# PARC-projects/video-query-algorithms

Measured on AMD Instinct MI355X. Metric: clips/sec TSN feature-extract, higher is better.
Workload: dtype f32; 1 GPU; configs[1]: TSN BN-Inception RGB, 224x224x3, T=3, B=32/GPU (96 crops/step), crops in HBM; global_batch=32, parallelism=dp1

## Files before the change

video-query-algorithms_amd/csrc/vq_tsn.hip:

```cpp
#include <algorithm>
#include <cmath>
#include <cstring>
#include <map>
#include <set>
#include <tuple>
#include <type_traits>
#include <vector>

#include "vq_common.h"
#include "vq_tsn_kernels.h"
#include "host/vq_block_pool.h"

using namespace vq;

typedef float floatx16 __attribute__((ext_vector_type(16)));
typedef float floatx4 __attribute__((ext_vector_type(4)));
typedef unsigned uintx4 __attribute__((__vector_size__(4 * sizeof(unsigned))));

__global__ void preprocess_kernel(const uint8_t* __restrict__ src, float* __restrict__ dst, int64_t nchunk, int C, int Cpad,
                                  const float* __restrict__ mean) {
    const int64_t i = (int64_t)blockIdx.x * blockDim.x + threadIdx.x;
    if (i >= nchunk) return;
    const int cpp = Cpad >> 2;
    const int64_t p = i / cpp;
    const int c0 = (int)(i - p * cpp) * 4;
    floatx4 v;
#pragma unroll
    for (int e = 0; e < 4; ++e) v[e] = c0 + e < C ? (float)src[p * C + c0 + e] - mean[c0 + e] : 0.0f;
    *reinterpret_cast<floatx4*>(dst + p * Cpad + c0) = v;
}

__global__ void preprocess_s2d_kernel(const uint8_t* __restrict__ src, float* __restrict__ dst, int64_t nchunk, int H, int W, int C,
                                      int Hs, int Ws, int pad, const float* __restrict__ mean, int xmajor) {
    const int64_t i = (int64_t)blockIdx.x * blockDim.x + threadIdx.x;
    if (i >= nchunk) return;
    const int64_t cell = i / C;
    const int j0 = (int)(i - cell * C) * 4;
    const int X = (int)(cell % Ws), Y = (int)((cell / Ws) % Hs);
    const int64_t n = cell / ((int64_t)Ws * Hs);
    floatx4 v;
#pragma unroll
    for (int e = 0; e < 4; ++e) {
        const int j = j0 + e, pq = j / C, c = j - pq * C;
        const int p = xmajor ? pq & 1 : pq >> 1, q = xmajor ? pq >> 1 : pq & 1;
        const int y = 2 * Y + p - pad, x = 2 * X + q - pad;
        const bool in = (unsigned)y < (unsigned)H && (unsigned)x < (unsigned)W;
        v[e] = in ? (float)src[((n * H + y) * W + x) * C + c] - mean[c] : 0.0f;
    }
    *reinterpret_cast<floatx4*>(dst + cell * (4 * C) + j0) = v;
}

__global__ __launch_bounds__(256) void preprocess_s2d3_kernel(const uint8_t* __restrict__ src, float* __restrict__ dst, int64_t ncell, int H, int W,
                                                              int Hs, int Ws, int pad, const float* __restrict__ mean, int xmajor) {
    const int64_t cell = (int64_t)blockIdx.x * blockDim.x + threadIdx.x;
    if (cell >= ncell) return;
    const int X = (int)(cell % Ws);
    const int64_t ny = cell / Ws;
    const int Y = (int)(ny % Hs);
    const int64_t n = ny / Hs;
    const float m0 = mean[0], m1 = mean[1], m2 = mean[2];
    float v[12];
#pragma unroll
    for (int p = 0; p < 2; ++p) {
        const int y = 2 * Y + p - pad;
        const bool row_in = (unsigned)y < (unsigned)H;
        const uint8_t* r = src + ((n * H + (row_in ? y : 0)) * W) * 3;
#pragma unroll
        for (int q = 0; q < 2; ++q) {
            const int x = 2 * X + q - pad;
            const bool in = row_in && (unsigned)x < (unsigned)W;
            const uint8_t* px = r + (in ? x : 0) * 3;
            const float a = (float)px[0] - m0, b = (float)px[1] - m1, c = (float)px[2] - m2;
            const int slot = xmajor ? q * 2 + p : p * 2 + q;
            v[slot * 3 + 0] = in ? a : 0.0f;
            v[slot * 3 + 1] = in ? b : 0.0f;
            v[slot * 3 + 2] = in ? c : 0.0f;
        }
    }
    floatx4* o = reinterpret_cast<floatx4*>(dst + cell * 12);
#pragma unroll
    for (int k = 0; k < 3; ++k) {
        floatx4 t;
        t[0] = v[4 * k], t[1] = v[4 * k + 1], t[2] = v[4 * k + 2], t[3] = v[4 * k + 3];
        o[k] = t;
    }
}

struct ConvSeg {
    float* out_base;
    int Cs;
    int relu;
};

struct ConvArgs {
    const float* in;
    const ConvSeg* segs;
    float* out;
    const float* w;
    const float* bias;
    const float* zeros;
    int H, W, Cs_in, coff_in, Cin;
    int Ho, Wo, Cs_out, coff_out, Cout;
    int k, stride, pad;
    int kw;
    int col_off;
    int c_step;
    int M, Kp, relu;
    int out_row0;
    int pool_k, pool_s;
    int tiles_m, tiles_n;
    unsigned in_bytes, w_bytes;
    int ksplit;
    int k_per;
    int seg_stride;
    unsigned m_tiles_n;
    FullDiv d_howo, d_wo;
    unsigned s_wo, s_ho;
};

constexpr int KPAD = 32;
static inline int stem_rows_kp(int c) { return 4 * ((14 * c + 3) / 4 * 4); }

template <int BM, int BN, int BK>
struct ConvSmem {
    float a[2][BM][BK + 4];
    float b[2][BN][BK + 4];
};

#define VQ_EPILOGUE()                                                                                             \
    {                                                                                                             \
        __syncthreads();                                \
        float* patch = reinterpret_cast<float*>(smem_raw) + wave * (32 * 36);                                     \
        const int prow = lane >> 3, pc4 = lane & 7;                                                               \
        const bool full_m = m0 + BM <= a.M;                                                                       \
        _Pragma("unroll") for (int j = 0; j < TN; ++j) {                                                          \
            const int nb = n0 + wn * (BN / WN) + 32 * j;                                                          \
            if (nb < a.Cout) {                                                                                    \
                const ConvSeg sg = seg_v[j];                                                                      \
                _Pragma("unroll") for (int i = 0; i < TM; ++i) {                                                  \
                    _Pragma("unroll") for (int r = 0; r < 16; ++r)                                                \
                        patch[((r & 3) + 8 * (r >> 2) + 4 * half) * 36 + l31] = acc[i][j][r];                     \
                    const int mb = m0 + wm * (BM / WM) + 32 * i;                                                  \
                    _Pragma("unroll") for (int ps = 0; ps < 4; ++ps) {                                            \
                        const int row = prow + 8 * ps;                                                            \
                        floatx4 v = *reinterpret_cast<const floatx4*>(&patch[row * 36 + pc4 * 4]);                \
                        v += bias_v[j];                                                                           \
                        if (sg.relu) {                                                                            \
                            v[0] = fmaxf(v[0], 0.f);                                                              \
                            v[1] = fmaxf(v[1], 0.f);                                                              \
                            v[2] = fmaxf(v[2], 0.f);                                                              \
                            v[3] = fmaxf(v[3], 0.f);                                                              \
                        }                                                                                         \
                        if ((full_m || mb + row < a.M) && nb + pc4 * 4 < a.Cout)                                  \
                            *reinterpret_cast<floatx4*>(sg.out_base + (size_t)(a.out_row0 + mb + row) * sg.Cs + nb + pc4 * 4) = v; \
                    }                                                                                             \
                }                                                                                                 \
            }                                                                                                     \
        }                                                                                                         \
    }

#define VQ_EPILOGUE_BUF()                                                                                         \
    {                                                                                                             \
        __syncthreads();                                \
        float* patch = reinterpret_cast<float*>(smem_raw) + wave * (32 * 36);                                     \
        const int prow = lane >> 3, pc4 = lane & 7;                                                               \
        const bool full_m = m0 + BM <= a.M;                                                                       \
        _Pragma("unroll") for (int j = 0; j < TN; ++j) {                                                          \
            const int nb = n0 + wn * (BN / WN) + 32 * j;                                                          \
            if (nb < a.Cout) {                                                                                    \
                const ConvSeg sg = seg_v[j];                                                                      \
                const __amdgpu_buffer_rsrc_t o_rsrc =                                                             \
                    __builtin_amdgcn_make_buffer_rsrc(sg.out_base + (size_t)a.out_row0 * sg.Cs, 0, 0x7FFFFFF0u, 0x00020000); \
                const unsigned lane_off = nb + pc4 * 4 < a.Cout ? (unsigned)((imul24(prow, sg.Cs) + pc4 * 4) * 4) : 0xFFFFFFFFu; \
                _Pragma("unroll") for (int i = 0; i < TM; ++i) {                                                  \
                    _Pragma("unroll") for (int r = 0; r < 16; ++r)                                                \
                        patch[((r & 3) + 8 * (r >> 2) + 4 * half) * 36 + l31] = acc[i][j][r];                     \
                    const int mb = m0 + wm * (BM / WM) + 32 * i;                                                  \
                    _Pragma("unroll") for (int ps = 0; ps < 4; ++ps) {                                            \
                        const int row = prow + 8 * ps;                                                            \
                        floatx4 v = *reinterpret_cast<const floatx4*>(&patch[row * 36 + pc4 * 4]);                \
                        v += bias_v[j];                                                                           \
                        if (sg.relu) {                                                                            \
                            v[0] = fmaxf(v[0], 0.f);                                                              \
                            v[1] = fmaxf(v[1], 0.f);                                                              \
                            v[2] = fmaxf(v[2], 0.f);                                                              \
                            v[3] = fmaxf(v[3], 0.f);                                                              \
                        }                                                                                         \
                        const unsigned off = (full_m || mb + row < a.M) ? lane_off : 0xFFFFFFFFu;                 \
                        __builtin_amdgcn_raw_buffer_store_b128(__builtin_bit_cast(uintx4, v), o_rsrc, off,        \
                                                               ((mb + 8 * ps) * sg.Cs + nb) * 4, 0);              \
                    }                                                                                             \
                }                                                                                                 \
            }                                                                                                     \
        }                                                                                                         \
    }

template <int BM, int BN, int WM, int WN, int BK, bool SMALL_CIN, bool POOL = false>
__global__ __launch_bounds__(256) void conv_igemm_kernel(ConvArgs a) {
    static_assert(WM * WN == 4, "4 waves per workgroup");
    static_assert(BK == 16 || BK == 32, "BK is 16 or 32");
    static_assert(!(POOL && SMALL_CIN), "the pooled loader walks whole channel chunks");
    constexpr int TM = BM / WM / 32, TN = BN / WN / 32;
    constexpr int CPR = BK / 4;
    constexpr int NA = (BM * CPR + 255) / 256, NB = (BN * CPR + 255) / 256;
    extern __shared__ __attribute__((aligned(16))) char smem_raw[];
    ConvSmem<BM, BN, BK>& sm = *reinterpret_cast<ConvSmem<BM, BN, BK>*>(smem_raw);

    const int tid = threadIdx.x;
    const int n_tiles = a.tiles_m * a.tiles_n;
    const int ks = a.ksplit > 1 ? (int)blockIdx.x / n_tiles : 0;
    const int kbeg = ks * a.k_per;
    const int tile = xcd_remap(blockIdx.x - ks * n_tiles, n_tiles);
    const int m0 = (tile / a.tiles_n) * BM;
    const int n0 = (tile % a.tiles_n) * BN;

    const float* a_img[NA];
    int a_ih0[NA], a_iw0[NA], a_row[NA], a_col[NA];
    const int HoWo = a.Ho * a.Wo;
#pragma unroll
    for (int i = 0; i < NA; ++i) {
        const int c = tid + 256 * i;
        a_row[i] = c / CPR;
        a_col[i] = c % CPR;
        const int m = m0 + a_row[i];
        const bool ok = m < a.M && a_row[i] < BM;
        const int mm = ok ? m : 0;
        const int n_img = mm / HoWo, rem = mm - n_img * HoWo;
        const int oh = rem / a.Wo, ow = rem - oh * a.Wo;
        a_img[i] = a.in + (size_t)n_img * a.H * a.W * a.Cs_in + a.coff_in;
        a_ih0[i] = ok ? oh * a.stride - a.pad : -(1 << 20);
        a_iw0[i] = ow * a.stride - a.pad;
        if (POOL) {
            a_ih0[i] = ok ? oh * a.pool_s : -(1 << 20);
            a_iw0[i] = ow * a.pool_s;
        }
    }
    const float* b_ptr[NB];
    bool b_ok[NB];
    int b_row[NB], b_col[NB];
#pragma unroll
    for (int i = 0; i < NB; ++i) {
        const int c = tid + 256 * i;
        b_row[i] = c / CPR;
        b_col[i] = c % CPR;
        const int n = n0 + b_row[i];
        b_ok[i] = n < a.Cout && b_row[i] < BN;
        b_ptr[i] = a.w + (size_t)(b_ok[i] ? n : 0) * a.Kp + b_col[i] * 4 + kbeg;
    }

    floatx4 ra[NA], rb[NB];
    constexpr int PT = POOL ? 8 : 1;
    floatx4 rp[NA][PT];
    int kh = 0, kw = 0, c0 = 0;
    if (!SMALL_CIN && kbeg > 0) {
        const int tap0 = kbeg / a.Cin;
        c0 = kbeg - tap0 * a.Cin;
        kh = tap0 / a.kw;
        kw = tap0 - kh * a.kw;
    }
#define VQ_LOAD_TILES(KC)                                                                                          \
    {                                                                                                              \
        _Pragma("unroll") for (int i = 0; i < NA; ++i) {                                                           \
            const float* src = a.zeros;                                                                            \
            if (SMALL_CIN) {                                                                                       \
                const int kidx = ((KC) * CPR + a_col[i]) * 4;                                                      \
                const int tap = kidx / a.Cin, c = kidx - tap * a.Cin;                                              \
                const int th = tap / a.kw, tw = tap - th * a.kw;                                                   \
                const int ih = a_ih0[i] + th, iw = a_iw0[i] + tw;                                                  \
                if (tap < a.k * a.kw && (unsigned)ih < (unsigned)a.H && (unsigned)iw < (unsigned)a.W)              \
                    src = a_img[i] + ((size_t)ih * a.W + iw) * a.Cs_in + c;                                        \
            } else if (POOL) {                                                                                     \
                      \
                const bool ok = a_ih0[i] >= 0;                                                                     \
                if (ok) src = a_img[i] + ((size_t)a_ih0[i] * a.W + a_iw0[i]) * a.Cs_in + c0 + a_col[i] * a.col_off; \
                _Pragma("unroll") for (int t = 1; t < 9; ++t) {                                                    \
                    const int ih = a_ih0[i] + t / 3, iw = a_iw0[i] + t % 3;                                        \
                    const float* q = src;                                                                          \
                    if (ok && ih < a.H && iw < a.W) q = a_img[i] + ((size_t)ih * a.W + iw) * a.Cs_in + c0 + a_col[i] * a.col_off; \
                    rp[i][t - 1] = *reinterpret_cast<const floatx4*>(q);                                           \
                }                                                                                                  \
            } else {                                                                                               \
                const int ih = a_ih0[i] + kh, iw = a_iw0[i] + kw;                                                  \
                if ((unsigned)ih < (unsigned)a.H && (unsigned)iw < (unsigned)a.W)                                  \
                    src = a_img[i] + ((size_t)ih * a.W + iw) * a.Cs_in + c0 + a_col[i] * a.col_off;                \
            }                                                                                                      \
            ra[i] = *reinterpret_cast<const floatx4*>(src);                                                        \
        }                                                                                                          \
        _Pragma("unroll") for (int i = 0; i < NB; ++i)                                                             \
            rb[i] = *reinterpret_cast<const floatx4*>(b_ok[i] ? b_ptr[i] + (size_t)(KC) * BK : a.zeros);           \
        if (!SMALL_CIN) {                                                                                          \
            c0 += a.c_step ? a.c_step : BK;                                                                        \
            if (c0 >= a.Cin) {                                                                                     \
                c0 = 0;                                                                                            \
                if (++kw == a.kw) {                                                                                \
                    kw = 0;                                                                                        \
                    ++kh;                                                                                          \
                }                                                                                                  \
            }                                                                                                      \
        }                                                                                                          \
    }
#define VQ_STORE_TILES(BUF)                                                                                        \
    {                                                                                                              \
        if (POOL) {                                                                                                \
            _Pragma("unroll") for (int i = 0; i < NA; ++i)                                                         \
                _Pragma("unroll") for (int t = 0; t < 8; ++t)                                                      \
                    _Pragma("unroll") for (int e = 0; e < 4; ++e) ra[i][e] = fmaxf(ra[i][e], rp[i][t][e]);         \
        }                                                                                                          \
        _Pragma("unroll") for (int i = 0; i < NA; ++i)                                                             \
            if ((BM * CPR) % 256 == 0 || a_row[i] < BM)                                                            \
                *reinterpret_cast<floatx4*>(&sm.a[BUF][a_row[i]][a_col[i] * 4]) = ra[i];                           \
        _Pragma("unroll") for (int i = 0; i < NB; ++i)                                                             \
            if ((BN * CPR) % 256 == 0 || b_row[i] < BN)                                                            \
                *reinterpret_cast<floatx4*>(&sm.b[BUF][b_row[i]][b_col[i] * 4]) = rb[i];                           \
    }

    const int wave = tid >> 6, lane = tid & 63, l31 = lane & 31, half = lane >> 5;
    const int wm = wave / WN, wn = wave % WN;
    const int arow0 = wm * (BM / WM) + l31, brow0 = wn * (BN / WN) + l31;
    floatx16 acc[TM][TN];
#pragma unroll
    for (int i = 0; i < TM; ++i)
#pragma unroll
        for (int j = 0; j < TN; ++j)
#pragma unroll
            for (int r = 0; r < 16; ++r) acc[i][j][r] = 0.f;

    floatx4 bias_v[TN];
    ConvSeg seg_v[TN];
#pragma unroll
    for (int j = 0; j < TN; ++j) {
        const int nb_ = n0 + wn * (BN / WN) + 32 * j;
        const int n = nb_ + (lane & 7) * 4;
        bias_v[j] = *reinterpret_cast<const floatx4*>(a.bias + (n < a.Cout ? n : 0));
        seg_v[j] = a.segs[ks * a.seg_stride + (nb_ < a.Cout ? nb_ >> 5 : 0)];
    }

    const int nk = (a.ksplit > 1 ? a.k_per : a.Kp) / BK;
    VQ_LOAD_TILES(0)
    VQ_STORE_TILES(0)
    __syncthreads();
    for (int kc = 0; kc < nk; ++kc) {
        const int buf = kc & 1;
        if (kc + 1 < nk) VQ_LOAD_TILES(kc + 1)
#pragma unroll
        for (int kk = 0; kk < BK / 8; ++kk) {
            floatx4 af[TM], bf[TN];
#pragma unroll
            for (int i = 0; i < TM; ++i) af[i] = *reinterpret_cast<const floatx4*>(&sm.a[buf][arow0 + 32 * i][kk * 8 + half * 4]);
#pragma unroll
            for (int j = 0; j < TN; ++j) bf[j] = *reinterpret_cast<const floatx4*>(&sm.b[buf][brow0 + 32 * j][kk * 8 + half * 4]);
#pragma unroll
            for (int s = 0; s < 4; ++s)
#pragma unroll
                for (int i = 0; i < TM; ++i)
#pragma unroll
                    for (int j = 0; j < TN; ++j)
                        acc[i][j] = __builtin_amdgcn_mfma_f32_32x32x2f32(af[i][s], bf[j][s], acc[i][j], 0, 0, 0);
        }
        if (kc + 1 < nk) VQ_STORE_TILES(buf ^ 1)
        __syncthreads();
    }

    VQ_EPILOGUE()
#undef VQ_LOAD_TILES
#undef VQ_STORE_TILES
}

#ifndef VQ_PIPE_WPE
#define VQ_PIPE_WPE 4
#endif
template <int BM, int BN, int WM, int WN, int BK, bool SMALL_CIN>
__global__ __launch_bounds__(256) __attribute__((amdgpu_waves_per_eu(BM * BN == 128 * 64 && BK == 16 ? VQ_PIPE_WPE : 1, 8)))
void conv_igemm_pipe_kernel(ConvArgs a) {
    static_assert(WM * WN == 4, "4 waves per workgroup");
    constexpr int NT = 256;
    constexpr int TM = BM / WM / 32, TN = BN / WN / 32;
    constexpr int CPR = BK / 4;
    constexpr int NA = (BM * CPR + NT - 1) / NT, NB = (BN * CPR + NT - 1) / NT;
    constexpr int NKK = BK / 8;
    constexpr int MFK = 4 * TM * TN;
    constexpr int NMF = NKK * MFK;
    constexpr int NFR = TM + TN;
    constexpr int NG = NA + NB;
    constexpr int NFREE = NMF - (NKK - 1) * NFR;
    static_assert(NFREE >= 2 * NG, "not enough MFMA gaps for the staging slices");
    constexpr bool EARLY = (NKK - 1) * (MFK - NFR) >= NG && NFREE - NFR >= 2 * NG;
    extern __shared__ __attribute__((aligned(16))) char smem_raw[];
    ConvSmem<BM, BN, BK>& sm = *reinterpret_cast<ConvSmem<BM, BN, BK>*>(smem_raw);

    const int tid = threadIdx.x;
    const int n_tiles = a.tiles_m * a.tiles_n;
    const int ks = a.ksplit > 1 ? (int)blockIdx.x / n_tiles : 0;
    const int kbeg = ks * a.k_per;
    const int tile = xcd_remap(blockIdx.x - ks * n_tiles, n_tiles);
    const int tm = (int)magic_div((unsigned)tile, a.m_tiles_n);
    const int m0 = tm * BM;
    const int n0 = (tile - tm * a.tiles_n) * BN;
    const unsigned img0 = full_div((unsigned)m0, a.d_howo), rem0 = (unsigned)m0 - img0 * (unsigned)(a.Ho * a.Wo);
    const unsigned oh0 = full_div(rem0, a.d_wo), ow0 = rem0 - oh0 * (unsigned)a.Wo;

    const __amdgpu_buffer_rsrc_t in_rsrc = __builtin_amdgcn_make_buffer_rsrc(const_cast<float*>(a.in), 0, a.in_bytes, 0x00020000);
    const __amdgpu_buffer_rsrc_t w_rsrc = __builtin_amdgcn_make_buffer_rsrc(const_cast<float*>(a.w), 0, a.w_bytes, 0x00020000);
    int a_off[NA];
    unsigned long long a_mask[NA];
    int a_row[NA], a_col[NA];
    const unsigned HW = (unsigned)(a.H * a.W);
#pragma unroll
    for (int i = 0; i < NA; ++i) {
        const int c = tid + NT * i;
        a_row[i] = c / CPR;
        a_col[i] = c % CPR;
        const bool ok = m0 + a_row[i] < a.M && a_row[i] < BM;
        const unsigned lin = ow0 + (unsigned)a_row[i];
        const unsigned q1 = umul24(lin, a.s_wo) >> kRecipShift;
        const unsigned ly = oh0 + q1;
        const unsigned q2 = umul24(ly, a.s_ho) >> kRecipShift;
        const int ow = (int)(lin - umul24(q1, (unsigned)a.Wo)), oh = (int)(ly - umul24(q2, (unsigned)a.Ho));
        const int ih0 = imul24(oh, a.stride) - a.pad, iw0 = imul24(ow, a.stride) - a.pad;
        a_off[i] = (imul24((int)umul24(img0 + q2, HW) + imul24(ih0, a.W) + iw0, a.Cs_in) + a.coff_in + (SMALL_CIN ? 0 : imul24(a_col[i], a.col_off))) * 4;
        unsigned long long mask = 0;
        for (int th = 0; th < a.k; ++th)
            for (int tw = 0; tw < a.kw; ++tw)
                if (ok && (unsigned)(ih0 + th) < (unsigned)a.H && (unsigned)(iw0 + tw) < (unsigned)a.W) mask |= 1ull << (th * a.kw + tw);
        a_mask[i] = mask;
    }
    unsigned b_off[NB];
    int b_row[NB], b_col[NB];
#pragma unroll
    for (int i = 0; i < NB; ++i) {
        const int c = tid + NT * i;
        b_row[i] = c / CPR;
        b_col[i] = c % CPR;
        const int n = n0 + b_row[i];
        b_off[i] = (n < a.Cout && b_row[i] < BN) ? (unsigned)((imul24(n, a.Kp) + b_col[i] * 4 + kbeg) * 4) : 0xFFFFFFFFu;
    }

    floatx4 ra[2][NA], rb[2][NB];
    int kh = 0, kw = 0, c0 = 0, tap = 0;
    unsigned a_voff[NA];
    if (!SMALL_CIN && kbeg > 0) {
        tap = kbeg / a.Cin;
        c0 = kbeg - tap * a.Cin;
        kh = tap / a.kw;
        kw = tap - kh * a.kw;
    }
    {
        const int tap_pix0 = ((kh * a.W + kw) * a.Cs_in) * 4;
#pragma unroll
        for (int i = 0; i < NA; ++i) a_voff[i] = ((a_mask[i] >> tap) & 1ull) ? (unsigned)(a_off[i] + tap_pix0) : 0xFFFFFFFFu;
    }
    const int c_step = a.c_step ? a.c_step : BK;
    const unsigned cpt = (unsigned)a.Cin >> 2, inv_cpt = 65536u / cpt + 1u, inv_k = 65536u / (unsigned)a.kw + 1u;

    const int wave = __builtin_amdgcn_readfirstlane(tid >> 6), lane = tid & 63, l31 = lane & 31, half = lane >> 5;
    const int wm = wave / WN, wn = wave % WN;
    const int arow0 = wm * (BM / WM) + l31, brow0 = wn * (BN / WN) + l31;
    floatx16 acc[TM][TN];
#pragma unroll
    for (int i = 0; i < TM; ++i)
#pragma unroll
        for (int j = 0; j < TN; ++j)
#pragma unroll
            for (int r = 0; r < 16; ++r) acc[i][j][r] = 0.f;
    floatx4 bias_v[TN];
    ConvSeg seg_v[TN];
#pragma unroll
    for (int j = 0; j < TN; ++j) {
        const int nb_ = n0 + wn * (BN / WN) + 32 * j;
        const int n = nb_ + (lane & 7) * 4;
        bias_v[j] = *reinterpret_cast<const floatx4*>(a.bias + (n < a.Cout ? n : 0));
        seg_v[j] = a.segs[ks * a.seg_stride + (nb_ < a.Cout ? nb_ >> 5 : 0)];
    }

#define VQ_G_LOAD(IDX, KC, SET)                                                                                \
    {                                                                                                          \
        if ((IDX) < NA) {                                                                                      \
            const int ii = (IDX) < NA ? (IDX) : 0;                                                             \
            unsigned off;                                                                                      \
            if (SMALL_CIN) {                                                                                   \
                const unsigned g_ = (unsigned)(KC) * CPR + a_col[ii];                                          \
                const unsigned tap_ = (g_ * inv_cpt) >> 16, c4_ = g_ - tap_ * cpt;                             \
                const unsigned th_ = (tap_ * inv_k) >> 16, tw_ = tap_ - th_ * a.kw;                            \
                const unsigned ok_ = (unsigned)(a_mask[ii] >> (tap_ & 63u)) & (tap_ < 64u ? 1u : 0u);          \
                off = ok_ ? (unsigned)(a_off[ii] + (int)(((th_ * a.W + tw_) * a.Cs_in + c4_ * 4) * 4)) : 0xFFFFFFFFu; \
            } else {                                                                                           \
                off = a_voff[ii];                                                                              \
            }                                                                                                  \
            ra[SET][ii] = __builtin_bit_cast(floatx4, __builtin_amdgcn_raw_buffer_load_b128(in_rsrc, off, SMALL_CIN ? 0 : c0 * 4, 0)); \
        } else {                                                                                               \
            const int ii = (IDX) >= NA ? (IDX) - NA : 0;                                                       \
            rb[SET][ii] = __builtin_bit_cast(floatx4, __builtin_amdgcn_raw_buffer_load_b128(w_rsrc, b_off[ii], (KC) * (BK * 4), 0)); \
        }                                                                                                      \
    }
#define VQ_G_STORE(IDX, BUF, SET)                                                                              \
    {                                                                                                          \
        if ((IDX) < NA) {                                                                                      \
            const int ii = (IDX) < NA ? (IDX) : 0;                                                             \
            if ((BM * CPR) % NT == 0 || a_row[ii] < BM)                                                        \
                *reinterpret_cast<floatx4*>(&sm.a[BUF][a_row[ii]][a_col[ii] * 4]) = ra[SET][ii];               \
        } else {                                                                                               \
            const int ii = (IDX) >= NA ? (IDX) - NA : 0;                                                       \
            if ((BN * CPR) % NT == 0 || b_row[ii] < BN)                                                        \
                *reinterpret_cast<floatx4*>(&sm.b[BUF][b_row[ii]][b_col[ii] * 4]) = rb[SET][ii];               \
        }                                                                                                      \
    }
#define VQ_ADVANCE_TAP()                                                                     \
    if (!SMALL_CIN) {                                                                        \
        c0 += c_step;                                                                        \
        if (c0 >= a.Cin) {                                                                   \
            c0 = 0;                                                                          \
            ++tap;                                                                           \
            if (++kw == a.kw) {                                                              \
                kw = 0;                                                                      \
                ++kh;                                                                        \
            }                                                                                \
            asm volatile("" ::: "memory");                  \
            const int tap_pix = ((kh * a.W + kw) * a.Cs_in) * 4;                             \
            _Pragma("unroll") for (int i = 0; i < NA; ++i)                                   \
                a_voff[i] = ((a_mask[i] >> tap) & 1ull) ? (unsigned)(a_off[i] + tap_pix) : 0xFFFFFFFFu; \
        }                                                                                    \
    }
#define VQ_PIPE_STEP(BUF, KC, DO_STORE, DO_LOAD, SS, SL)                                                       \
    {                                                                                                          \
        if (!EARLY) {                                                                                          \
            _Pragma("unroll") for (int i = 0; i < TM; ++i)                                                     \
                fa[0][i] = *reinterpret_cast<const floatx4*>(&sm.a[BUF][arow0 + 32 * i][half * 4]);            \
            _Pragma("unroll") for (int j = 0; j < TN; ++j)                                                     \
                fb[0][j] = *reinterpret_cast<const floatx4*>(&sm.b[BUF][brow0 + 32 * j][half * 4]);            \
        }                                                                                                      \
        _Pragma("unroll") for (int q = 0; q < NMF; ++q) {                                                      \
            const int kk = q / MFK, r = q % MFK, s_ = r / (TM * TN), i_ = (r / TN) % TM, j_ = r % TN;          \
            acc[i_][j_] = __builtin_amdgcn_mfma_f32_32x32x2f32(fa[kk & 1][i_][s_], fb[kk & 1][j_][s_], acc[i_][j_], 0, 0, 0); \
            if (kk + 1 < NKK && r < NFR) {                                                                     \
                if (r < TM)                                                                                    \
                    fa[(kk + 1) & 1][r < TM ? r : 0] = *reinterpret_cast<const floatx4*>(                      \
                        &sm.a[BUF][arow0 + 32 * (r < TM ? r : 0)][(kk + 1) * 8 + half * 4]);                   \
                else                                                                                           \
                    fb[(kk + 1) & 1][r >= TM ? r - TM : 0] = *reinterpret_cast<const floatx4*>(                \
                        &sm.b[BUF][brow0 + 32 * (r >= TM ? r - TM : 0)][(kk + 1) * 8 + half * 4]);             \
            } else if (EARLY && (DO_STORE) && kk + 1 == NKK && r < NFR) {                                      \
                if (r < TM)                                                                                    \
                    fa[0][r < TM ? r : 0] = *reinterpret_cast<const floatx4*>(                                 \
                        &sm.a[(BUF) ^ 1][arow0 + 32 * (r < TM ? r : 0)][half * 4]);                            \
                else                                                                                           \
                    fb[0][r >= TM ? r - TM : 0] = *reinterpret_cast<const floatx4*>(                           \
                        &sm.b[(BUF) ^ 1][brow0 + 32 * (r >= TM ? r - TM : 0)][half * 4]);                      \
            } else {                                                                                           \
                const int fidx = q - (kk + 1 < NKK ? (kk + 1) * NFR : (NKK - 1) * NFR + (EARLY && (DO_STORE) ? NFR : 0)); \
                if ((DO_STORE) && fidx < NG) {                                                                 \
                    VQ_G_STORE(fidx < NG ? fidx : 0, (BUF) ^ 1, SS)                                            \
                    if (EARLY && fidx == NG - 1) __syncthreads();            \
                } else if ((DO_LOAD) && fidx >= NG && fidx < 2 * NG)                                           \
                    VQ_G_LOAD(fidx - NG < NG ? fidx - NG : 0, (KC) + 2, SL)                                    \
            }                                                                                                  \
            __builtin_amdgcn_sched_barrier(0);                                                                 \
        }                                                                                                      \
    }

    const int nk = (a.ksplit > 1 ? a.k_per : a.Kp) / BK;
    _Pragma("unroll") for (int i = 0; i < NG; ++i) VQ_G_LOAD(i, 0, 0)
    _Pragma("unroll") for (int i = 0; i < NG; ++i) VQ_G_STORE(i, 0, 0)
    if (nk > 1) {
        VQ_ADVANCE_TAP()
        _Pragma("unroll") for (int i = 0; i < NG; ++i) VQ_G_LOAD(i, 1, 1)
    }
    __syncthreads();
    floatx4 fa[2][TM], fb[2][TN];
    if (EARLY) {
#pragma unroll
        for (int i = 0; i < TM; ++i) fa[0][i] = *reinterpret_cast<const floatx4*>(&sm.a[0][arow0 + 32 * i][half * 4]);
#pragma unroll
        for (int j = 0; j < TN; ++j) fb[0][j] = *reinterpret_cast<const floatx4*>(&sm.b[0][brow0 + 32 * j][half * 4]);
    }
#define VQ_END_BARRIER()                                                     \
    {                                                                        \
        if (EARLY) {                                                         \
            asm volatile("s_waitcnt lgkmcnt(%0)" ::"n"(NFR) : "memory");     \
            __builtin_amdgcn_s_barrier();                                    \
            asm volatile("" ::: "memory");                                   \
        } else {                                                             \
            __syncthreads();                                                 \
        }                                                                    \
    }
    const int n_steady = nk > 2 ? nk - 2 : 0;
    int kc = 0;
    for (; kc + 1 < n_steady; kc += 2) {
        VQ_ADVANCE_TAP()
        VQ_PIPE_STEP(0, kc, true, true, 1, 0)
        VQ_END_BARRIER()
        VQ_ADVANCE_TAP()
        VQ_PIPE_STEP(1, kc + 1, true, true, 0, 1)
        VQ_END_BARRIER()
    }
    if (kc < n_steady) {
        VQ_ADVANCE_TAP()
        VQ_PIPE_STEP(0, kc, true, true, 1, 0)
        VQ_END_BARRIER()
        ++kc;
    }
    if (kc + 1 < nk) {
        if (kc & 1) {
            VQ_PIPE_STEP(1, kc, true, false, 0, 0)
        } else {
            VQ_PIPE_STEP(0, kc, true, false, 1, 1)
        }
        VQ_END_BARRIER()
        ++kc;
    }
    if (kc & 1) {
        VQ_PIPE_STEP(1, kc, false, false, 0, 0)
    } else {
        VQ_PIPE_STEP(0, kc, false, false, 0, 0)
    }
    VQ_EPILOGUE_BUF()
#undef VQ_G_LOAD
#undef VQ_G_STORE
#undef VQ_ADVANCE_TAP
#undef VQ_PIPE_STEP
#undef VQ_END_BARRIER
}

template <int BM, int BN, int WM, int WN>
__global__ __launch_bounds__(256) void pool_gemm_kernel(ConvArgs a) {
    static_assert(WM * WN == 4, "4 waves per workgroup");
    static_assert(BM == 64 || BM == 128, "two staged chunks per thread and slab");
    constexpr int TM = BM / WM / 32, TN = BN / WN / 32;
    constexpr int SLAB = 2048 / BM;
    constexpr int CPS = SLAB / 4;
    constexpr int GS = SLAB / 8;
    extern __shared__ __attribute__((aligned(16))) char smem_raw[];
    float* As = reinterpret_cast<float*>(smem_raw);
    const int K = a.Cin, pitch = K + 4;
    const int tid = threadIdx.x;
    const int tile = xcd_remap(blockIdx.x, a.tiles_m * a.tiles_n);
    const int m0 = (tile / a.tiles_n) * BM, n0 = (tile % a.tiles_n) * BN;
    const __amdgpu_buffer_rsrc_t in_rsrc = __builtin_amdgcn_make_buffer_rsrc(const_cast<float*>(a.in), 0, a.in_bytes, 0x00020000);
    const __amdgpu_buffer_rsrc_t w_rsrc = __builtin_amdgcn_make_buffer_rsrc(const_cast<float*>(a.w), 0, a.w_bytes, 0x00020000);

    const int wave = tid >> 6, lane = tid & 63, l31 = lane & 31, half = lane >> 5;
    const int wm = wave / WN, wn = wave % WN;
    floatx4 bias_v[TN];
    ConvSeg seg_v[TN];
    unsigned b_voff[TN];
#pragma unroll
    for (int j = 0; j < TN; ++j) {
        const int nb_ = n0 + wn * (BN / WN) + 32 * j;
        const int n = nb_ + (lane & 7) * 4;
        bias_v[j] = *reinterpret_cast<const floatx4*>(a.bias + (n < a.Cout ? n : 0));
        seg_v[j] = a.segs[nb_ < a.Cout ? nb_ >> 5 : 0];
        b_voff[j] = nb_ + l31 < a.Cout ? (unsigned)(((nb_ + l31) * a.Kp + half * 4) * 4) : 0xFFFFFFFFu;
    }

    unsigned tap_base[2], tap_ok[2];
    int a_dst[2];
    const int px = a.Cs_in * 4, rowb = a.W * px;
    {
        const int HoWo = a.Ho * a.Wo;
#pragma unroll
        for (int u = 0; u < 2; ++u) {
            const int idx = tid + 256 * u, row = idx / CPS, col = idx % CPS;
            const int m = m0 + row;
            const bool ok = m < a.M;
            const int mm = ok ? m : 0;
            const int n_img = mm / HoWo, rem = mm - n_img * HoWo;
            const int oh = rem / a.Wo, ow = rem - oh * a.Wo;
            const int ih0 = oh * a.pool_s, iw0 = ow * a.pool_s;
            tap_base[u] = ok ? (unsigned)((((n_img * a.H + ih0) * a.W + iw0) * a.Cs_in + a.coff_in + col * 4) * 4) : 0xFFFFFFFFu;
            const int nvy = min(3, a.H - ih0), nvx = min(3, a.W - iw0);
            unsigned mask = 0;
#pragma unroll
            for (int t = 0; t < 9; ++t)
                if (ok && t / 3 < nvy && t % 3 < nvx) mask |= 1u << t;
            tap_ok[u] = mask;
            a_dst[u] = row * pitch + col * 4;
        }
    }
    floatx4 v[2][9];
#define VQ_PG_TAPS(S)                                                                                               \
    _Pragma("unroll") for (int u = 0; u < 2; ++u) {                                                                 \
        unsigned inside = tap_ok[u];                                                                                \
        asm volatile("" : "+v"(inside));  \
        _Pragma("unroll") for (int t = 0; t < 9; ++t)                                                               \
            v[u][t] = __builtin_bit_cast(floatx4, __builtin_amdgcn_raw_buffer_load_b128(                            \
                in_rsrc, tap_base[u] + (((inside >> t) & 1u) ? (unsigned)((t / 3) * rowb + (t % 3) * px) : 0u), (S) * (SLAB * 4), 0)); \
    }
#define VQ_PG_POOL(S)                                                                                               \
    _Pragma("unroll") for (int u = 0; u < 2; ++u) {                                                                 \
        floatx4 r;                                                                                                  \
        _Pragma("unroll") for (int e = 0; e < 4; ++e) {                                                             \
            const float x = __builtin_fmaxf(__builtin_fmaxf(v[u][0][e], v[u][1][e]), v[u][2][e]);                  \
            const float y = __builtin_fmaxf(__builtin_fmaxf(v[u][3][e], v[u][4][e]), v[u][5][e]);                  \
            const float z = __builtin_fmaxf(__builtin_fmaxf(v[u][6][e], v[u][7][e]), v[u][8][e]);                  \
            r[e] = __builtin_fmaxf(__builtin_fmaxf(x, y), z);                                                       \
        }                                                                                                           \
        *reinterpret_cast<floatx4*>(As + a_dst[u] + (S) * SLAB) = r;                                                \
    }

    floatx16 acc[TM][TN];
#pragma unroll
    for (int i = 0; i < TM; ++i)
#pragma unroll
        for (int j = 0; j < TN; ++j)
#pragma unroll
            for (int r = 0; r < 16; ++r) acc[i][j][r] = 0.f;
    const float* a_frag = As + (wm * (BM / WM) + l31) * pitch + half * 4;
    floatx4 fa[2][TM], fbs[2][GS][TN];
#define VQ_PG_FETCH_B(SET, S)                                                                                       \
    _Pragma("unroll") for (int q = 0; q < GS; ++q)                                                                  \
        _Pragma("unroll") for (int j = 0; j < TN; ++j)                                                              \
            fbs[SET][q][j] = __builtin_bit_cast(floatx4, __builtin_amdgcn_raw_buffer_load_b128(w_rsrc, b_voff[j], ((S) * GS + q) * 32, 0));
#define VQ_PG_FETCH_A(SET, G)                                                                                       \
    _Pragma("unroll") for (int i = 0; i < TM; ++i)                                                                  \
        fa[SET][i] = *reinterpret_cast<const floatx4*>(a_frag + 32 * i * pitch + (G) * 8);
#define VQ_PG_MFMA(SET, BSET, Q)                                                                                    \
    _Pragma("unroll") for (int s_ = 0; s_ < 4; ++s_)                                                                \
        _Pragma("unroll") for (int i = 0; i < TM; ++i)                                                              \
            _Pragma("unroll") for (int j = 0; j < TN; ++j)                                                          \
                acc[i][j] = __builtin_amdgcn_mfma_f32_32x32x2f32(fa[SET][i][s_], fbs[BSET][Q][j][s_], acc[i][j], 0, 0, 0);
#define VQ_PG_SLAB(S, BSET)                                                                                         \
    {                                                                                                               \
        const bool more = (S) + 1 < ns;                                                                             \
        if (more) {                                                                                                 \
            VQ_PG_FETCH_B((BSET) ^ 1, (S) + 1)                                                                      \
            VQ_PG_TAPS((S) + 1)                                              \
        }                                                                                                           \
        VQ_PG_FETCH_A(0, (S) * GS)                                                                                  \
        __builtin_amdgcn_sched_barrier(0);                                                                          \
        _Pragma("unroll") for (int q = 0; q < GS; ++q) {                                                            \
            if (q + 1 < GS) VQ_PG_FETCH_A((q + 1) & 1, (S) * GS + q + 1)                                            \
            __builtin_amdgcn_sched_barrier(0);                                                                      \
            VQ_PG_MFMA(q & 1, BSET, q)                                                                              \
            __builtin_amdgcn_sched_barrier(0);                                                                      \
        }                                                                                                           \
        if (more) {                                                                                                 \
            VQ_PG_POOL((S) + 1)                                                                                     \
            __syncthreads();                                  \
        }                                                                                                           \
    }

    const int ns = K / SLAB;
    VQ_PG_FETCH_B(0, 0)
    VQ_PG_TAPS(0)
    VQ_PG_POOL(0)
    __syncthreads();
    int s = 0;
    for (; s + 1 < ns; s += 2) {
        VQ_PG_SLAB(s, 0)
        VQ_PG_SLAB(s + 1, 1)
    }
    if (s < ns) VQ_PG_SLAB(s, 0)
#undef VQ_PG_SLAB
#undef VQ_PG_TAPS
#undef VQ_PG_POOL
#undef VQ_PG_FETCH_A
#undef VQ_PG_FETCH_B
#undef VQ_PG_MFMA
    VQ_EPILOGUE()
}

template <bool IS_MAX>
__global__ __launch_bounds__(256) void pool_kernel(PoolArgs a) {
    const int64_t i = (int64_t)blockIdx.x * blockDim.x + threadIdx.x;
    if (i < a.total) pool_one<IS_MAX>(a, i);
}

__global__ void gavgpool_kernel(const float* __restrict__ in, float* __restrict__ out, int n, int HW, int Cs_in, int coff_in,
                                int C, int Cs_out, int coff_out) {
    const int i = blockIdx.x * blockDim.x + threadIdx.x;
    if (i >= n * C) return;
    const int c = i % C, img = i / C;
    const float* p = in + (size_t)img * HW * Cs_in + coff_in + c;
    float acc = 0.f;
    for (int q = 0; q < HW; ++q) acc += p[(size_t)q * Cs_in];
    out[(size_t)img * Cs_out + coff_out + c] = acc / (float)HW;
}

__global__ void splitk_combine_kernel(const float* __restrict__ part, int ksplit, size_t slice_stride, int M, int Cout,
                                      const float* __restrict__ bias, int relu, float* __restrict__ out, int Cs_out) {
    const int64_t i = (int64_t)blockIdx.x * blockDim.x + threadIdx.x;
    const int c4 = Cout / 4;
    if (i >= (int64_t)M * c4) return;
    const int m = (int)(i / c4), n = (int)(i - (int64_t)m * c4) * 4;
    floatx4 v = *reinterpret_cast<const floatx4*>(part + (size_t)m * Cout + n);
    for (int q = 1; q < ksplit; ++q) v += *reinterpret_cast<const floatx4*>(part + q * slice_stride + (size_t)m * Cout + n);
    v += *reinterpret_cast<const floatx4*>(bias + n);
    if (relu) {
        v[0] = fmaxf(v[0], 0.f);
        v[1] = fmaxf(v[1], 0.f);
        v[2] = fmaxf(v[2], 0.f);
        v[3] = fmaxf(v[3], 0.f);
    }
    *reinterpret_cast<floatx4*>(out + (size_t)m * Cs_out + n) = v;
}

constexpr int kMaxFusedT = 16;
__global__ void gavgpool_consensus_kernel(const float* __restrict__ in, float* __restrict__ out, double* __restrict__ feat, int T,
                                          int HW, int Cs_in, int coff_in, int C, int Cs_out, int coff_out) {
    __shared__ float pooled[kMaxFusedT][64];
    const int c = blockIdx.x * 64 + threadIdx.x, t = threadIdx.y, b = blockIdx.y;
    float v = 0.f;
    if (c < C) {
        const int img = b * T + t;
        const float* p = in + (size_t)img * HW * Cs_in + coff_in + c;
        float acc = 0.f;
        int q = 0;
        for (; q + 7 <= HW; q += 7) {
            float x[7];
#pragma unroll
            for (int u = 0; u < 7; ++u) x[u] = p[(size_t)(q + u) * Cs_in];
#pragma unroll
            for (int u = 0; u < 7; ++u) acc += x[u];
        }
        for (; q < HW; ++q) acc += p[(size_t)q * Cs_in];
        v = acc / (float)HW;
        out[(size_t)img * Cs_out + coff_out + c] = v;
    }
    pooled[t][threadIdx.x] = v;
    __syncthreads();
    if (t == 0 && c < C) {
        double cons = (double)pooled[0][threadIdx.x];
        for (int s = 1; s < T; ++s) cons = cons + (double)pooled[s][threadIdx.x];
        feat[(size_t)b * C + c] = cons / (double)T;
    }
}

__global__ void consensus_kernel(const float* __restrict__ per_snippet, double* __restrict__ feat, int B, int T, int D, int Cs) {
    const int i = blockIdx.x * blockDim.x + threadIdx.x;
    if (i >= B * D) return;
    const int d = i % D, b = i / D;
    double acc = (double)per_snippet[(size_t)(b * T) * Cs + d];
    for (int t = 1; t < T; ++t) acc = acc + (double)per_snippet[(size_t)(b * T + t) * Cs + d];
    feat[i] = acc / (double)T;
}

static inline double first_layer_k2c(const vq_input_desc& in, const vq_layer_desc& L) {
    if (L.src != 0) return (double)L.k * L.k * L.cin;
    const int k = (in.s2d_pad >= 0 && in.s2d_kernel > 0) ? in.s2d_kernel : L.k;
    return (double)k * k * in.c;
}

static inline bool is_wino(int op) { return op == VQ_OP_CONV_WINOGRAD || op == VQ_OP_CONV_WINOGRAD16; }
static inline bool is_conv(int op) { return op == VQ_OP_CONV || is_wino(op); }

struct LaunchItem {
    int kind = 0;
    std::vector<int> layers;
    int max_crops = 0;
};

struct vq_tsn {
    std::mutex mu;
    int device = 0;
    hipStream_t stream = nullptr;
    int cus = 256;
    int max_crops = 0;
    int in_channels = 0;
    vq_input_desc input = {0, 0, 0, -1, 0};
    std::vector<vq_tensor_desc> tensors;
    std::vector<vq_layer_desc> layers;
    std::vector<LaunchItem> items;
    std::vector<int> item_of_layer;
    int consensus_layer = -1;
    std::map<int, std::vector<int>> tuned;
    std::map<int, int> split_pref;
    std::set<int> tuned_borrowed;
    bool autotune = true;
    bool group_wino = true;
    bool group_pool = true;
    bool poison = false;
    int forced_tile = -1;
    std::vector<float*> slots;
    std::vector<size_t> slot_bytes;
    size_t blob_bytes = 0;
    float* zeros = nullptr;
    ConvSeg* seg_table = nullptr;
    std::vector<int> seg_table_off;
    std::vector<int> ksplit;
    float* split_scratch = nullptr;
    size_t split_slice_floats = 0;
    size_t split_crop_floats = 0;
    float* zero_bias = nullptr;
    float* blob = nullptr;
    int64_t blob_floats = 0;
    int feature_slot = -1, D = 0;
    uint8_t* crops_dev = nullptr;
    size_t crops_cap = 0;
    float* mean_dev = nullptr;
    std::vector<float> mean_cached;
    double* feat_dev = nullptr;
    double flops_per_crop = 0;
    int last_crops = 0;
    int cur_T = 1;
    bool fused_consensus = false;
    int profile_depth = 0;
    int profile_count = 0;
    int profile_every = 1;
    int profile_tick = 0;
    bool profile_split = false;
    std::vector<hipEvent_t> events;
    int crop_off = 0;
    int n_split = 1;
    std::vector<int> split_parts;
    hipStream_t ls = nullptr;
    hipEvent_t ev_start = nullptr, ev_stop = nullptr;
    std::vector<hipStream_t> split_streams;
    hipEvent_t fork_ev = nullptr;
    std::vector<hipEvent_t> join_ev;
};

static vq::BlockPool& device_pool() {
    static vq::BlockPool p(vq::BlockPool::cap_from_env());
    return p;
}
void vq::device_pool_trim() {
    for (void* blk : device_pool().drain()) (void)hipFree(blk);
}
static hipError_t pool_alloc(int device, size_t bytes, void** out) {
    if (void* blk = device_pool().take(device, bytes)) {
        *out = blk;
        return hipSuccess;
    }
    hipError_t e = hipMalloc(out, bytes);
    if (e == hipErrorOutOfMemory) {
        (void)hipGetLastError();
        vq::device_pool_trim();
        e = hipMalloc(out, bytes);
    }
    return e;
}
static void pool_free(int device, void* p, size_t bytes) {
    if (!p) return;
    if (!device_pool().give(device, p, bytes)) (void)hipFree(p);
}

static void tsn_free(vq_tsn* net) {
    for (hipEvent_t e : net->events) (void)hipEventDestroy(e);
    net->events.clear();
    for (hipEvent_t e : net->join_ev)
        if (e) (void)hipEventDestroy(e);
    if (net->fork_ev) (void)hipEventDestroy(net->fork_ev);
    for (hipStream_t st : net->split_streams)
        if (st) (void)hipStreamDestroy(st);
    for (size_t i = 0; i < net->slots.size(); ++i) pool_free(net->device, net->slots[i], i < net->slot_bytes.size() ? net->slot_bytes[i] : 0);
    pool_free(net->device, net->blob, net->blob_bytes);
    if (net->zeros) (void)hipFree(net->zeros);
    if (net->seg_table) (void)hipFree(net->seg_table);
    pool_free(net->device, net->split_scratch, net->split_slice_floats * 4 * sizeof(float));
    if (net->zero_bias) (void)hipFree(net->zero_bias);
    if (net->crops_dev) (void)hipFree(net->crops_dev);
    if (net->mean_dev) (void)hipFree(net->mean_dev);
    if (net->feat_dev) (void)hipFree(net->feat_dev);
}

enum : int { kConv = 1, kPipe = 2, kPool = 4, kGemm = 8 };

constexpr size_t kPoolGemmMaxLds = 64 * 1024;
static size_t pool_gemm_lds(int bm, int K) { return std::max((size_t)bm * (K + 4) * sizeof(float), (size_t)4 * 32 * 36 * sizeof(float)); }

static bool pixel_walk_ok(const ConvArgs& a) {
    const long long n_img = cdiv(a.M, a.Ho * a.Wo);
    return n_img * a.H * a.W < (1 << 23) && a.Cs_in < (1 << 23) && a.Kp < (1 << 23) && a.Cout < (1 << 23) && a.stride < (1 << 23) &&
           recip22_ok((unsigned)a.Wo, (unsigned)a.Wo + 128u) && recip22_ok((unsigned)a.Ho, (unsigned)a.Ho + 130u);
}

template <int BM, int BN, int WM, int WN, int BK, int KERNEL, bool SMALL>
static int launch_conv_t(vq_tsn* net, ConvArgs& a) {
    a.tiles_m = cdiv(a.M, BM);
    a.tiles_n = cdiv(a.Cout, BN);
    void (*kern)(ConvArgs);
    size_t lds = sizeof(ConvSmem<BM, BN, BK>), lds_max = lds;
    if constexpr (KERNEL == kPipe) {
        VQ_REQUIRE(pixel_walk_ok(a) && (unsigned long long)a.tiles_m * a.tiles_n * a.tiles_n < 0x100000000ull,
                   "pipelined convolution: shape outside the range of its reciprocal divisions");
        a.m_tiles_n = a.tiles_n == 1 ? 0u : (unsigned)(0x100000000ull / (unsigned)a.tiles_n) + 1u;
        a.d_howo = full_div_for((unsigned)(a.Ho * a.Wo));
        a.d_wo = full_div_for((unsigned)a.Wo);
        a.s_wo = recip22((unsigned)a.Wo);
        a.s_ho = recip22((unsigned)a.Ho);
        kern = conv_igemm_pipe_kernel<BM, BN, WM, WN, BK, SMALL>;
    } else if constexpr (KERNEL == kGemm) {
        VQ_REQUIRE(a.pool_k == 3 && a.Cin % 32 == 0 && a.Kp == a.Cin, "pool_gemm_kernel: a 3x3 window over a multiple of 32 channels");
        kern = pool_gemm_kernel<BM, BN, WM, WN>;
        lds = pool_gemm_lds(BM, a.Cin);
        lds_max = kPoolGemmMaxLds;
    } else {
        kern = conv_igemm_kernel<BM, BN, WM, WN, BK, SMALL, KERNEL == kPool>;
    }
    VQ_DYN_LDS(kern, lds_max);
    VQ_LAUNCH(kern, a.tiles_m * a.tiles_n * a.ksplit, 256, lds, net->ls, net->ev_start, net->ev_stop, a);
    VQ_CHECK_LAUNCH();
    return VQ_OK;
}

typedef int (*ConvLaunch)(vq_tsn*, ConvArgs&);

struct ConvTile {
    int bm, bn, bk;
    int pipe;
    ConvLaunch conv[2];
    ConvLaunch piped[2];
    ConvLaunch pooled;
};

template <int BM, int BN, int BK, int WM, int WN, int HAS>
constexpr ConvTile tiling() {
    ConvTile t{BM, BN, BK, (HAS & kGemm) ? 3 : (HAS & kPipe) ? 1 : 0, {}, {}, nullptr};
    if constexpr ((HAS & (kConv | kPipe)) != 0) {
        t.conv[0] = launch_conv_t<BM, BN, WM, WN, BK, kConv, false>;
        t.conv[1] = launch_conv_t<BM, BN, WM, WN, BK, kConv, true>;
    }
    if constexpr ((HAS & kPipe) != 0) {
        t.piped[0] = launch_conv_t<BM, BN, WM, WN, BK, kPipe, false>;
        t.piped[1] = launch_conv_t<BM, BN, WM, WN, BK, kPipe, true>;
    }
    if constexpr ((HAS & kPool) != 0) t.pooled = launch_conv_t<BM, BN, WM, WN, BK, kPool, false>;
    if constexpr ((HAS & kGemm) != 0) t.pooled = launch_conv_t<BM, BN, WM, WN, BK, kGemm, false>;
    return t;
}

static constexpr ConvTile kTiles[] = {
    tiling<128, 128, 32, 2, 2, kConv>(), tiling<128, 128, 16, 2, 2, kConv | kPool>(),
    tiling<128, 96, 32, 4, 1, kConv>(),  tiling<128, 96, 16, 4, 1, kConv | kPool>(),
    tiling<128, 64, 32, 2, 2, kConv>(),  tiling<128, 64, 16, 2, 2, kConv | kPool>(),
    tiling<64, 128, 32, 2, 2, kConv | kPool>(), tiling<64, 128, 16, 2, 2, kConv | kPool>(),
    tiling<64, 64, 32, 2, 2, kConv | kPool>(),  tiling<64, 64, 16, 2, 2, kConv | kPool>(),
    tiling<128, 32, 32, 4, 1, kConv>(),  tiling<128, 32, 16, 4, 1, kConv | kPool>(),
    tiling<32, 128, 32, 1, 4, kConv>(),  tiling<32, 128, 16, 1, 4, kConv>(),
    tiling<128, 128, 32, 2, 2, kPipe>(), tiling<128, 128, 16, 2, 2, kPipe>(),
    tiling<128, 96, 32, 4, 1, kPipe>(),  tiling<128, 96, 16, 4, 1, kPipe>(),
    tiling<128, 64, 32, 2, 2, kPipe>(),  tiling<128, 64, 16, 2, 2, kPipe>(),
    tiling<64, 128, 32, 2, 2, kPipe>(),  tiling<64, 128, 16, 2, 2, kPipe>(),
    tiling<64, 64, 32, 2, 2, kPipe>(),   tiling<64, 64, 16, 2, 2, kPipe>(),
    tiling<128, 32, 32, 4, 1, kPipe>(),  tiling<128, 32, 16, 4, 1, kPipe>(),
    tiling<32, 128, 32, 1, 4, kPipe>(),  tiling<32, 128, 16, 1, 4, kPipe>(),
    tiling<64, 256, 16, 1, 4, kPool>(), tiling<64, 256, 8, 1, 4, kGemm>(), tiling<64, 64, 8, 2, 2, kGemm>(), tiling<128, 64, 8, 2, 2, kGemm>()};
constexpr int kNumTiles = (int)(sizeof(kTiles) / sizeof(kTiles[0]));

static int tile_index(int bm, int bn, int bk, int pipe) {
    for (int i = 0; i < kNumTiles; ++i)
        if (kTiles[i].bm == bm && kTiles[i].bn == bn && kTiles[i].bk == bk && kTiles[i].pipe == pipe) return i;
    return -1;
}

static bool pooled_ok(const ConvTile& t, int K) { return t.pooled && (t.pipe != 3 || pool_gemm_lds(t.bm, K) <= kPoolGemmMaxLds); }

static bool tile_candidate(const vq_layer_desc& L, const ConvTile& t, bool timed) {
    if (!timed) return t.pipe == 0 && t.bk == 32 && t.conv[0];
    if (L.pre_pool_k > 0 ? !pooled_ok(t, L.cin) : !t.conv[0]) return false;
    return t.bn < 2 * ((L.cout + 63) / 64 * 64);
}

static int heuristic_tile(const vq_tsn* net, int li, int n_crops) {
    const vq_layer_desc& L = net->layers[li];
    const vq_tensor_desc& td = net->tensors[L.dst];
    const int M = n_crops * td.h * td.w, N = L.cout;
    int best = 0;
    double bs = -1;
    for (int i = 0; i < kNumTiles; ++i) {
        const ConvTile& t = kTiles[i];
        if (!tile_candidate(L, t, false)) continue;
        const long long tiles = (long long)cdiv(M, t.bm) * cdiv(N, t.bn);
        const double per_cu = (double)tiles / net->cus;
        const double balance = per_cu / std::ceil(per_cu);
        const double padding = ((double)M * N) / ((double)tiles * t.bm * t.bn);
        const double area = (double)t.bm * t.bn;
        const double intrinsic = area >= 128 * 128 ? 1.0 : area >= 128 * 96 ? 0.97 : area >= 128 * 64 ? 0.92 : area >= 64 * 64 ? 0.8 : 0.7;
        const double sc = balance * padding * intrinsic;
        if (sc > bs) {
            bs = sc;
            best = i;
        }
    }
    return best;
}

static ConvLaunch conv_launch(const vq_tsn* net, int li, const ConvArgs& a, bool stem_rows, int ti) {
    const ConvTile* t = &kTiles[ti];
    if (net->layers[li].pre_pool_k > 0) {
        if (!pooled_ok(*t, a.Cin)) ti = tile_index(std::min(t->bm, 128), std::min(t->bn, 128), 16, 0);
        return ti < 0 ? nullptr : kTiles[ti].pooled;
    }
    if (stem_rows) ti = tile_index(t->bm, t->bn, 16, t->pipe);
    if (ti < 0) return nullptr;
    t = &kTiles[ti];
    const bool small = (a.Cin % t->bk) != 0;
    return t->piped[small] && pixel_walk_ok(a) ? t->piped[small] : t->conv[small];
}

static void fill_conv_args(vq_tsn* net, int li, int n_crops, ConvArgs& a) {
    const vq_layer_desc& L = net->layers[li];
    const vq_tensor_desc& ts = net->tensors[L.src];
    const vq_tensor_desc& td = net->tensors[L.dst];
    a.in = net->slots[L.src] + (size_t)net->crop_off * ts.h * ts.w * ts.c;
    a.out = net->slots[L.dst];
    a.out_row0 = net->crop_off * td.h * td.w;
    a.w = net->blob + L.w_off;
    a.bias = net->blob + L.b_off;
    a.zeros = net->zeros;
    a.segs = net->seg_table + net->seg_table_off[li];
    a.H = ts.h;
    a.W = ts.w;
    a.Cs_in = ts.c;
    a.coff_in = L.src_coff;
    a.Cin = L.cin;
    a.Ho = td.h;
    a.Wo = td.w;
    a.Cs_out = td.c;
    a.coff_out = L.dst_coff;
    a.Cout = L.cout;
    a.k = L.k;
    a.kw = L.k;
    a.col_off = 4;
    a.c_step = 0;
    a.stride = L.stride;
    a.pad = L.pad;
    a.M = n_crops * td.h * td.w;
    a.Kp = (L.k * L.k * L.cin + KPAD - 1) / KPAD * KPAD;
    a.relu = L.relu;
    a.pool_k = L.pre_pool_k;
    a.pool_s = L.pre_pool_stride;
    a.ksplit = 1;
    a.k_per = 0;
    a.seg_stride = 0;
    a.tiles_m = a.tiles_n = 0;
    a.in_bytes = (unsigned)((size_t)n_crops * ts.h * ts.w * ts.c * sizeof(float));
    a.w_bytes = (unsigned)((size_t)L.cout * a.Kp * sizeof(float));
}

static int launch_conv_layer(vq_tsn* net, int li, int n_crops, int tile_idx) {
    ConvArgs a;
    fill_conv_args(net, li, n_crops, a);
    const vq_layer_desc& L = net->layers[li];
    const bool stem_rows = L.src == 0 && net->input.s2d_pad >= 0 && net->input.s2d_order == 1;
    if (stem_rows) {
        a.k = a.kw = 1;
        a.Cin = 4 * L.k * L.cin;
        a.col_off = net->tensors[L.src].w * net->tensors[L.src].c;
        a.c_step = 4;
        a.Kp = stem_rows_kp(net->input.c);
        a.w_bytes = (unsigned)((size_t)L.cout * a.Kp * sizeof(float));
    } else if (L.pad == 0 && L.k > 1 && L.cin == net->tensors[L.src].c && L.src_coff == 0) {
        a.kw = 1;
        a.Cin = L.k * L.cin;
    }
    const ConvLaunch run = conv_launch(net, li, a, stem_rows, tile_idx);
    const ConvTile& t = kTiles[tile_idx];
    if (!run) return fail(VQ_E_INVALID, "layer %d: no kernel for tile %dx%dx%d pipe=%d", li, t.bm, t.bn, t.bk, t.pipe);
    if (net->ksplit[li] == 1) return run(net, a);
    const hipEvent_t e0 = net->ev_start, e1 = net->ev_stop;
    a.ksplit = net->ksplit[li];
    a.k_per = a.Kp / a.ksplit;
    a.seg_stride = (L.cout + 31) / 32;
    a.bias = net->zero_bias;
    a.out_row0 = (int)cdiv((int64_t)net->crop_off * (int64_t)net->split_crop_floats, (int64_t)L.cout);
    net->ev_stop = nullptr;
    int rc = run(net, a);
    net->ev_stop = e1;
    if (rc != VQ_OK) return rc;
    net->ev_start = nullptr;
    const vq_tensor_desc& td = net->tensors[L.dst];
    float* out = net->slots[L.dst] + (size_t)net->crop_off * td.h * td.w * td.c + L.dst_coff;
    const int64_t work = (int64_t)a.M * (L.cout / 4);
    VQ_LAUNCH(splitk_combine_kernel, (unsigned)cdiv(work, 256), 256, 0, net->ls, net->ev_start, net->ev_stop,
              net->split_scratch + (size_t)a.out_row0 * L.cout, a.ksplit, net->split_slice_floats, a.M, L.cout, net->blob + L.b_off, L.relu, out, td.c);
    net->ev_start = e0;
    VQ_CHECK_LAUNCH();
    return VQ_OK;
}

static void fill_wino_job(vq_tsn* net, int li, int n_crops, WinoJob& a, int variant) {
    const vq_layer_desc& L = net->layers[li];
    const vq_tensor_desc& ts = net->tensors[L.src];
    const vq_tensor_desc& td = net->tensors[L.dst];
    memset(&a, 0, sizeof a);
    a.in = net->slots[L.src] + (size_t)net->crop_off * ts.h * ts.w * ts.c;
    a.u = net->blob + L.w_off;
    a.bias = net->blob + L.b_off;
    a.out = net->slots[L.dst] + (size_t)net->crop_off * td.h * td.w * td.c;
    a.H = ts.h;
    a.W = ts.w;
    a.Cs_in = ts.c;
    a.coff_in = L.src_coff;
    a.Cin = L.cin;
    a.Cs_out = td.c;
    a.coff_out = L.dst_coff;
    a.Cout = L.cout;
    a.th = (ts.h + 1) / 2;
    a.tw = (ts.w + 1) / 2;
    a.P = n_crops * a.th * a.tw;
    a.relu = L.relu;
    a.t16 = L.op == VQ_OP_CONV_WINOGRAD16 && variant >= 2;
    if (a.t16) a.u += (size_t)16 * L.cout * L.cin;
    a.in_bytes = (unsigned)((size_t)n_crops * ts.h * ts.w * ts.c * sizeof(float));
    a.out_bytes = (unsigned)((size_t)n_crops * td.h * td.w * td.c * sizeof(float));
    a.u_bytes = (unsigned)((size_t)16 * L.cout * L.cin * sizeof(float));
}

static void fill_pool_args(vq_tsn* net, int li, int n_crops, PoolArgs& a) {
    const vq_layer_desc& L = net->layers[li];
    const vq_tensor_desc& ts = net->tensors[L.src];
    const vq_tensor_desc& td = net->tensors[L.dst];
    memset(&a, 0, sizeof a);
    a.in = net->slots[L.src] + (size_t)net->crop_off * ts.h * ts.w * ts.c;
    a.out = net->slots[L.dst] + (size_t)net->crop_off * td.h * td.w * td.c;
    a.H = ts.h;
    a.W = ts.w;
    a.Cs_in = ts.c;
    a.coff_in = L.src_coff;
    a.C = L.cin;
    a.Ho = td.h;
    a.Wo = td.w;
    a.Cs_out = td.c;
    a.coff_out = L.dst_coff;
    a.k = L.k;
    a.stride = L.stride;
    a.pad = L.pad;
    a.is_max = L.op == VQ_OP_MAXPOOL;
    a.total = (int64_t)n_crops * td.h * td.w * (L.cin / 4);
    a.bias = (L.op == VQ_OP_AVGPOOL && L.has_bias) ? net->blob + L.b_off : nullptr;
    a.relu = (L.op == VQ_OP_AVGPOOL) ? L.relu : 0;
}

static int launch_wino_layers(vq_tsn* net, const std::vector<int>& members, int n_crops, int variant) {
    WinoGroup g;
    memset(&g, 0, sizeof g);
    for (int li : members) {
        if (is_wino(net->layers[li].op)) {
            VQ_REQUIRE(g.n_jobs < kWinoMaxJobs, "a Winograd launch carries at most %d convolutions", kWinoMaxJobs);
            fill_wino_job(net, li, n_crops, g.job[g.n_jobs++], variant);
        } else {
            VQ_REQUIRE(g.n_pools < kWinoMaxPools, "a Winograd launch carries at most %d pooling layers", kWinoMaxPools);
            fill_pool_args(net, li, n_crops, g.pool[g.n_pools++]);
        }
    }
    bool both = true;
    for (int li : members)
        if (net->layers[li].op == VQ_OP_CONV_WINOGRAD) both = false;
    if (variant >= 2 && !both) {
        variant -= 2;
        for (int q = 0; q < g.n_jobs; ++q) VQ_REQUIRE(!g.job[q].t16, "internal: mixed Winograd layouts in one launch");
    }
    return launch_wino_group(g, variant, net->ls, net->ev_start, net->ev_stop);
}

static int run_layer(vq_tsn* net, int li, int n_crops, int tune_key);

static int run_item(vq_tsn* net, const LaunchItem& it, int crop0, int n_crops, int tune_key) {
    const hipEvent_t e0 = net->ev_start, e1 = net->ev_stop;
    for (int done = 0; done < n_crops;) {
        const int n = std::min(n_crops - done, it.max_crops);
        net->crop_off = crop0 + done;
        net->ev_start = done == 0 ? e0 : nullptr;
        net->ev_stop = done + n == n_crops ? e1 : nullptr;
        int rc;
        if (it.kind == 1) {
            auto tn = net->tuned.find(tune_key);
            rc = launch_wino_layers(net, it.layers, n, tn != net->tuned.end() ? tn->second[it.layers[0]] : 0);
        } else {
            rc = run_layer(net, it.layers[0], n, tune_key);
        }
        if (rc != VQ_OK) {
            net->crop_off = 0;
            net->ev_start = net->ev_stop = nullptr;
            return rc;
        }
        done += n;
    }
    net->crop_off = 0;
    net->ev_start = net->ev_stop = nullptr;
    return VQ_OK;
}

constexpr int kPairedKey = 1 << 24;
static inline int tile_key(int n_crops, bool paired) { return n_crops + (paired ? kPairedKey : 0); }

struct EventSet {
    std::vector<hipEvent_t> ev;
    ~EventSet() {
        for (hipEvent_t e : ev)
            if (e) (void)hipEventDestroy(e);
    }
};

static int autotune(vq_tsn* net, int n_crops, bool paired) {
    const int key = tile_key(n_crops, paired);
    std::vector<int>& choice = net->tuned[key];
    choice.assign(net->layers.size(), 0);
    net->tuned_borrowed.erase(key);
    net->ls = net->stream;
    const int ways = paired ? std::max(1, std::min(net->n_split, net->max_crops / n_crops)) : 1;
    EventSet events;
    events.ev.assign(2 + ways, nullptr);
    for (int l = 0; l < 2 + ways; ++l)
        if (l != 2) VQ_HIP(hipEventCreate(&events.ev[l]));
    const hipEvent_t e0 = events.ev[0], e1 = events.ev[1];
    hipEvent_t* const f = events.ev.data() + 2;
    auto timed = [&](const LaunchItem& it, int reps, float* ms) -> int {
        VQ_HIP(hipEventRecord(e0, net->stream));
        int rc = run_item(net, it, 0, n_crops, key);
        if (rc != VQ_OK) return rc;
        VQ_HIP(hipEventRecord(e1, net->stream));
        VQ_HIP(hipEventSynchronize(e1));
        float warm = 0.f;
        VQ_HIP(hipEventElapsedTime(&warm, e0, e1));
        if (warm > 2.0f) reps = 1;
        VQ_HIP(hipEventRecord(e0, net->stream));
        for (int l = 1; l < ways; ++l) VQ_HIP(hipStreamWaitEvent(net->split_streams[l], e0, 0));
        for (int r = 0; r < reps; ++r)
            for (int l = 0; l < ways; ++l) {
                net->ls = l > 0 ? net->split_streams[l] : net->stream;
                rc = run_item(net, it, l * n_crops, n_crops, key);
                net->ls = net->stream;
                if (rc != VQ_OK) return rc;
            }
        VQ_HIP(hipEventRecord(e1, net->stream));
        for (int l = 1; l < ways; ++l) VQ_HIP(hipEventRecord(f[l], net->split_streams[l]));
        VQ_HIP(hipEventSynchronize(e1));
        VQ_HIP(hipEventElapsedTime(ms, e0, e1));
        for (int l = 1; l < ways; ++l) {
            float other = 0.f;
            VQ_HIP(hipEventSynchronize(f[l]));
            VQ_HIP(hipEventElapsedTime(&other, e0, f[l]));
            *ms = std::max(*ms, other);
        }
        return VQ_OK;
    };
    {
        std::vector<int> saved = choice;
        net->tuned.erase(key);
        for (int r = 0; r < 10; ++r)
            for (const LaunchItem& it : net->items) {
                const int rc = run_item(net, it, 0, n_crops, key);
                if (rc != VQ_OK) return rc;
            }
        VQ_HIP(hipStreamSynchronize(net->stream));
        net->tuned[key] = saved;
    }
    std::vector<int>& pick = net->tuned[key];
    for (const LaunchItem& it : net->items) {
        const int li = it.layers[0];
        if (!is_conv(net->layers[li].op)) continue;
        const bool wino = is_wino(net->layers[li].op);
        std::vector<std::pair<float, int>> seen;
        const int n_wino = net->layers[li].op == VQ_OP_CONV_WINOGRAD16 ? 2 * kWinoVariants : kWinoVariants;
        for (int t = 0; t < (wino ? n_wino : kNumTiles); ++t) {
            if (!wino && !tile_candidate(net->layers[li], kTiles[t], true)) continue;
            for (int m : it.layers) pick[m] = t;
            float ms = 0.f;
            const int rc = timed(it, 3, &ms);
            if (rc != VQ_OK) return rc;
            seen.emplace_back(ms, t);
        }
        std::sort(seen.begin(), seen.end());
        float best = 1e30f;
        int win = seen.empty() ? 0 : seen[0].second;
        for (size_t k = 0; k < std::min<size_t>(3, seen.size()) && seen.size() > 1; ++k) {
            for (int m : it.layers) pick[m] = seen[k].second;
            float ms = 0.f;
            const int rc = timed(it, 5, &ms);
            if (rc != VQ_OK) return rc;
            if (ms < best) {
                best = ms;
                win = seen[k].second;
            }
        }
        for (int m : it.layers) pick[m] = win;
    }
    return VQ_OK;
}

static int ensure_tuned(vq_tsn* net, int n_crops, bool paired) {
    const int key = tile_key(n_crops, paired);
    if (net->forced_tile >= 0 || net->tuned.find(key) != net->tuned.end()) return VQ_OK;
    int nearest = 0, nearest_key = 0;
    for (int same = 1; same >= 0 && nearest == 0; --same)
        for (const auto& kv : net->tuned) {
            const bool kp = kv.first >= kPairedKey;
            const int size = kv.first - (kp ? kPairedKey : 0);
            if ((kp == paired) != (same == 1) || net->tuned_borrowed.count(kv.first)) continue;
            if (10 * std::max(size, n_crops) > 16 * std::min(size, n_crops)) continue;
            if (nearest == 0 || std::abs(size - n_crops) < std::abs(nearest - n_crops)) {
                nearest = size;
                nearest_key = kv.first;
            }
        }
    if (nearest > 0) {
        net->tuned[key] = net->tuned[nearest_key];
        net->tuned_borrowed.insert(key);
        return VQ_OK;
    }
    if (!net->autotune) return VQ_OK;
    return autotune(net, n_crops, paired);
}

static int run_layer(vq_tsn* net, int li, int n_crops, int tune_key) {
    const vq_layer_desc& L = net->layers[li];
    const vq_tensor_desc& ts = net->tensors[L.src];
    const vq_tensor_desc& td = net->tensors[L.dst];
    if (L.op == VQ_OP_CONV) {
        int t = net->forced_tile;
        if (t < 0) {
            auto it = net->tuned.find(tune_key);
            t = it != net->tuned.end() ? it->second[li] : heuristic_tile(net, li, n_crops);
        }
        return launch_conv_layer(net, li, n_crops, t);
    }
    if (is_wino(L.op)) {
        auto it = net->tuned.find(tune_key);
        return launch_wino_layers(net, std::vector<int>{li}, n_crops, it != net->tuned.end() ? it->second[li] : 0);
    }
    if (L.op == VQ_OP_MAXPOOL || L.op == VQ_OP_AVGPOOL) {
        PoolArgs a;
        fill_pool_args(net, li, n_crops, a);
        const int64_t blocks = (a.total + 255) / 256;
        if (L.op == VQ_OP_MAXPOOL)
            VQ_LAUNCH(pool_kernel<true>, (unsigned)blocks, 256, 0, net->ls, net->ev_start, net->ev_stop, a);
        else
            VQ_LAUNCH(pool_kernel<false>, (unsigned)blocks, 256, 0, net->ls, net->ev_start, net->ev_stop, a);
        VQ_CHECK_LAUNCH();
        return VQ_OK;
    }
    if (L.op == VQ_OP_GLOBAL_AVGPOOL) {
        const float* gin = net->slots[L.src] + (size_t)net->crop_off * ts.h * ts.w * ts.c;
        float* gout = net->slots[L.dst] + (size_t)net->crop_off * td.c;
        const int T = net->cur_T;
        if (li == net->consensus_layer && net->fused_consensus) {
            const int B = n_crops / T;
            VQ_LAUNCH(gavgpool_consensus_kernel, dim3(cdiv(L.cin, 64), B), dim3(64, T), 0, net->ls, net->ev_start, net->ev_stop, gin, gout,
                      net->feat_dev + (size_t)(net->crop_off / T) * net->D, T, ts.h * ts.w, ts.c, L.src_coff, L.cin, td.c, L.dst_coff);
        } else {
            VQ_LAUNCH(gavgpool_kernel, cdiv((int64_t)n_crops * L.cin, 256), 256, 0, net->ls, net->ev_start, net->ev_stop, gin, gout, n_crops,
                      ts.h * ts.w, ts.c, L.src_coff, L.cin, td.c, L.dst_coff);
        }
        VQ_CHECK_LAUNCH();
        return VQ_OK;
    }
    return fail(VQ_E_INVALID, "layer %d: unknown op %d", li, L.op);
}

static int pool_out_size(int size, int k, int s, int p) {
    int out = (size + 2 * p - k + s - 1) / s + 1;
    if (p > 0 && (out - 1) * s >= size + p) --out;
    return out;
}

struct SlotRange {
    int slot, c0, c1;
};
static bool overlaps(const std::vector<SlotRange>& x, const std::vector<SlotRange>& y) {
    for (const SlotRange& p : x)
        for (const SlotRange& q : y)
            if (p.slot == q.slot && p.c0 < q.c1 && q.c0 < p.c1) return true;
    return false;
}

static void build_items(vq_tsn* net, const vq_conv_segment* segments) {
    const int n = (int)net->layers.size();
    std::vector<std::vector<SlotRange>> rd(n), wr(n);
    for (int i = 0; i < n; ++i) {
        const vq_layer_desc& L = net->layers[i];
        const bool whole = L.op == VQ_OP_CONV && L.cin % KPAD != 0;
        rd[i].push_back(whole ? SlotRange{L.src, 0, net->tensors[L.src].c} : SlotRange{L.src, L.src_coff, L.src_coff + L.cin});
        if (L.op == VQ_OP_CONV && L.seg_count > 0)
            for (int q = 0; q < L.seg_count; ++q) {
                const vq_conv_segment& sg = segments[L.seg_first + q];
                wr[i].push_back(SlotRange{sg.dst, sg.dst_coff, sg.dst_coff + sg.cout});
            }
        else
            wr[i].push_back(SlotRange{L.dst, L.dst_coff, L.dst_coff + L.cout});
    }
    std::vector<int> level(n, 0), floor_level(n, 0);
    int n_levels = 0;
    auto levelise = [&]() {
        n_levels = 0;
        for (int i = 0; i < n; ++i) {
            level[i] = floor_level[i];
            for (int j = 0; j < i; ++j)
                if (overlaps(wr[j], rd[i]) || overlaps(rd[j], wr[i]) || overlaps(wr[j], wr[i])) level[i] = std::max(level[i], level[j] + 1);
            n_levels = std::max(n_levels, level[i] + 1);
        }
    };
    levelise();
    if (net->group_wino && net->group_pool) {
        for (int i = 0; i < n; ++i) {
            const int op = net->layers[i].op;
            if (op != VQ_OP_MAXPOOL && op != VQ_OP_AVGPOOL) continue;
            bool here = false, next = false;
            for (int j = 0; j < n; ++j)
                if (is_wino(net->layers[j].op)) {
                    here |= level[j] == level[i];
                    next |= level[j] == level[i] + 1;
                }
            if (!here && next) floor_level[i] = level[i] + 1;
        }
        levelise();
    }
    auto slot_bytes_per_crop = [&](int slot) {
        const vq_tensor_desc& t = net->tensors[slot];
        return (size_t)t.h * t.w * t.c * sizeof(float);
    };
    auto item_limit = [&](const std::vector<int>& members) {
        size_t worst = 1;
        for (int li : members) {
            const vq_layer_desc& L = net->layers[li];
            worst = std::max(worst, slot_bytes_per_crop(L.src));
            if (L.op == VQ_OP_CONV && L.seg_count > 0)
                for (int q = 0; q < L.seg_count; ++q) worst = std::max(worst, slot_bytes_per_crop(segments[L.seg_first + q].dst));
            else
                worst = std::max(worst, slot_bytes_per_crop(L.dst));
        }
        size_t limit = std::max<size_t>(1, (size_t)0x7FFFFFF0u / worst);
        for (int li : members) {
            const vq_layer_desc& L = net->layers[li];
            if (!is_wino(L.op)) continue;
            for (int slot : {L.src, L.dst}) {
                const vq_tensor_desc& t = net->tensors[slot];
                limit = std::min(limit, std::max<size_t>(1, ((size_t)(1u << 23) - 1) / ((size_t)t.h * t.w)));
            }
            const vq_tensor_desc& ts = net->tensors[L.src];
            const size_t tpi = (size_t)((ts.h + 1) / 2) * ((ts.w + 1) / 2);
            if ((1ull << 32) / tpi > 64) limit = std::min(limit, std::max<size_t>(1, ((size_t)((1ull << 32) / tpi) - 64) / tpi));
        }
        return (int)limit;
    };
    net->items.clear();
    net->item_of_layer.assign(n, -1);
    for (int lv = 0; lv < n_levels; ++lv) {
        std::vector<int> wino, pools;
        for (int i = 0; i < n; ++i)
            if (level[i] == lv && is_wino(net->layers[i].op) && net->group_wino) wino.push_back(i);
        for (int i = 0; i < n; ++i) {
            if (level[i] != lv || (is_wino(net->layers[i].op) && net->group_wino)) continue;
            const int op = net->layers[i].op;
            if (!wino.empty() && (op == VQ_OP_MAXPOOL || op == VQ_OP_AVGPOOL) && (int)pools.size() < kWinoMaxPools && net->group_pool) {
                pools.push_back(i);
                continue;
            }
            LaunchItem it;
            it.kind = 0;
            it.layers = {i};
            it.max_crops = item_limit(it.layers);
            net->item_of_layer[i] = (int)net->items.size();
            net->items.push_back(it);
        }
        std::stable_sort(wino.begin(), wino.end(), [&](int x, int y) {
            if (net->layers[x].op != net->layers[y].op) return net->layers[x].op < net->layers[y].op;
            return net->layers[x].cin > net->layers[y].cin;
        });
        for (size_t q = 0; q < wino.size();) {
            size_t end = q;
            while (end < wino.size() && end - q < (size_t)kWinoMaxJobs && net->layers[wino[end]].op == net->layers[wino[q]].op) ++end;
            LaunchItem it;
            it.kind = 1;
            it.layers.assign(wino.begin() + q, wino.begin() + end);
            const bool first = q == 0;
            q = end;
            if (first) it.layers.insert(it.layers.end(), pools.begin(), pools.end());
            it.max_crops = item_limit(it.layers);
            for (int m : it.layers) net->item_of_layer[m] = (int)net->items.size();
            net->items.push_back(it);
        }
    }
}

extern "C" {

int vq_tsn_create(const vq_tensor_desc* tensors, int32_t n_tensors, const vq_layer_desc* layers, int32_t n_layers,
                  const vq_conv_segment* segments, int32_t n_segments, const float* blob_host, int64_t blob_floats,
                  const vq_input_desc* input, int32_t feature_slot, int32_t max_crops, int32_t device, vq_tsn** out) {
    VQ_REQUIRE(out, "out is NULL");
    *out = nullptr;
    VQ_REQUIRE(tensors && layers && blob_host && input, "NULL argument");
    const int in_channels = input->c;
    VQ_REQUIRE(n_tensors > 0 && n_layers > 0 && blob_floats > 0 && max_crops > 0, "sizes must be positive");
    VQ_REQUIRE(n_segments >= 0 && (n_segments == 0 || segments), "bad segment table");
    VQ_REQUIRE(feature_slot > 0 && feature_slot < n_tensors, "feature_slot out of range");
    VQ_REQUIRE(tensors[feature_slot].h == 1 && tensors[feature_slot].w == 1, "feature slot must be 1x1xD");
    VQ_REQUIRE(tensors[0].c % 4 == 0, "input slot channels must be padded to a multiple of 4 (got %d)", tensors[0].c);
    VQ_REQUIRE(input->h > 0 && input->w > 0 && in_channels > 0, "input crops must be h x w x c with positive sizes");
    if (input->s2d_pad < 0) {
        VQ_REQUIRE(tensors[0].h == input->h && tensors[0].w == input->w, "input slot is %dx%d but the crops are %dx%d", tensors[0].h,
                   tensors[0].w, input->h, input->w);
        VQ_REQUIRE(in_channels <= tensors[0].c && tensors[0].c - in_channels < 4, "in_channels %d does not fit the %d-channel input slot",
                   in_channels, tensors[0].c);
    } else {
        VQ_REQUIRE(tensors[0].c == 4 * in_channels, "space-to-depth input slot needs 4 x %d channels (got %d)", in_channels, tensors[0].c);
        VQ_REQUIRE(input->s2d_pad <= 64, "space-to-depth shift out of range");
        VQ_REQUIRE(input->s2d_order == 0 || input->s2d_order == 1, "s2d_order must be 0 or 1");
    }
    double macs = 0;
    for (int i = 0; i < n_layers; ++i) {
        const vq_layer_desc& L = layers[i];
        const bool multi = L.op == VQ_OP_CONV && L.seg_count > 0;
        VQ_REQUIRE(L.src >= 0 && L.src < n_tensors && L.dst > 0 && L.dst < n_tensors && L.src != L.dst,
                   "layer %d: bad tensor slots %d -> %d", i, L.src, L.dst);
        const vq_tensor_desc& ts = tensors[L.src];
        const vq_tensor_desc& td = tensors[L.dst];
        VQ_REQUIRE((size_t)ts.h * ts.w * ts.c * sizeof(float) <= 0x7FFFFFF0u && (size_t)td.h * td.w * td.c * sizeof(float) <= 0x7FFFFFF0u,
                   "layer %d: one crop of a tensor slot exceeds 2 GiB", i);
        VQ_REQUIRE(L.src_coff >= 0 && L.cin > 0 && L.src_coff + L.cin <= ts.c, "layer %d: reads channels [%d,%d) of a %d-channel slot",
                   i, L.src_coff, L.src_coff + L.cin, ts.c);
        VQ_REQUIRE(multi || (L.dst_coff >= 0 && L.cout > 0 && L.dst_coff + L.cout <= td.c),
                   "layer %d: writes channels [%d,%d) of a %d-channel slot", i, L.dst_coff, L.dst_coff + L.cout, td.c);
        if (multi) {
            VQ_REQUIRE(L.seg_first >= 0 && L.seg_first + L.seg_count <= n_segments, "layer %d: segments outside the table", i);
            int sum = 0;
            for (int q = 0; q < L.seg_count; ++q) {
                const vq_conv_segment& sg = segments[L.seg_first + q];
                VQ_REQUIRE(sg.dst > 0 && sg.dst < n_tensors && sg.dst != L.src, "layer %d segment %d: bad slot", i, q);
                const vq_tensor_desc& t2 = tensors[sg.dst];
                VQ_REQUIRE(sg.cout > 0 && sg.cout % 32 == 0 && sg.dst_coff >= 0 && sg.dst_coff % 4 == 0 && sg.dst_coff + sg.cout <= t2.c,
                           "layer %d segment %d: channels [%d,%d) do not fit a %d-channel slot (cout must be a multiple of 32)", i, q,
                           sg.dst_coff, sg.dst_coff + sg.cout, t2.c);
                VQ_REQUIRE(t2.h == td.h && t2.w == td.w && t2.c % 4 == 0, "layer %d segment %d: spatial size differs", i, q);
                sum += sg.cout;
            }
            VQ_REQUIRE(sum == L.cout, "layer %d: segments cover %d of %d output channels", i, sum, L.cout);
        }
        VQ_REQUIRE(L.k >= 1 && L.stride >= 1 && L.pad >= 0 && L.pad < L.k, "layer %d: bad kernel/stride/pad", i);
        VQ_REQUIRE(ts.c % 4 == 0 && td.c % 4 == 0 && L.src_coff % 4 == 0 && L.dst_coff % 4 == 0 && L.cin % 4 == 0 && L.cout % 4 == 0,
                   "layer %d: channel counts and offsets must be multiples of 4", i);
        if (L.op == VQ_OP_CONV) {
            VQ_REQUIRE(L.k <= 8, "layer %d: conv kernels up to 8x8 (the tap mask is 64 bits)", i);
            if (L.pre_pool_k > 0) {
                VQ_REQUIRE(L.pre_pool_k == 3 && L.pre_pool_stride >= 1 && L.pre_pool_stride <= 3,
                           "layer %d: the pooled-input form takes a 3x3 max window with stride 1..3", i);
                VQ_REQUIRE(L.k == 1 && L.stride == 1 && L.pad == 0 && L.cin % 32 == 0, "layer %d: the pooled-input form is a 1x1 convolution over a multiple of 32 channels", i);
                VQ_REQUIRE(td.h == pool_out_size(ts.h, 3, L.pre_pool_stride, 0) && td.w == pool_out_size(ts.w, 3, L.pre_pool_stride, 0),
                           "layer %d: pooled-input size mismatch (Caffe ceil rule)", i);
            } else
            VQ_REQUIRE(td.h == (ts.h + 2 * L.pad - L.k) / L.stride + 1 && td.w == (ts.w + 2 * L.pad - L.k) / L.stride + 1,
                       "layer %d: conv output size mismatch", i);
            int64_t kp = (int64_t)(L.k * L.k * L.cin + KPAD - 1) / KPAD * KPAD;
            if (L.src == 0 && input->s2d_pad >= 0 && input->s2d_order == 1) {
                VQ_REQUIRE(L.k == 4 && L.cin == 4 * in_channels && L.stride == 1 && L.pad == 0 && L.src_coff == 0 && L.pre_pool_k == 0 &&
                               L.seg_count == 0 && input->s2d_kernel == 7,
                           "layer %d: the x-major space-to-depth stem is a 7x7 / stride-2 convolution reading the whole input slot", i);
                kp = stem_rows_kp(in_channels);
            }
            VQ_REQUIRE(L.w_off >= 0 && L.w_off % 4 == 0 && L.w_off + (int64_t)L.cout * kp <= blob_floats,
                       "layer %d: weights outside the blob", i);
            VQ_REQUIRE(L.b_off >= 0 && L.b_off + L.cout <= blob_floats, "layer %d: bias outside the blob", i);
            VQ_REQUIRE(L.cin % KPAD == 0 || L.src_coff == 0, "layer %d: small-Cin convolution must read a whole slot", i);
            VQ_REQUIRE(L.cin % KPAD == 0 || L.cin == ts.c, "layer %d: small-Cin convolution must read a whole slot", i);
            macs += (double)td.h * td.w * L.cout * first_layer_k2c(*input, L);
        } else if (is_wino(L.op)) {
            VQ_REQUIRE(L.k == 3 && L.stride == 1 && L.pad == 1 && L.seg_count == 0, "layer %d: Winograd form is 3x3 / stride 1 / pad 1, one destination", i);
            VQ_REQUIRE(L.cin % (L.op == VQ_OP_CONV_WINOGRAD16 ? 16 : 8) == 0 && L.cout % 32 == 0,
                       "layer %d: Winograd form needs Cin %% 8 == 0 (16-tile units: %% 16) and Cout %% 32 == 0", i);
            VQ_REQUIRE(td.h == ts.h && td.w == ts.w, "layer %d: conv output size mismatch", i);
            VQ_REQUIRE(L.w_off >= 0 && L.w_off % 4 == 0 &&
                           L.w_off + (int64_t)(L.op == VQ_OP_CONV_WINOGRAD16 ? 2 : 1) * 16 * L.cout * L.cin <= blob_floats,
                       "layer %d: transformed filters outside the blob", i);
            VQ_REQUIRE(L.b_off >= 0 && L.b_off % 4 == 0 && L.b_off + L.cout <= blob_floats, "layer %d: bias outside the blob", i);
            macs += (double)td.h * td.w * L.cout * L.cin * 9;
        } else if (L.op == VQ_OP_MAXPOOL || L.op == VQ_OP_AVGPOOL) {
            VQ_REQUIRE(L.cin == L.cout, "layer %d: pooling keeps the channel count", i);
            VQ_REQUIRE(!(L.op == VQ_OP_AVGPOOL && L.has_bias) || (L.b_off >= 0 && L.b_off % 4 == 0 && L.b_off + L.cout <= blob_floats),
                       "layer %d: pooling bias outside the blob", i);
            VQ_REQUIRE(td.h == pool_out_size(ts.h, L.k, L.stride, L.pad) && td.w == pool_out_size(ts.w, L.k, L.stride, L.pad),
                       "layer %d: pooling output size mismatch (Caffe ceil rule)", i);
        } else if (L.op == VQ_OP_GLOBAL_AVGPOOL) {
            VQ_REQUIRE(L.cin == L.cout && td.h == 1 && td.w == 1, "layer %d: global pool must write a 1x1 slot", i);
        } else {
            return fail(VQ_E_INVALID, "layer %d: unknown op %d", i, L.op);
        }
    }
    int ndev = 0;
    VQ_HIP(hipGetDeviceCount(&ndev));
    VQ_REQUIRE(device >= 0 && device < ndev, "device %d out of range (%d visible)", device, ndev);
    DeviceGuard g(device);
    auto* net = new vq_tsn;
    net->device = device;
    net->max_crops = max_crops;
    net->in_channels = in_channels;
    net->input = *input;
    net->tensors.assign(tensors, tensors + n_tensors);
    net->layers.assign(layers, layers + n_layers);
    net->feature_slot = feature_slot;
    net->D = tensors[feature_slot].c;
    net->blob_floats = blob_floats;
    net->flops_per_crop = 2.0 * macs;
    for (int i = 0; i < n_layers; ++i)
        if (layers[i].op == VQ_OP_GLOBAL_AVGPOOL && layers[i].dst == feature_slot && layers[i].dst_coff == 0 && layers[i].cout == net->D)
            net->consensus_layer = i;
    hipDeviceProp_t prop;
    if (hipGetDeviceProperties(&prop, device) == hipSuccess) net->cus = prop.multiProcessorCount;
    net->slots.assign(n_tensors, nullptr);
    auto bail = [&](const char* what, hipError_t e) {
        tsn_free(net);
        delete net;
        return fail(e == hipErrorOutOfMemory ? VQ_E_NOMEM : VQ_E_HIP, "%s failed: %s", what, hipGetErrorString(e));
    };
    net->slot_bytes.assign(n_tensors, 0);
    for (int i = 0; i < n_tensors; ++i) {
        const size_t bytes = (size_t)max_crops * tensors[i].h * tensors[i].w * tensors[i].c * sizeof(float);
        hipError_t e = pool_alloc(device, bytes, (void**)&net->slots[i]);
        if (e != hipSuccess) return bail("hipMalloc(activation slot)", e);
        net->slot_bytes[i] = bytes;
    }
    net->blob_bytes = (size_t)blob_floats * sizeof(float);
    hipError_t e = pool_alloc(device, net->blob_bytes, (void**)&net->blob);
    if (e != hipSuccess) return bail("hipMalloc(weights)", e);
    e = hipMemcpy(net->blob, blob_host, (size_t)blob_floats * sizeof(float), hipMemcpyHostToDevice);
    if (e != hipSuccess) return bail("hipMemcpy(weights)", e);
    {
        net->ksplit.assign(n_layers, 1);
        const char* sk = getenv("VQ_TSN_SPLITK");
        size_t scratch = 0;
        int max_cout = 4;
        for (int i = 0; i < n_layers && !(sk && atoi(sk) == 0); ++i) {
            const vq_layer_desc& L = layers[i];
            const vq_tensor_desc& td = tensors[L.dst];
            if (L.op != VQ_OP_CONV || L.seg_count > 0 || L.pre_pool_k > 0 || L.cin % KPAD != 0 || td.h * td.w > 49) continue;
            const int steps = L.k * L.k * L.cin / KPAD;
            int ks = std::min(4, steps / 16);
            while (ks > 1 && steps % ks != 0) --ks;
            if (ks <= 1) continue;
            net->ksplit[i] = ks;
            scratch = std::max(scratch, (size_t)td.h * td.w * L.cout);
            max_cout = std::max(max_cout, L.cout);
        }
        if (scratch > 0) {
            net->split_crop_floats = scratch + (size_t)max_cout;
            net->split_slice_floats = (size_t)max_crops * net->split_crop_floats;
            e = pool_alloc(device, net->split_slice_floats * 4 * sizeof(float), (void**)&net->split_scratch);
            if (e != hipSuccess) return bail("hipMalloc(split-K scratch)", e);
            e = hipMalloc((void**)&net->zero_bias, (size_t)max_cout * sizeof(float));
            if (e != hipSuccess) return bail("hipMalloc(zero bias)", e);
            e = hipMemset(net->zero_bias, 0, (size_t)max_cout * sizeof(float));
            if (e != hipSuccess) return bail("hipMemset(zero bias)", e);
        }
    }
    {
        std::vector<ConvSeg> table;
        net->seg_table_off.assign(n_layers, 0);
        for (int i = 0; i < n_layers; ++i) {
            const vq_layer_desc& L = layers[i];
            if (L.op != VQ_OP_CONV) continue;
            net->seg_table_off[i] = (int)table.size();
            if (net->ksplit[i] > 1) {
                for (int q = 0; q < net->ksplit[i]; ++q)
                    for (int b = 0; b < (L.cout + 31) / 32; ++b)
                        table.push_back(ConvSeg{net->split_scratch + (size_t)q * net->split_slice_floats, L.cout, 0});
                continue;
            }
            if (L.seg_count > 0) {
                int col0 = 0;
                for (int q = 0; q < L.seg_count; ++q) {
                    const vq_conv_segment& sg = segments[L.seg_first + q];
                    for (int b = 0; b < sg.cout / 32; ++b)
                        table.push_back(ConvSeg{net->slots[sg.dst] + sg.dst_coff - col0, tensors[sg.dst].c, sg.relu});
                    col0 += sg.cout;
                }
            } else {
                for (int b = 0; b < (L.cout + 31) / 32; ++b)
                    table.push_back(ConvSeg{net->slots[L.dst] + L.dst_coff, tensors[L.dst].c, L.relu});
            }
        }
        e = vq::malloc_trim((void**)&net->seg_table, std::max<size_t>(table.size(), 1) * sizeof(ConvSeg));
        if (e != hipSuccess) return bail("vq::malloc_trim(destination tables)", e);
        e = hipMemcpy(net->seg_table, table.data(), table.size() * sizeof(ConvSeg), hipMemcpyHostToDevice);
        if (e != hipSuccess) return bail("hipMemcpy(destination tables)", e);
    }
    {
        if (const char* at = getenv("VQ_TSN_AUTOTUNE")) net->autotune = atoi(at) != 0;
        if (const char* gr = getenv("VQ_TSN_GROUP")) net->group_wino = atoi(gr) != 0;
        if (const char* gp = getenv("VQ_TSN_GROUP_POOL")) net->group_pool = atoi(gp) != 0;
        if (const char* po = getenv("VQ_TSN_POISON")) net->poison = atoi(po) != 0;
        if (const char* force = getenv("VQ_TSN_TILE")) {
            int bm = 0, bn = 0, bk = 32, pipe = 0;
            if (sscanf(force, "%dx%dx%dx%d", &bm, &bn, &bk, &pipe) >= 2) net->forced_tile = tile_index(bm, bn, bk, pipe);
        }
        const char* sp = getenv("VQ_TSN_SPLIT");
        if (sp && strchr(sp, ',')) {
            for (const char* q = sp; *q;) {
                net->split_parts.push_back(std::max(atoi(q), 1));
                q = strchr(q, ',');
                if (!q) break;
                ++q;
            }
            net->n_split = std::min<int>((int)net->split_parts.size(), 8);
            net->split_parts.resize(net->n_split);
        } else {
            net->n_split = std::min(std::max(sp ? atoi(sp) : 2, 1), 8);
            net->split_parts.assign(net->n_split, 1);
        }
        build_items(net, segments);
        net->split_streams.assign(net->n_split, nullptr);
        net->join_ev.assign(net->n_split, nullptr);
        for (int l = 1; l < net->n_split; ++l) {
            e = hipStreamCreateWithFlags(&net->split_streams[l], hipStreamNonBlocking);
            if (e != hipSuccess) return bail("hipStreamCreate(sub-batch)", e);
            e = hipEventCreateWithFlags(&net->join_ev[l], hipEventDisableTiming);
            if (e != hipSuccess) return bail("hipEventCreate(sub-batch join)", e);
        }
        e = hipEventCreateWithFlags(&net->fork_ev, hipEventDisableTiming);
        if (e != hipSuccess) return bail("hipEventCreate(fork)", e);
    }
    e = vq::malloc_trim((void**)&net->zeros, 256);
    if (e != hipSuccess) return bail("vq::malloc_trim(zero page)", e);
    e = hipMemset(net->zeros, 0, 256);
    if (e != hipSuccess) return bail("hipMemset(zero page)", e);
    e = vq::malloc_trim((void**)&net->mean_dev, (size_t)in_channels * sizeof(float));
    if (e != hipSuccess) return bail("vq::malloc_trim(mean)", e);
    e = vq::malloc_trim((void**)&net->feat_dev, (size_t)max_crops * net->D * sizeof(double));
    if (e != hipSuccess) return bail("vq::malloc_trim(features)", e);
    *out = net;
    return VQ_OK;
}

int vq_tsn_destroy(vq_tsn* net) {
    if (!net) return VQ_OK;
    {
        DeviceGuard g(net->device);
        (void)hipDeviceSynchronize();
        tsn_free(net);
    }
    delete net;
    return VQ_OK;
}

int vq_tsn_set_stream(vq_tsn* net, void* s) {
    VQ_REQUIRE(net, "net is NULL");
    std::lock_guard<std::mutex> lk(net->mu);
    net->stream = (hipStream_t)s;
    return VQ_OK;
}

static int forward_launches(vq_tsn* net, const uint8_t* src, int n_crops, int T, int n_split, const std::vector<int>& sub,
                            const std::vector<int>& sub_off, hipEvent_t* ev) {
    const vq_tensor_desc& t0 = net->tensors[0];
    const int in_c = net->in_channels;
    const int n_items = (int)net->items.size();
    auto preprocess = [&](int crop0, int n, hipStream_t st) -> int {
        const uint8_t* from = src + (size_t)crop0 * net->input.h * net->input.w * in_c;
        float* to = net->slots[0] + (size_t)crop0 * t0.h * t0.w * t0.c;
        if (net->input.s2d_pad < 0) {
            const int64_t nchunk = (int64_t)n * net->input.h * net->input.w * (t0.c / 4);
            preprocess_kernel<<<cdiv(nchunk, 256), 256, 0, st>>>(from, to, nchunk, in_c, t0.c, net->mean_dev);
        } else {
            const int64_t nchunk = (int64_t)n * t0.h * t0.w * in_c;
            if (in_c == 3 && t0.c == 12)
                preprocess_s2d3_kernel<<<cdiv(nchunk / 3, 256), 256, 0, st>>>(from, to, nchunk / 3, net->input.h, net->input.w, t0.h, t0.w,
                                                                               net->input.s2d_pad, net->mean_dev, net->input.s2d_order);
            else
                preprocess_s2d_kernel<<<cdiv(nchunk, 256), 256, 0, st>>>(from, to, nchunk, net->input.h, net->input.w, in_c, t0.h, t0.w,
                                                                        net->input.s2d_pad, net->mean_dev, net->input.s2d_order);
        }
        VQ_CHECK_LAUNCH();
        return VQ_OK;
    };
    if (n_split > 1) {
        VQ_HIP(hipEventRecord(net->fork_ev, net->stream));
        for (int l = 1; l < n_split; ++l) VQ_HIP(hipStreamWaitEvent(net->split_streams[l], net->fork_ev, 0));
        for (int sb = 0; sb < n_split; ++sb) {
            const int rc = preprocess(sub_off[sb], sub[sb], sb > 0 ? net->split_streams[sb] : net->stream);
            if (rc != VQ_OK) return rc;
        }
        for (const LaunchItem& it : net->items)
            for (int sb = 0; sb < n_split; ++sb) {
                net->ls = sb > 0 ? net->split_streams[sb] : net->stream;
                const int rc = run_item(net, it, sub_off[sb], sub[sb], tile_key(sub[sb], true));
                if (rc != VQ_OK) return rc;
            }
        net->ls = net->stream;
        for (int l = 1; l < n_split; ++l) {
            VQ_HIP(hipEventRecord(net->join_ev[l], net->split_streams[l]));
            VQ_HIP(hipStreamWaitEvent(net->stream, net->join_ev[l], 0));
        }
    } else {
        const int prc = preprocess(0, n_crops, net->stream);
        if (prc != VQ_OK) return prc;
        net->ls = net->stream;
        for (int q = 0; q < n_items; ++q) {
            if (ev) {
                net->ev_start = ev[2 * q];
                net->ev_stop = ev[2 * q + 1];
            }
            const int rc = run_item(net, net->items[q], 0, n_crops, tile_key(n_crops, false));
            if (rc != VQ_OK) return rc;
        }
    }
    if (ev) ++net->profile_count;
    const int B = n_crops / T;
    if (!net->fused_consensus) {
        consensus_kernel<<<cdiv((int64_t)B * net->D, 256), 256, 0, net->stream>>>(net->slots[net->feature_slot], net->feat_dev, B, T,
                                                                                  net->D, net->D);
        VQ_CHECK_LAUNCH();
    }
    return VQ_OK;
}

int vq_tsn_forward(vq_tsn* net, const uint8_t* crops, int32_t crops_on_device, int32_t n_crops, int32_t T,
                   const float* mean_host, double* feat_host, float* per_snippet_host) {
    VQ_REQUIRE(net && crops && mean_host, "NULL argument");
    VQ_REQUIRE(n_crops > 0 && n_crops <= net->max_crops, "n_crops %d outside (0,%d]", n_crops, net->max_crops);
    VQ_REQUIRE(T > 0 && n_crops % T == 0, "n_crops (%d) must be a multiple of T (%d)", n_crops, T);
    std::lock_guard<std::mutex> lk(net->mu);
    DeviceGuard g(net->device);
    const int in_c = net->in_channels;
    const int64_t npix = (int64_t)n_crops * net->input.h * net->input.w;
    const uint8_t* src = crops;
    if (!crops_on_device) {
        const size_t bytes = (size_t)npix * in_c;
        if (net->crops_cap < bytes) {
            if (net->crops_dev) VQ_HIP(hipFree(net->crops_dev));
            net->crops_dev = nullptr;
            net->crops_cap = 0;
            VQ_HIP(vq::malloc_trim((void**)&net->crops_dev, bytes));
            net->crops_cap = bytes;
        }
        VQ_HIP(hipMemcpyAsync(net->crops_dev, crops, bytes, hipMemcpyHostToDevice, net->stream));
        src = net->crops_dev;
    }
    if (net->mean_cached.size() != (size_t)in_c || memcmp(net->mean_cached.data(), mean_host, in_c * sizeof(float)) != 0) {
        net->mean_cached.assign(mean_host, mean_host + in_c);
        VQ_HIP(hipMemcpyAsync(net->mean_dev, net->mean_cached.data(), in_c * sizeof(float), hipMemcpyHostToDevice, net->stream));
        VQ_HIP(hipStreamSynchronize(net->stream));
    }
    if (net->poison)
        for (size_t i = 0; i < net->slots.size(); ++i) {
            const vq_tensor_desc& t = net->tensors[i];
            VQ_HIP(hipMemsetAsync(net->slots[i], 0xFF, (size_t)net->max_crops * t.h * t.w * t.c * sizeof(float), net->stream));
        }
    net->cur_T = T;
    const int n_items = (int)net->items.size();
    hipEvent_t* ev = nullptr;
    const bool profiling = net->profile_depth > 0;
    if (profiling && net->profile_tick++ % net->profile_every == 0)
        ev = net->events.data() + (size_t)(net->profile_count % net->profile_depth) * (2 * n_items);
    int parts_sum = 0;
    for (int v : net->split_parts) parts_sum += v;
    bool one_stream = profiling && (ev || !net->profile_split);
    if (!one_stream && !net->split_pref.empty()) {
        int best = 0, pref = 1;
        for (const auto& kv : net->split_pref)
            if (10 * std::max(kv.first, n_crops) <= 16 * std::min(kv.first, n_crops) && (best == 0 || std::abs(kv.first - n_crops) < std::abs(best - n_crops))) {
                best = kv.first;
                pref = kv.second;
            }
        if (pref == 0) one_stream = true;
    }
    int n_split = (!one_stream && net->n_split > 1 && n_crops % parts_sum == 0) ? net->n_split : 1;
    std::vector<int> sub(n_split, n_crops), sub_off(n_split, 0);
    if (n_split > 1) {
        for (int sb = 0, o = 0; sb < n_split; ++sb) {
            sub[sb] = n_crops / parts_sum * net->split_parts[sb];
            sub_off[sb] = o;
            o += sub[sb];
        }
    }
    {
        bool whole = net->consensus_layer >= 0 && T <= kMaxFusedT;
        if (whole) {
            const int cap = net->items[net->item_of_layer[net->consensus_layer]].max_crops;
            for (int sb = 0; sb < n_split; ++sb)
                if (sub[sb] % T != 0 || sub_off[sb] % T != 0 || (sub[sb] > cap && cap % T != 0)) whole = false;
        }
        net->fused_consensus = whole;
    }
    for (int sb = 0; sb < n_split; ++sb) {
        const int rc = ensure_tuned(net, sub[sb], n_split > 1);
        if (rc != VQ_OK) return rc;
    }
    const int frc = forward_launches(net, src, n_crops, T, n_split, sub, sub_off, ev);
    if (frc != VQ_OK) return frc;
    net->last_crops = n_crops;
    const int B = n_crops / T;
    if (feat_host)
        VQ_HIP(hipMemcpyAsync(feat_host, net->feat_dev, (size_t)B * net->D * sizeof(double), hipMemcpyDeviceToHost, net->stream));
    if (per_snippet_host)
        VQ_HIP(hipMemcpyAsync(per_snippet_host, net->slots[net->feature_slot], (size_t)n_crops * net->D * sizeof(float),
                              hipMemcpyDeviceToHost, net->stream));
    if (feat_host || per_snippet_host || !crops_on_device) VQ_HIP(hipStreamSynchronize(net->stream));
    return VQ_OK;
}

int vq_tsn_feat_devptr(vq_tsn* net, void** feat_dev, void** per_snippet_dev) {
    VQ_REQUIRE(net, "net is NULL");
    if (feat_dev) *feat_dev = net->feat_dev;
    if (per_snippet_dev) *per_snippet_dev = net->slots[net->feature_slot];
    return VQ_OK;
}

int vq_tsn_read_tensor(vq_tsn* net, int32_t slot, int32_t n_crops, float* host) {
    VQ_REQUIRE(net && host, "NULL argument");
    VQ_REQUIRE(slot >= 0 && slot < (int)net->tensors.size(), "slot out of range");
    VQ_REQUIRE(n_crops > 0 && n_crops <= net->max_crops, "n_crops out of range");
    std::lock_guard<std::mutex> lk(net->mu);
    DeviceGuard g(net->device);
    const vq_tensor_desc& t = net->tensors[slot];
    VQ_HIP(hipMemcpyAsync(host, net->slots[slot], (size_t)n_crops * t.h * t.w * t.c * sizeof(float), hipMemcpyDeviceToHost,
                          net->stream));
    VQ_HIP(hipStreamSynchronize(net->stream));
    return VQ_OK;
}

int vq_tsn_set_profile(vq_tsn* net, int32_t depth) {
    VQ_REQUIRE(net, "net is NULL");
    VQ_REQUIRE(depth >= 0 && depth <= 1024, "profile depth must be in [0,1024]");
    std::lock_guard<std::mutex> lk(net->mu);
    DeviceGuard g(net->device);
    VQ_HIP(hipStreamSynchronize(net->stream));
    for (hipEvent_t e : net->events) (void)hipEventDestroy(e);
    net->events.clear();
    net->events.resize((size_t)depth * 2 * net->items.size());
    for (hipEvent_t& e : net->events) VQ_HIP(hipEventCreate(&e));
    net->profile_depth = depth;
    net->profile_count = 0;
    net->profile_tick = 0;
    return VQ_OK;
}

int vq_tsn_set_profile_every(vq_tsn* net, int32_t every) {
    VQ_REQUIRE(net && every >= 1, "every must be >= 1");
    std::lock_guard<std::mutex> lk(net->mu);
    net->profile_every = every;
    net->profile_tick = 0;
    return VQ_OK;
}

static double wino_weight(const vq_tsn* net, int li) {
    const vq_layer_desc& L = net->layers[li];
    const vq_tensor_desc& td = net->tensors[L.dst];
    if (!is_wino(L.op)) {
        const vq_tensor_desc& ts = net->tensors[L.src];
        return ((double)ts.h * ts.w + (double)td.h * td.w) * L.cin * 4.0 / 4e12;
    }
    return 2.0 * 16.0 * ((td.h + 1) / 2) * ((td.w + 1) / 2) * (double)L.cin * L.cout / 100e12;
}

int vq_tsn_set_profile_split(vq_tsn* net, int32_t unsampled_split) {
    VQ_REQUIRE(net, "net is NULL");
    std::lock_guard<std::mutex> lk(net->mu);
    net->profile_split = unsampled_split != 0;
    return VQ_OK;
}

int vq_tsn_layer_times(vq_tsn* net, float* ms, double* flops, int32_t n_layers) {
    VQ_REQUIRE(net && ms, "NULL argument");
    VQ_REQUIRE(n_layers == (int)net->layers.size(), "n_layers must be %d", (int)net->layers.size());
    std::lock_guard<std::mutex> lk(net->mu);
    if (net->profile_depth == 0 || net->profile_count == 0) return fail(VQ_E_STATE, "no profiled forward has run");
    DeviceGuard g(net->device);
    VQ_HIP(hipStreamSynchronize(net->stream));
    const int sets = std::min(net->profile_count, net->profile_depth);
    const int n_items = (int)net->items.size();
    for (int i = 0; i < n_layers; ++i) ms[i] = 0.f;
    for (int sidx = 0; sidx < sets; ++sidx) {
        hipEvent_t* ev = net->events.data() + (size_t)sidx * (2 * n_items);
        for (int q = 0; q < n_items; ++q) {
            float t = 0.f;
            VQ_HIP(hipEventElapsedTime(&t, ev[2 * q], ev[2 * q + 1]));
            const LaunchItem& it = net->items[q];
            double wsum = 0;
            for (int m : it.layers) wsum += it.kind == 1 ? wino_weight(net, m) : 1.0;
            for (int m : it.layers)
                ms[m] += (float)(t / sets * ((it.kind == 1 ? wino_weight(net, m) : 1.0) / wsum));
        }
    }
    if (flops) {
        for (int i = 0; i < n_layers; ++i) {
            const vq_layer_desc& L = net->layers[i];
            const vq_tensor_desc& td = net->tensors[L.dst];
            flops[i] = is_conv(L.op) ? 2.0 * net->last_crops * td.h * td.w * L.cout * first_layer_k2c(net->input, L)
                                          : 0.0;
        }
    }
    return VQ_OK;
}

int vq_tsn_launch_items(vq_tsn* net, int32_t* item_of_layer, int32_t n_layers, int32_t* n_items) {
    VQ_REQUIRE(net && item_of_layer && n_items, "NULL argument");
    VQ_REQUIRE(n_layers == (int)net->layers.size(), "n_layers must be %d", (int)net->layers.size());
    for (int i = 0; i < n_layers; ++i) item_of_layer[i] = net->item_of_layer[i];
    *n_items = (int)net->items.size();
    return VQ_OK;
}

int vq_tsn_tuned_sizes(vq_tsn* net, int32_t* sizes, int32_t cap, int32_t* n) {
    VQ_REQUIRE(net && n && (cap == 0 || sizes), "NULL argument");
    std::lock_guard<std::mutex> lk(net->mu);
    std::set<int> distinct;
    for (const auto& kv : net->tuned) distinct.insert(kv.first >= kPairedKey ? kv.first - kPairedKey : kv.first);
    int k = 0;
    for (int v : distinct) {
        if (k < cap) sizes[k] = v;
        ++k;
    }
    *n = k;
    return VQ_OK;
}

int vq_device_pool_trim(void) {
    vq::device_pool_trim();
    return VQ_OK;
}

int vq_tsn_set_split(vq_tsn* net, int32_t n_crops, int32_t split) {
    VQ_REQUIRE(net && n_crops > 0, "bad argument");
    std::lock_guard<std::mutex> lk(net->mu);
    if (split < 0)
        net->split_pref.erase(n_crops);
    else
        net->split_pref[n_crops] = split ? 1 : 0;
    return VQ_OK;
}

int vq_tsn_tune(vq_tsn* net, int32_t n_crops, int32_t paired) {
    VQ_REQUIRE(net, "net is NULL");
    VQ_REQUIRE(n_crops > 0 && n_crops * (paired ? std::min(net->n_split, 2) : 1) <= net->max_crops, "n_crops out of range");
    std::lock_guard<std::mutex> lk(net->mu);
    DeviceGuard g(net->device);
    const int rc = autotune(net, n_crops, paired != 0);
    if (rc != VQ_OK) net->tuned.erase(tile_key(n_crops, paired != 0));
    VQ_HIP(hipStreamSynchronize(net->stream));
    return rc;
}

int vq_tsn_tile_tables(vq_tsn* net, int32_t* sizes, int32_t* flags, int32_t cap, int32_t* n) {
    VQ_REQUIRE(net && n && (cap == 0 || (sizes && flags)), "NULL argument");
    std::lock_guard<std::mutex> lk(net->mu);
    int k = 0;
    for (const auto& kv : net->tuned) {
        if (k < cap) {
            const bool paired = kv.first >= kPairedKey;
            sizes[k] = paired ? kv.first - kPairedKey : kv.first;
            flags[k] = (paired ? 1 : 0) | (net->tuned_borrowed.count(kv.first) ? 2 : 0);
        }
        ++k;
    }
    *n = k;
    return VQ_OK;
}

int vq_tsn_get_tiles(vq_tsn* net, int32_t n_crops, int32_t paired, int32_t* tiles, int32_t n_layers) {
    VQ_REQUIRE(net && tiles, "NULL argument");
    VQ_REQUIRE(n_layers == (int)net->layers.size(), "n_layers must be %d", (int)net->layers.size());
    std::lock_guard<std::mutex> lk(net->mu);
    auto it = net->tuned.find(tile_key(n_crops, paired != 0));
    for (int i = 0; i < n_layers; ++i) {
        tiles[4 * i] = tiles[4 * i + 1] = tiles[4 * i + 2] = tiles[4 * i + 3] = 0;
        if (is_wino(net->layers[i].op)) {
            const int lead = net->items[net->item_of_layer[i]].layers[0];
            const int v = it != net->tuned.end() ? it->second[lead] : 0;
            tiles[4 * i] = v >= 2 ? 64 : 128;
            tiles[4 * i + 1] = 32 * ((v & 1) + 1);
            tiles[4 * i + 2] = v >= 2 ? 16 : 8;
            tiles[4 * i + 3] = 2;
            continue;
        }
        if (net->layers[i].op != VQ_OP_CONV) continue;
        const int t = it != net->tuned.end() ? it->second[i] : heuristic_tile(net, i, n_crops);
        tiles[4 * i] = kTiles[t].bm;
        tiles[4 * i + 1] = kTiles[t].bn;
        tiles[4 * i + 2] = kTiles[t].bk;
        tiles[4 * i + 3] = kTiles[t].pipe;
    }
    return VQ_OK;
}

int vq_tsn_layer_tiles(vq_tsn* net, int32_t n_crops, int32_t* tiles, int32_t n_layers) {
    VQ_REQUIRE(net, "NULL argument");
    bool paired = false;
    {
        std::lock_guard<std::mutex> lk(net->mu);
        paired = net->tuned.find(tile_key(n_crops, false)) == net->tuned.end() && net->tuned.find(tile_key(n_crops, true)) != net->tuned.end();
    }
    return vq_tsn_get_tiles(net, n_crops, paired ? 1 : 0, tiles, n_layers);
}

int vq_tsn_set_tiles(vq_tsn* net, int32_t n_crops, int32_t paired, const int32_t* tiles, int32_t n_layers) {
    VQ_REQUIRE(net && tiles, "NULL argument");
    VQ_REQUIRE(n_layers == (int)net->layers.size(), "n_layers must be %d", (int)net->layers.size());
    VQ_REQUIRE(n_crops > 0 && n_crops <= net->max_crops, "n_crops out of range");
    std::vector<int> choice(net->layers.size(), 0);
    for (int i = 0; i < n_layers; ++i) {
        if (is_wino(net->layers[i].op)) {
            const int bn = tiles[4 * i + 1], bk = tiles[4 * i + 2];
            const bool t16 = tiles[4 * i] == 64 && bk == 16;
            VQ_REQUIRE(tiles[4 * i + 3] == 2 && (bn == 32 || bn == 64) && (t16 || (tiles[4 * i] == 128 && bk == 8)) &&
                           (!t16 || net->layers[i].op == VQ_OP_CONV_WINOGRAD16),
                       "layer %d: no Winograd variant for tile %dx%dx%d", i, tiles[4 * i], bn, bk);
            choice[i] = bn / 32 - 1 + (t16 ? 2 : 0);
            continue;
        }
        if (net->layers[i].op != VQ_OP_CONV) continue;
        const int found = tile_index(tiles[4 * i], tiles[4 * i + 1], tiles[4 * i + 2], tiles[4 * i + 3]);
        VQ_REQUIRE(found >= 0, "layer %d: no kernel for tile %dx%dx%d pipe=%d", i, tiles[4 * i], tiles[4 * i + 1], tiles[4 * i + 2],
                   tiles[4 * i + 3]);
        choice[i] = found;
    }
    std::lock_guard<std::mutex> lk(net->mu);
    const int key = tile_key(n_crops, paired != 0);
    net->tuned[key] = choice;
    net->tuned_borrowed.erase(key);
    return VQ_OK;
}

int vq_tsn_set_layer_tiles(vq_tsn* net, int32_t n_crops, const int32_t* tiles, int32_t n_layers) {
    int rc = vq_tsn_set_tiles(net, n_crops, 0, tiles, n_layers);
    if (rc != VQ_OK) return rc;
    int parts_sum = 0;
    for (int v : net->split_parts) parts_sum += v;
    if (net->n_split > 1 && parts_sum > 0 && n_crops % parts_sum == 0)
        for (int v : net->split_parts) {
            rc = vq_tsn_set_tiles(net, n_crops / parts_sum * v, 1, tiles, n_layers);
            if (rc != VQ_OK) return rc;
        }
    return VQ_OK;
}

int vq_tsn_flops_per_crop(vq_tsn* net, double* flops) {
    VQ_REQUIRE(net && flops, "NULL argument");
    *flops = net->flops_per_crop;
    return VQ_OK;
}

}
```

video-query-algorithms_amd/csrc/vq_tsn_kernels.h:

```cpp
#pragma once
#include <hip/hip_runtime.h>
#include <hip/hip_ext.h>

namespace vq {

__device__ __forceinline__ int xcd_remap(int bid, int nwg) {
    const int q = nwg >> 3, r = nwg & 7, xcd = bid & 7, idx = bid >> 3;
    return (xcd < r ? xcd * (q + 1) : r * (q + 1) + (xcd - r) * q) + idx;
}

__device__ __forceinline__ unsigned magic_div(unsigned x, unsigned m) { return m ? __umulhi(x, m) : x; }

struct FullDiv {
    unsigned m, sh1, sh2;
};
__device__ __forceinline__ unsigned full_div(unsigned x, const FullDiv& d) {
    const unsigned t = __umulhi(d.m, x);
    return (t + ((x - t) >> d.sh1)) >> d.sh2;
}
static inline FullDiv full_div_for(unsigned d) {
    unsigned l = 0;
    while ((1ull << l) < d) ++l;
    FullDiv f;
    f.m = (unsigned)(((1ull << 32) * ((1ull << l) - d)) / d + 1);
    f.sh1 = l < 1 ? l : 1;
    f.sh2 = l > 1 ? l - 1 : 0;
    return f;
}
constexpr int kRecipShift = 22;
__device__ __forceinline__ unsigned umul24(unsigned x, unsigned y_uniform) {
    unsigned r;
    asm("v_mul_u32_u24 %0, %2, %1" : "=v"(r) : "v"(x), "s"(y_uniform));
    return r;
}
__device__ __forceinline__ int imul24(int x, int y_uniform) {
    int r;
    asm("v_mul_i32_i24 %0, %2, %1" : "=v"(r) : "v"(x), "s"(y_uniform));
    return r;
}
static inline unsigned recip22(unsigned d) { return (1u << kRecipShift) / d + 1u; }
static inline bool recip22_ok(unsigned d, unsigned xmax) {
    return d >= 1 && (unsigned long long)xmax * d < (1ull << kRecipShift) && (unsigned long long)xmax * recip22(d) < (1ull << 32);
}

struct PoolArgs {
    const float* in;
    float* out;
    int H, W, Cs_in, coff_in, C;
    int Ho, Wo, Cs_out, coff_out;
    int k, stride, pad;
    int is_max;
    int64_t total;
    const float* bias;
    int relu;
    int unit0, n_units;
};
constexpr int kPoolPerWG = 1024;

template <bool IS_MAX>
__device__ __forceinline__ void pool_one(const PoolArgs& a, int64_t i) {
    const int c4n = a.C >> 2;
    const int c4 = (int)(i % c4n);
    int64_t pix = i / c4n;
    const int pw = (int)(pix % a.Wo);
    pix /= a.Wo;
    const int ph = (int)(pix % a.Ho);
    const int64_t n = pix / a.Ho;
    int hs = ph * a.stride - a.pad, ws = pw * a.stride - a.pad;
    int he = min(hs + a.k, a.H + a.pad), we = min(ws + a.k, a.W + a.pad);
    const float pool_size = (float)((he - hs) * (we - ws));
    hs = max(hs, 0);
    ws = max(ws, 0);
    he = min(he, a.H);
    we = min(we, a.W);
    const float* base = a.in + (size_t)n * a.H * a.W * a.Cs_in + a.coff_in + c4 * 4;
    float4 acc = IS_MAX ? make_float4(-INFINITY, -INFINITY, -INFINITY, -INFINITY) : make_float4(0.f, 0.f, 0.f, 0.f);
    for (int h = hs; h < he; ++h)
        for (int w = ws; w < we; ++w) {
            const float4 v = *reinterpret_cast<const float4*>(base + ((size_t)h * a.W + w) * a.Cs_in);
            if (IS_MAX) {
                acc.x = fmaxf(acc.x, v.x);
                acc.y = fmaxf(acc.y, v.y);
                acc.z = fmaxf(acc.z, v.z);
                acc.w = fmaxf(acc.w, v.w);
            } else {
                acc.x += v.x;
                acc.y += v.y;
                acc.z += v.z;
                acc.w += v.w;
            }
        }
    if (!IS_MAX) {
        acc.x /= pool_size;
        acc.y /= pool_size;
        acc.z /= pool_size;
        acc.w /= pool_size;
        if (a.bias) {
            const float4 b = *reinterpret_cast<const float4*>(a.bias + c4 * 4);
            acc.x += b.x;
            acc.y += b.y;
            acc.z += b.z;
            acc.w += b.w;
        }
        if (a.relu) {
            acc.x = fmaxf(acc.x, 0.f);
            acc.y = fmaxf(acc.y, 0.f);
            acc.z = fmaxf(acc.z, 0.f);
            acc.w = fmaxf(acc.w, 0.f);
        }
    }
    float* o = a.out + (((size_t)n * a.Ho + ph) * a.Wo + pw) * a.Cs_out + a.coff_out + c4 * 4;
    *reinterpret_cast<float4*>(o) = acc;
}

struct WinoJob {
    const float* in;
    const float* u;
    const float* bias;
    float* out;
    int H, W, Cs_in, coff_in, Cin;
    int Cs_out, coff_out, Cout;
    int th, tw, P;
    int relu;
    int t16;
    int tiles_n;
    int unit0, n_units;
    unsigned in_bytes, u_bytes, out_bytes;
    unsigned m_tiles_n, m_tpi, m_tw;
    unsigned s_tw, s_th;
#ifdef VQ_WINO_PHASES
    long long* phases;
#endif
};

constexpr int kWinoMaxJobs = 4;
constexpr int kWinoMaxPools = 2;
struct WinoGroup {
    int n_jobs;
    int n_pools;
    int total_units;
    int pool_unit0;
    WinoJob job[kWinoMaxJobs];
    PoolArgs pool[kWinoMaxPools];
};

constexpr int kWinoVariants = 2;

int launch_wino_group(WinoGroup& g, int variant, hipStream_t stream, hipEvent_t ev_start, hipEvent_t ev_stop);

#define VQ_LAUNCH(KERN, GRID, BLOCK, LDS, STREAM, EV_START, EV_STOP, ...)                                     \
    do {                                                                                                      \
        if ((EV_START) || (EV_STOP))                                                                          \
            hipExtLaunchKernelGGL(KERN, dim3(GRID), dim3(BLOCK), (std::uint32_t)(LDS), STREAM, EV_START, EV_STOP, 0, __VA_ARGS__); \
        else                                                                                                  \
            KERN<<<GRID, BLOCK, LDS, STREAM>>>(__VA_ARGS__);                                                  \
    } while (0)

}
```

video-query-algorithms_amd/csrc/vq_wino.hip:

```cpp
#include "vq_common.h"
#include "vq_tsn_kernels.h"

using namespace vq;

typedef float floatx16 __attribute__((ext_vector_type(16)));
typedef float floatx4 __attribute__((ext_vector_type(4)));
typedef float floatx2 __attribute__((ext_vector_type(2)));
typedef unsigned uintx4 __attribute__((__vector_size__(4 * sizeof(unsigned))));

namespace {

__device__ __forceinline__ floatx2 pk_add2(floatx2 x, floatx2 y) {
    floatx2 r;
    asm("v_pk_add_f32 %0, %1, %2" : "=v"(r) : "v"(x), "v"(y));
    return r;
}
__device__ __forceinline__ floatx2 pk_sub2(floatx2 x, floatx2 y) {
    floatx2 r;
    asm("v_pk_add_f32 %0, %1, %2 neg_lo:[0,1] neg_hi:[0,1]" : "=v"(r) : "v"(x), "v"(y));
    return r;
}
__device__ __forceinline__ floatx4 pk_add(floatx4 x, floatx4 y) {
    const floatx2 lo = pk_add2(x.xy, y.xy), hi = pk_add2(x.zw, y.zw);
    return (floatx4){lo.x, lo.y, hi.x, hi.y};
}
__device__ __forceinline__ floatx4 pk_sub(floatx4 x, floatx4 y) {
    const floatx2 lo = pk_sub2(x.xy, y.xy), hi = pk_sub2(x.zw, y.zw);
    return (floatx4){lo.x, lo.y, hi.x, hi.y};
}
__device__ __forceinline__ floatx4 pk_fma(floatx4 x, floatx2 s, floatx4 z) {
    const floatx2 lo = __builtin_elementwise_fma(x.xy, s, z.xy), hi = __builtin_elementwise_fma(x.zw, s, z.zw);
    return (floatx4){lo.x, lo.y, hi.x, hi.y};
}

__device__ __forceinline__ float relu1(float x) {
    float r;
    asm("v_max_f32 %0, 0, %1" : "=v"(r) : "v"(x));
    return r;
}

#ifdef VQ_WINO_PHASES
#define VQ_PHASE(K)                                                                                               \
    if (threadIdx.x == 0) {                                                                                       \
        a.phases[(size_t)blockIdx.x * 6 + (K)] = (long long)__builtin_readcyclecounter();                         \
        if ((K) == 0) {                                                                                           \
            a.phases[(size_t)blockIdx.x * 6 + 4] = __builtin_amdgcn_s_getreg((31 << 11) | 4);           \
            a.phases[(size_t)blockIdx.x * 6 + 5] = __builtin_amdgcn_s_getreg((31 << 11) | 20);        \
        }                                                                                                         \
    }
#else
#define VQ_PHASE(K)
#endif

constexpr int BP = 32;
constexpr int KC = 8;
constexpr int HS_STAGE = 4 * 4 * BP * KC;
constexpr int EP_ROW = 36;
constexpr int EP_FLOATS = 2 * 4 * BP * EP_ROW;
constexpr int LDS_FLOATS = EP_FLOATS > 2 * HS_STAGE ? EP_FLOATS : 2 * HS_STAGE;

struct TileAt {
    int img, ty, tx;
};
__device__ __forceinline__ TileAt tile_at(int t, int img0, int ty0, int tx0, int th, int tw, unsigned s_th, unsigned s_tw) {
    const unsigned lin = (unsigned)(tx0 + t);
    const unsigned q1 = umul24(lin, s_tw) >> kRecipShift;
    const unsigned ly = (unsigned)ty0 + q1;
    const unsigned q2 = umul24(ly, s_th) >> kRecipShift;
    return TileAt{img0 + (int)q2, (int)(ly - umul24(q2, (unsigned)th)), (int)(lin - umul24(q1, (unsigned)tw))};
}

template <int NB>
__device__ __forceinline__ void wino_unit(const WinoJob& a, int unit, float* hs) {
    VQ_PHASE(0)
    const int tid = threadIdx.x;
    const int lane = tid & 63, l31 = lane & 31, half = lane >> 5;
    const int wave = __builtin_amdgcn_readfirstlane(tid >> 6);
    const int tile = xcd_remap(unit, a.n_units);
    const int pb = (int)magic_div((unsigned)tile, a.m_tiles_n);
    const int p0 = pb * BP;
    const int n0 = (tile - pb * a.tiles_n) * (32 * NB);
    const int tpi = a.th * a.tw;
    const int img0 = (int)magic_div((unsigned)p0, a.m_tpi);
    const int rem0 = p0 - img0 * tpi;
    const int ty0 = (int)magic_div((unsigned)rem0, a.m_tw);
    const int tx0 = rem0 - ty0 * a.tw;

    const __amdgpu_buffer_rsrc_t in_rsrc = __builtin_amdgcn_make_buffer_rsrc(const_cast<float*>(a.in), 0, a.in_bytes, 0x00020000);
    const __amdgpu_buffer_rsrc_t u_rsrc = __builtin_amdgcn_make_buffer_rsrc(const_cast<float*>(a.u), 0, a.u_bytes, 0x00020000);

    unsigned poff[4];
    {
        const int t = lane >> 1, c4 = lane & 1;
        const TileAt ta = tile_at(t, img0, ty0, tx0, a.th, a.tw, a.s_th, a.s_tw);
        const int y = 2 * ta.ty - 1 + wave, x0 = 2 * ta.tx - 1;
        const bool row_ok = p0 + t < a.P && (unsigned)y < (unsigned)a.H;
        const int base = (imul24(imul24(ta.img * a.H + y, a.W) + x0, a.Cs_in) + a.coff_in + c4 * 4) * 4;
        const int px = a.Cs_in * 4;
#pragma unroll
        for (int c = 0; c < 4; ++c)
            poff[c] = (row_ok && (unsigned)(x0 + c) < (unsigned)a.W) ? (unsigned)(base + c * px) : 0xFFFFFFFFu;
    }
    const int hs_store = (wave * 4 * BP * KC) + lane * 4;

    const int ra = wave == 0 ? 0 : (wave == 2 ? 2 : 1);
    const int rb = wave == 3 ? 3 : (wave == 2 ? 1 : 2);
    const float sgn = wave == 1 ? 1.0f : -1.0f;
    const floatx2 sgn2 = {sgn, sgn};
    const int fa_off = ra * 4 * BP * KC + l31 * KC + half * 4;
    const int fb_off = rb * 4 * BP * KC + l31 * KC + half * 4;
    unsigned uvoff[NB];
#pragma unroll
    for (int nb = 0; nb < NB; ++nb) uvoff[nb] = (n0 + 32 * nb < a.Cout) ? (unsigned)((l31 * 8 + half * 4) * 4) : 0xFFFFFFFFu;
    const unsigned u_step = (unsigned)(16 * a.Cout * 8 * 4);
    const unsigned u_wave = (unsigned)(((wave * 4) * a.Cout + n0) * 8 * 4);
    const unsigned u_pos = (unsigned)(a.Cout * 8 * 4);

    floatx16 acc[4][NB];
#pragma unroll
    for (int j = 0; j < 4; ++j)
#pragma unroll
        for (int nb = 0; nb < NB; ++nb)
#pragma unroll
            for (int e = 0; e < 16; ++e) acc[j][nb][e] = 0.f;
    if (wave == 1) {
        const __amdgpu_buffer_rsrc_t b_rsrc = __builtin_amdgcn_make_buffer_rsrc(const_cast<float*>(a.bias), 0, (unsigned)a.Cout * 4u, 0x00020000);
#pragma unroll
        for (int nb = 0; nb < NB; ++nb)
#pragma unroll
            for (int g = 0; g < 4; ++g) {
                const floatx4 bv = __builtin_bit_cast(floatx4, __builtin_amdgcn_raw_buffer_load_b128(
                                                                   b_rsrc, (unsigned)((n0 + 32 * nb + 8 * g + 4 * half) * 4), 0, 0));
#pragma unroll
                for (int r = 0; r < 4; ++r) acc[1][nb][4 * g + r] = bv[r];
            }
    }

    constexpr int G = NB == 1 ? 2 : 1, NGRP = 4 / G;
    floatx4 d[4];
    floatx4 bq[4][NB];

#define VQ_W_LOAD_PATCH(KSTEP)                                                                                  \
    _Pragma("unroll") for (int c = 0; c < 4; ++c)                                                               \
        d[c] = __builtin_bit_cast(floatx4, __builtin_amdgcn_raw_buffer_load_b128(in_rsrc, poff[c], (KSTEP) * (KC * 4), 0));
#define VQ_W_LOAD_U(KSTEP, J)                                                                                   \
    _Pragma("unroll") for (int nb = 0; nb < NB; ++nb)                                                           \
        bq[J][nb] = __builtin_bit_cast(floatx4, __builtin_amdgcn_raw_buffer_load_b128(                          \
            u_rsrc, uvoff[nb], (KSTEP) * u_step + u_wave + (J) * u_pos + nb * (32 * 8 * 4), 0));
#define VQ_W_STORE_H(ST)                                                                                        \
    {                                                                                                           \
        float* dst = hs + (ST) * HS_STAGE + hs_store;                                                           \
        *reinterpret_cast<floatx4*>(dst + 0 * BP * KC) = pk_sub(d[0], d[2]);                                    \
        *reinterpret_cast<floatx4*>(dst + 1 * BP * KC) = pk_add(d[1], d[2]);                                    \
        *reinterpret_cast<floatx4*>(dst + 2 * BP * KC) = pk_sub(d[2], d[1]);                                    \
        *reinterpret_cast<floatx4*>(dst + 3 * BP * KC) = pk_sub(d[1], d[3]);                                    \
    }
#define VQ_W_READ_A(ST, GRP, SET)                                                                               \
    _Pragma("unroll") for (int q = 0; q < G; ++q) {                                                             \
        a0[SET][q] = *reinterpret_cast<const floatx4*>(hs + (ST) * HS_STAGE + fa_off + (G * (GRP) + q) * BP * KC); \
        a1[SET][q] = *reinterpret_cast<const floatx4*>(hs + (ST) * HS_STAGE + fb_off + (G * (GRP) + q) * BP * KC); \
    }
#define VQ_W_STEP(ST, KSTEP, NEXT)                                                                              \
    {                                                                                                           \
        floatx4 a0[2][G], a1[2][G];                                                                             \
        VQ_W_READ_A(ST, 0, 0)                                                                                   \
        _Pragma("unroll") for (int g = 0; g < NGRP; ++g) {                                                      \
            if (g + 1 < NGRP) VQ_W_READ_A(ST, g + 1, (g + 1) & 1)                                               \
            floatx4 av[G];                                                                                      \
            _Pragma("unroll") for (int q = 0; q < G; ++q)                                                       \
                av[q] = pk_fma(a1[g & 1][q], sgn2, a0[g & 1][q]);                                                  \
            _Pragma("unroll") for (int e = 0; e < 4; ++e)                                                       \
                _Pragma("unroll") for (int q = 0; q < G; ++q)                                                   \
                    _Pragma("unroll") for (int nb = 0; nb < NB; ++nb)                                           \
                        acc[G * g + q][nb] = __builtin_amdgcn_mfma_f32_32x32x2f32(bq[G * g + q][nb][e], av[q][e], acc[G * g + q][nb], 0, 0, 0); \
            if (NEXT) {                                                                                         \
                _Pragma("unroll") for (int q = 0; q < G; ++q) VQ_W_LOAD_U((KSTEP) + 1, G * g + q)               \
            }                                                                                                   \
            __builtin_amdgcn_sched_barrier(0);                                                                  \
        }                                                                                                       \
    }

    const int nk = a.Cin / KC;
    VQ_W_LOAD_PATCH(0)
#pragma unroll
    for (int j = 0; j < 4; ++j) VQ_W_LOAD_U(0, j)
    VQ_W_STORE_H(0)
    __syncthreads();
    VQ_PHASE(1)
    int kc = 0;
    for (; kc + 1 < nk; ++kc) {
        const int st = kc & 1;
        VQ_W_LOAD_PATCH(kc + 1)
        __builtin_amdgcn_sched_barrier(0);
        VQ_W_STEP(st, kc, true)
        VQ_W_STORE_H(st ^ 1)
        __syncthreads();
    }
    VQ_W_STEP(kc & 1, kc, false)
    VQ_PHASE(2)
#undef VQ_W_LOAD_PATCH
#undef VQ_W_LOAD_U
#undef VQ_W_STORE_H
#undef VQ_W_STEP
#undef VQ_W_READ_A

    const int et = tid >> 3, ec = tid & 7;
    const TileAt te = tile_at(et, img0, ty0, tx0, a.th, a.tw, a.s_th, a.s_tw);
    const __amdgpu_buffer_rsrc_t out_rsrc = __builtin_amdgcn_make_buffer_rsrc(a.out, 0, a.out_bytes, 0x00020000);
    const int oy = 2 * te.ty, ox = 2 * te.tx;
    const int obase = (imul24(imul24(te.img * a.H + oy, a.W) + ox, a.Cs_out) + a.coff_out + n0 + ec * 4) * 4;
    const bool tile_ok = p0 + et < a.P;
    unsigned ooff[4];
#pragma unroll
    for (int u = 0; u < 4; ++u)
        ooff[u] = (tile_ok && oy + (u >> 1) < a.H && ox + (u & 1) < a.W) ? (unsigned)(obase + ((u >> 1) * a.W + (u & 1)) * a.Cs_out * 4)
                                                                           : 0xFFFFFFFFu;
    float* ep_w = hs + ((wave * 2) * BP + l31) * EP_ROW + 4 * half;
    const float* ep_r = hs + et * EP_ROW + ec * 4;
    __syncthreads();
#pragma unroll
    for (int nb = 0; nb < NB; ++nb) {
#pragma unroll
        for (int g = 0; g < 4; ++g) {
            floatx4 t0, t1;
#pragma unroll
            for (int h2 = 0; h2 < 2; ++h2) {
                const int e = 4 * g + 2 * h2;
                const floatx2 m0 = {acc[0][nb][e], acc[0][nb][e + 1]}, m1 = {acc[1][nb][e], acc[1][nb][e + 1]};
                const floatx2 m2 = {acc[2][nb][e], acc[2][nb][e + 1]}, m3 = {acc[3][nb][e], acc[3][nb][e + 1]};
                const floatx2 s0 = pk_add2(pk_add2(m0, m1), m2), s1 = pk_sub2(pk_sub2(m1, m2), m3);
                t0[2 * h2] = s0.x;
                t0[2 * h2 + 1] = s0.y;
                t1[2 * h2] = s1.x;
                t1[2 * h2 + 1] = s1.y;
            }
            *reinterpret_cast<floatx4*>(ep_w + 8 * g) = t0;
            *reinterpret_cast<floatx4*>(ep_w + BP * EP_ROW + 8 * g) = t1;
        }
        __syncthreads();
#pragma unroll
        for (int b_ = 0; b_ < 2; ++b_) {
            const floatx4 v0 = *reinterpret_cast<const floatx4*>(ep_r + (0 * 2 + b_) * BP * EP_ROW);
            const floatx4 v1 = *reinterpret_cast<const floatx4*>(ep_r + (1 * 2 + b_) * BP * EP_ROW);
            const floatx4 v2 = *reinterpret_cast<const floatx4*>(ep_r + (2 * 2 + b_) * BP * EP_ROW);
            const floatx4 v3 = *reinterpret_cast<const floatx4*>(ep_r + (3 * 2 + b_) * BP * EP_ROW);
            floatx4 y0 = pk_add(pk_add(v0, v1), v2);
            floatx4 y1 = pk_sub(pk_sub(v1, v2), v3);
            if (a.relu) {
#pragma unroll
                for (int r = 0; r < 4; ++r) {
                    y0[r] = relu1(y0[r]);
                    y1[r] = relu1(y1[r]);
                }
            }
            const bool blk_ok = n0 + 32 * nb < a.Cout;
            __builtin_amdgcn_raw_buffer_store_b128(__builtin_bit_cast(uintx4, y0), out_rsrc, blk_ok ? ooff[b_] : 0xFFFFFFFFu, nb * (32 * 4), 0);
            __builtin_amdgcn_raw_buffer_store_b128(__builtin_bit_cast(uintx4, y1), out_rsrc, blk_ok ? ooff[2 + b_] : 0xFFFFFFFFu, nb * (32 * 4), 0);
        }
        if (nb + 1 < NB) __syncthreads();
    }
    VQ_PHASE(3)
}

constexpr int BP16 = 16;
constexpr int KC16 = 16;
constexpr int HS16_STAGE = 4 * 4 * BP16 * KC16;
constexpr int EP16_FLOATS = 2 * 4 * BP16 * EP_ROW;
constexpr int LDS16_FLOATS = EP16_FLOATS > 2 * HS16_STAGE ? EP16_FLOATS : 2 * HS16_STAGE;

template <int NB>
__device__ __forceinline__ void wino16_unit(const WinoJob& a, int unit, float* hs) {
    constexpr int NBLK = 2 * NB;
    const int tid = threadIdx.x;
    const int lane = tid & 63, l15 = lane & 15, kq = lane >> 4;
    const int wave = __builtin_amdgcn_readfirstlane(tid >> 6);
    const int tile = xcd_remap(unit, a.n_units);
    const int pb = (int)magic_div((unsigned)tile, a.m_tiles_n);
    const int p0 = pb * BP16;
    const int n0 = (tile - pb * a.tiles_n) * (32 * NB);
    const int tpi = a.th * a.tw;
    const int img0 = (int)magic_div((unsigned)p0, a.m_tpi);
    const int rem0 = p0 - img0 * tpi;
    const int ty0 = (int)magic_div((unsigned)rem0, a.m_tw);
    const int tx0 = rem0 - ty0 * a.tw;

    const __amdgpu_buffer_rsrc_t in_rsrc = __builtin_amdgcn_make_buffer_rsrc(const_cast<float*>(a.in), 0, a.in_bytes, 0x00020000);
    const __amdgpu_buffer_rsrc_t u_rsrc = __builtin_amdgcn_make_buffer_rsrc(const_cast<float*>(a.u), 0, a.u_bytes, 0x00020000);

    unsigned poff[4];
    const int lq = lane & 3;
    {
        const int t = lane >> 2;
        const TileAt ta = tile_at(t, img0, ty0, tx0, a.th, a.tw, a.s_th, a.s_tw);
        const int y = 2 * ta.ty - 1 + wave, x0 = 2 * ta.tx - 1;
        const bool row_ok = p0 + t < a.P && (unsigned)y < (unsigned)a.H;
        const int base = (imul24(imul24(ta.img * a.H + y, a.W) + x0, a.Cs_in) + a.coff_in + lq * 4) * 4;
        const int px = a.Cs_in * 4;
#pragma unroll
        for (int c = 0; c < 4; ++c)
            poff[c] = (row_ok && (unsigned)(x0 + c) < (unsigned)a.W) ? (unsigned)(base + c * px) : 0xFFFFFFFFu;
    }
    const int slot_a = ((lq & 1) << 2) | (lq & 2);
    const int hs_store = (wave * 4 * BP16 + (lane >> 2)) * KC16 + slot_a;

    const int ra = wave == 0 ? 0 : (wave == 2 ? 2 : 1);
    const int rb = wave == 3 ? 3 : (wave == 2 ? 1 : 2);
    const float sgn = wave == 1 ? 1.0f : -1.0f;
    const floatx2 sgn2 = {sgn, sgn};
    const int fa_off = (ra * 4 * BP16 + l15) * KC16 + kq * 4;
    const int fb_off = (rb * 4 * BP16 + l15) * KC16 + kq * 4;
    unsigned uvoff[NBLK];
#pragma unroll
    for (int b = 0; b < NBLK; ++b) uvoff[b] = (n0 + 16 * b < a.Cout) ? (unsigned)(((16 * b + l15) * 16 + kq * 4) * 4) : 0xFFFFFFFFu;
    const unsigned u_step = (unsigned)(16 * a.Cout * 16 * 4);
    const unsigned u_wave = (unsigned)(((wave * 4) * a.Cout + n0) * 16 * 4);
    const unsigned u_pos = (unsigned)(a.Cout * 16 * 4);

    floatx4 acc[4][NBLK];
#pragma unroll
    for (int j = 0; j < 4; ++j)
#pragma unroll
        for (int b = 0; b < NBLK; ++b) acc[j][b] = (floatx4){0.f, 0.f, 0.f, 0.f};
    if (wave == 1) {
        const __amdgpu_buffer_rsrc_t b_rsrc = __builtin_amdgcn_make_buffer_rsrc(const_cast<float*>(a.bias), 0, (unsigned)a.Cout * 4u, 0x00020000);
#pragma unroll
        for (int b = 0; b < NBLK; ++b)
            acc[1][b] = __builtin_bit_cast(floatx4, __builtin_amdgcn_raw_buffer_load_b128(b_rsrc, (unsigned)((n0 + 16 * b + 4 * kq) * 4), 0, 0));
    }

    floatx4 d[4];
    floatx4 bq[4][NBLK];

#define VQ_W16_LOAD_PATCH(KSTEP)                                                                                \
    _Pragma("unroll") for (int c = 0; c < 4; ++c)                                                               \
        d[c] = __builtin_bit_cast(floatx4, __builtin_amdgcn_raw_buffer_load_b128(in_rsrc, poff[c], (KSTEP) * (KC16 * 4), 0));
#define VQ_W16_LOAD_U(KSTEP, J)                                                                                 \
    _Pragma("unroll") for (int b = 0; b < NBLK; ++b)                                                            \
        bq[J][b] = __builtin_bit_cast(floatx4, __builtin_amdgcn_raw_buffer_load_b128(                           \
            u_rsrc, uvoff[b], (KSTEP) * u_step + u_wave + (J) * u_pos, 0));
#define VQ_W16_PUT(J, V)                                                                                        \
    {                                                                                                           \
        const floatx4 v_ = (V);                                                                                 \
        *reinterpret_cast<floatx2*>(dst + (J) * BP16 * KC16) = (floatx2){v_.x, v_.z};                           \
        *reinterpret_cast<floatx2*>(dst + (J) * BP16 * KC16 + 8) = (floatx2){v_.y, v_.w};                       \
    }
#define VQ_W16_STORE_H(ST)                                                                                      \
    {                                                                                                           \
        float* dst = hs + (ST) * HS16_STAGE + hs_store;                                                         \
        VQ_W16_PUT(0, pk_sub(d[0], d[2]))                                                                       \
        VQ_W16_PUT(1, pk_add(d[1], d[2]))                                                                       \
        VQ_W16_PUT(2, pk_sub(d[2], d[1]))                                                                       \
        VQ_W16_PUT(3, pk_sub(d[1], d[3]))                                                                       \
    }
#define VQ_W16_READ_A(ST, GRP, SET)                                                                             \
    _Pragma("unroll") for (int q = 0; q < 2; ++q) {                                                             \
        a0[SET][q] = *reinterpret_cast<const floatx4*>(hs + (ST) * HS16_STAGE + fa_off + (2 * (GRP) + q) * BP16 * KC16); \
        a1[SET][q] = *reinterpret_cast<const floatx4*>(hs + (ST) * HS16_STAGE + fb_off + (2 * (GRP) + q) * BP16 * KC16); \
    }
#define VQ_W16_STEP(ST, KSTEP, NEXT)                                                                            \
    {                                                                                                           \
        floatx4 a0[2][2], a1[2][2];                                                                             \
        VQ_W16_READ_A(ST, 0, 0)                                                                                 \
        _Pragma("unroll") for (int g2 = 0; g2 < 2; ++g2) {                                                      \
            if (g2 + 1 < 2) VQ_W16_READ_A(ST, g2 + 1, (g2 + 1) & 1)                                             \
            floatx4 av[2];                                                                                      \
            _Pragma("unroll") for (int q = 0; q < 2; ++q)                                                       \
                av[q] = pk_fma(a1[g2 & 1][q], sgn2, a0[g2 & 1][q]);                                             \
            _Pragma("unroll") for (int e = 0; e < 4; ++e)                                                       \
                _Pragma("unroll") for (int q = 0; q < 2; ++q)                                                   \
                    _Pragma("unroll") for (int b = 0; b < NBLK; ++b)                                            \
                        acc[2 * g2 + q][b] = __builtin_amdgcn_mfma_f32_16x16x4f32(bq[2 * g2 + q][b][e], av[q][e], acc[2 * g2 + q][b], 0, 0, 0); \
            if (NEXT) {                                                                                         \
                _Pragma("unroll") for (int q = 0; q < 2; ++q) VQ_W16_LOAD_U((KSTEP) + 1, 2 * g2 + q)            \
            }                                                                                                   \
            __builtin_amdgcn_sched_barrier(0);                                                                  \
        }                                                                                                       \
    }

    const int nk = a.Cin / KC16;
    VQ_W16_LOAD_PATCH(0)
#pragma unroll
    for (int j = 0; j < 4; ++j) VQ_W16_LOAD_U(0, j)
    VQ_W16_STORE_H(0)
    __syncthreads();
    int kc = 0;
    for (; kc + 1 < nk; ++kc) {
        const int st = kc & 1;
        VQ_W16_LOAD_PATCH(kc + 1)
        __builtin_amdgcn_sched_barrier(0);
        VQ_W16_STEP(st, kc, true)
        VQ_W16_STORE_H(st ^ 1)
        __syncthreads();
    }
    VQ_W16_STEP(kc & 1, kc, false)
#undef VQ_W16_LOAD_PATCH
#undef VQ_W16_LOAD_U
#undef VQ_W16_PUT
#undef VQ_W16_STORE_H
#undef VQ_W16_STEP
#undef VQ_W16_READ_A

    const int et = (tid >> 3) & 15, ec = tid & 7, bsel = tid >> 7;
    const TileAt te = tile_at(et, img0, ty0, tx0, a.th, a.tw, a.s_th, a.s_tw);
    const __amdgpu_buffer_rsrc_t out_rsrc = __builtin_amdgcn_make_buffer_rsrc(a.out, 0, a.out_bytes, 0x00020000);
    const int oy = 2 * te.ty, ox = 2 * te.tx;
    const int obase = (imul24(imul24(te.img * a.H + oy, a.W) + ox, a.Cs_out) + a.coff_out + n0 + ec * 4) * 4;
    const bool tile_ok = p0 + et < a.P;
    unsigned ooff[2];
#pragma unroll
    for (int u = 0; u < 2; ++u)
        ooff[u] = (tile_ok && oy + u < a.H && ox + bsel < a.W) ? (unsigned)(obase + (u * a.W + bsel) * a.Cs_out * 4) : 0xFFFFFFFFu;
    float* ep_w = hs + ((wave * 2) * BP16 + l15) * EP_ROW + 4 * kq;
    const float* ep_r = hs + et * EP_ROW + ec * 4;
    __syncthreads();
#pragma unroll
    for (int nb = 0; nb < NB; ++nb) {
#pragma unroll
        for (int bb = 0; bb < 2; ++bb) {
            const int b = 2 * nb + bb;
            floatx4 t0, t1;
#pragma unroll
            for (int h2 = 0; h2 < 2; ++h2) {
                const floatx2 m0 = {acc[0][b][2 * h2], acc[0][b][2 * h2 + 1]}, m1 = {acc[1][b][2 * h2], acc[1][b][2 * h2 + 1]};
                const floatx2 m2 = {acc[2][b][2 * h2], acc[2][b][2 * h2 + 1]}, m3 = {acc[3][b][2 * h2], acc[3][b][2 * h2 + 1]};
                const floatx2 s0 = pk_add2(pk_add2(m0, m1), m2), s1 = pk_sub2(pk_sub2(m1, m2), m3);
                t0[2 * h2] = s0.x;
                t0[2 * h2 + 1] = s0.y;
                t1[2 * h2] = s1.x;
                t1[2 * h2 + 1] = s1.y;
            }
            *reinterpret_cast<floatx4*>(ep_w + 16 * bb) = t0;
            *reinterpret_cast<floatx4*>(ep_w + BP16 * EP_ROW + 16 * bb) = t1;
        }
        __syncthreads();
        {
            const floatx4 v0 = *reinterpret_cast<const floatx4*>(ep_r + (0 * 2 + bsel) * BP16 * EP_ROW);
            const floatx4 v1 = *reinterpret_cast<const floatx4*>(ep_r + (1 * 2 + bsel) * BP16 * EP_ROW);
            const floatx4 v2 = *reinterpret_cast<const floatx4*>(ep_r + (2 * 2 + bsel) * BP16 * EP_ROW);
            const floatx4 v3 = *reinterpret_cast<const floatx4*>(ep_r + (3 * 2 + bsel) * BP16 * EP_ROW);
            floatx4 y0 = pk_add(pk_add(v0, v1), v2);
            floatx4 y1 = pk_sub(pk_sub(v1, v2), v3);
            if (a.relu) {
#pragma unroll
                for (int r = 0; r < 4; ++r) {
                    y0[r] = relu1(y0[r]);
                    y1[r] = relu1(y1[r]);
                }
            }
            const bool blk_ok = n0 + 32 * nb < a.Cout;
            __builtin_amdgcn_raw_buffer_store_b128(__builtin_bit_cast(uintx4, y0), out_rsrc, blk_ok ? ooff[0] : 0xFFFFFFFFu, nb * (32 * 4), 0);
            __builtin_amdgcn_raw_buffer_store_b128(__builtin_bit_cast(uintx4, y1), out_rsrc, blk_ok ? ooff[1] : 0xFFFFFFFFu, nb * (32 * 4), 0);
        }
        if (nb + 1 < NB) __syncthreads();
    }
}

template <int NB, int TB>
__global__ __launch_bounds__(256) __attribute__((amdgpu_waves_per_eu(NB == 1 ? 4 : 2, NB == 1 ? 4 : 2)))
void wino_f2x2_3x3_kernel(WinoGroup g) {
    extern __shared__ __attribute__((aligned(16))) char smem_raw[];
    float* hs = reinterpret_cast<float*>(smem_raw);
    const int b = blockIdx.x;
    if (b >= g.pool_unit0) {
        int q = 0;
        if (g.n_pools > 1 && b >= g.pool[1].unit0) q = 1;
        const PoolArgs& pa = g.pool[q];
        const int unit = b - pa.unit0;
        if (unit >= pa.n_units) return;
#pragma unroll
        for (int r = 0; r < kPoolPerWG / 256; ++r) {
            const int64_t i = (int64_t)unit * kPoolPerWG + r * 256 + threadIdx.x;
            if (i < pa.total) {
                if (pa.is_max)
                    pool_one<true>(pa, i);
                else
                    pool_one<false>(pa, i);
            }
        }
        return;
    }
    int j = 0;
#pragma unroll
    for (int q = 1; q < kWinoMaxJobs; ++q)
        if (q < g.n_jobs && b >= g.job[q].unit0) j = q;
    const WinoJob& a = g.job[j];
    const int unit = b - a.unit0;
    if (unit >= a.n_units) return;
    if constexpr (TB == 16)
        wino16_unit<NB>(a, unit, hs);
    else
        wino_unit<NB>(a, unit, hs);
}

unsigned magic_u32(unsigned d) { return d == 1 ? 0u : (unsigned)(0x100000000ull / d) + 1u; }

template <int NB, int TB>
int launch_t(WinoGroup& g, hipStream_t stream, hipEvent_t ev_start, hipEvent_t ev_stop) {
    int units = 0;
    for (int q = 0; q < g.n_jobs; ++q) {
        WinoJob& a = g.job[q];
        a.tiles_n = cdiv(a.Cout, 32 * NB);
        const long long n = (long long)cdiv(a.P, TB) * a.tiles_n;
        VQ_REQUIRE(n > 0 && n < (1 << 24), "Winograd job %d: %lld workgroups", q, n);
        a.unit0 = units;
        a.n_units = (int)n;
        units += ((int)n + 7) & ~7;
        const unsigned tpi = (unsigned)(a.th * a.tw);
        VQ_REQUIRE((unsigned long long)n * a.tiles_n < 0x100000000ull && (unsigned long long)(a.P + BP) * tpi < 0x100000000ull &&
                       recip22_ok((unsigned)a.tw, (unsigned)a.tw + BP) && recip22_ok((unsigned)a.th, (unsigned)a.th + BP + 2),
                   "Winograd job %d: shape outside the reciprocal-division range", q);
        VQ_REQUIRE((unsigned long long)cdiv(a.P, (int)tpi) * a.H * a.W < (1ull << 23) && a.Cs_in < (1 << 23) && a.Cs_out < (1 << 23),
                   "Winograd job %d: more than 2^23 pixels in a slot (split the batch)", q);
        a.m_tiles_n = magic_u32((unsigned)a.tiles_n);
        a.m_tpi = magic_u32(tpi);
        a.m_tw = magic_u32((unsigned)a.tw);
        a.s_tw = recip22((unsigned)a.tw);
        a.s_th = recip22((unsigned)a.th);
    }
    g.pool_unit0 = units;
    for (int q = 0; q < g.n_pools; ++q) {
        PoolArgs& pa = g.pool[q];
        const long long n = (pa.total + kPoolPerWG - 1) / kPoolPerWG;
        VQ_REQUIRE(n > 0 && n < (1 << 24), "pooling job %d: %lld workgroups", q, n);
        pa.unit0 = units;
        pa.n_units = (int)n;
        units += (int)n;
    }
    g.total_units = units;
    auto kern = wino_f2x2_3x3_kernel<NB, TB>;
    const size_t lds = (TB == 16 ? LDS16_FLOATS : LDS_FLOATS) * sizeof(float);
    VQ_LAUNCH(kern, units, 256, lds, stream, ev_start, ev_stop, g);
    VQ_CHECK_LAUNCH();
    return VQ_OK;
}

}

namespace vq {

int launch_wino_group(WinoGroup& g, int variant, hipStream_t stream, hipEvent_t ev_start, hipEvent_t ev_stop) {
    VQ_REQUIRE(g.n_jobs >= 1 && g.n_jobs <= kWinoMaxJobs, "a Winograd launch carries 1..%d jobs", kWinoMaxJobs);
    VQ_REQUIRE(g.n_pools >= 0 && g.n_pools <= kWinoMaxPools, "a Winograd launch carries at most %d pooling layers", kWinoMaxPools);
    for (int q = 0; q < g.n_jobs; ++q) {
        const WinoJob& a = g.job[q];
        VQ_REQUIRE(a.Cin % KC == 0 && a.Cout % 32 == 0 && a.Cs_out % 4 == 0 && a.coff_out % 4 == 0 && a.Cs_in % 4 == 0 && a.coff_in % 4 == 0,
                   "Winograd convolution needs Cin %% 8 == 0, Cout %% 32 == 0 and 16-byte aligned channel offsets");
        VQ_REQUIRE(a.in_bytes <= 0x7FFFFFF0u && a.out_bytes <= 0x7FFFFFF0u,
                   "Winograd convolution: a launch addresses its slots with signed 32-bit byte offsets (split the batch)");
    }
    VQ_REQUIRE((variant >= 2) == (g.job[0].t16 != 0), "Winograd variant %d on the other filter layout", variant);
    if (variant == 0) return launch_t<1, 32>(g, stream, ev_start, ev_stop);
    if (variant == 1) return launch_t<2, 32>(g, stream, ev_start, ev_stop);
    if (variant == 2) return launch_t<1, 16>(g, stream, ev_start, ev_stop);
    if (variant == 3) return launch_t<2, 16>(g, stream, ev_start, ev_stop);
    return fail(VQ_E_INVALID, "no Winograd kernel variant %d", variant);
}

}
```

Before: 12820 clips/s.

## Make Winograd kernel persistent, walking units and prefetching next unit during epilogue

The Winograd conv kernel becomes persistent. It launches only as many workgroups as can be resident, computed from an occupancy query times the CU count, and each workgroup strides through its units. While storing the current unit's epilogue it opens the next unit: index math, buffer descriptors, the first patch and filter loads, and accumulator and bias initialisation. This is meant to cut workgroup launch and ramp-up cost and hide load latency behind the output stores. In exchange it adds register pressure, extra syncs and a static unit schedule that can leave load imbalanced across workgroups.

```diff
diff --git a/video-query-algorithms_amd/csrc/vq_tsn.hip b/video-query-algorithms_amd/csrc/vq_tsn.hip
--- a/video-query-algorithms_amd/csrc/vq_tsn.hip
+++ b/video-query-algorithms_amd/csrc/vq_tsn.hip
@@ -867,6 +867,7 @@
     bool autotune = true;
     bool group_wino = true;
     bool group_pool = true;
+    int wino_slots[2 * kWinoVariants] = {0, 0, 0, 0};
     bool poison = false;
     int forced_tile = -1;
     std::vector<float*> slots;
@@ -1240,6 +1241,7 @@
         variant -= 2;
         for (int q = 0; q < g.n_jobs; ++q) VQ_REQUIRE(!g.job[q].t16, "internal: mixed Winograd layouts in one launch");
     }
+    g.walk_slots = variant >= 0 && variant < 2 * kWinoVariants ? net->wino_slots[variant] : 0;
     return launch_wino_group(g, variant, net->ls, net->ev_start, net->ev_stop);
 }
 
@@ -1768,6 +1770,9 @@
         if (const char* gr = getenv("VQ_TSN_GROUP")) net->group_wino = atoi(gr) != 0;
         if (const char* gp = getenv("VQ_TSN_GROUP_POOL")) net->group_pool = atoi(gp) != 0;
         if (const char* po = getenv("VQ_TSN_POISON")) net->poison = atoi(po) != 0;
+        const char* ww = getenv("VQ_WINO_WALK");
+        if (!ww || atoi(ww) != 0)
+            for (int v = 0; v < 2 * kWinoVariants; ++v) net->wino_slots[v] = wino_resident_workgroups(v, net->cus);
         if (const char* force = getenv("VQ_TSN_TILE")) {
             int bm = 0, bn = 0, bk = 32, pipe = 0;
             if (sscanf(force, "%dx%dx%dx%d", &bm, &bn, &bk, &pipe) >= 2) net->forced_tile = tile_index(bm, bn, bk, pipe);
diff --git a/video-query-algorithms_amd/csrc/vq_tsn_kernels.h b/video-query-algorithms_amd/csrc/vq_tsn_kernels.h
--- a/video-query-algorithms_amd/csrc/vq_tsn_kernels.h
+++ b/video-query-algorithms_amd/csrc/vq_tsn_kernels.h
@@ -140,6 +140,8 @@
     int n_pools;
     int total_units;
     int pool_unit0;
+    int walk_slots;
+    int walk_wgs;
     WinoJob job[kWinoMaxJobs];
     PoolArgs pool[kWinoMaxPools];
 };
@@ -147,6 +149,7 @@
 constexpr int kWinoVariants = 2;
 
 int launch_wino_group(WinoGroup& g, int variant, hipStream_t stream, hipEvent_t ev_start, hipEvent_t ev_stop);
+int wino_resident_workgroups(int variant, int cus);
 
 #define VQ_LAUNCH(KERN, GRID, BLOCK, LDS, STREAM, EV_START, EV_STOP, ...)                                     \
     do {                                                                                                      \
diff --git a/video-query-algorithms_amd/csrc/vq_wino.hip b/video-query-algorithms_amd/csrc/vq_wino.hip
--- a/video-query-algorithms_amd/csrc/vq_wino.hip
+++ b/video-query-algorithms_amd/csrc/vq_wino.hip
@@ -39,13 +39,18 @@
     return r;
 }
 
+__device__ __forceinline__ int fresh(int x) {
+    asm volatile("" : "+v"(x));
+    return x;
+}
+
 #ifdef VQ_WINO_PHASES
 #define VQ_PHASE(K)                                                                                               \
     if (threadIdx.x == 0) {                                                                                       \
-        a.phases[(size_t)blockIdx.x * 6 + (K)] = (long long)__builtin_readcyclecounter();                         \
+        ph_[(size_t)v * 6 + (K)] = (long long)__builtin_readcyclecounter();            \
         if ((K) == 0) {                                                                                           \
-            a.phases[(size_t)blockIdx.x * 6 + 4] = __builtin_amdgcn_s_getreg((31 << 11) | 4);           \
-            a.phases[(size_t)blockIdx.x * 6 + 5] = __builtin_amdgcn_s_getreg((31 << 11) | 20);        \
+            ph_[(size_t)v * 6 + 4] = __builtin_amdgcn_s_getreg((31 << 11) | 4);                         \
+            ph_[(size_t)v * 6 + 5] = __builtin_amdgcn_s_getreg((31 << 11) | 20);                       \
         }                                                                                                         \
     }
 #else
@@ -70,72 +75,66 @@
     return TileAt{img0 + (int)q2, (int)(ly - umul24(q2, (unsigned)th)), (int)(lin - umul24(q1, (unsigned)tw))};
 }
 
+__device__ __forceinline__ int walk_find(const WinoGroup& g, int v, int stride, int& job) {
+    while (v < g.pool_unit0) {
+        int j = 0;
+#pragma unroll
+        for (int q = 1; q < kWinoMaxJobs; ++q)
+            if (q < g.n_jobs && v >= g.job[q].unit0) j = q;
+        if (v - g.job[j].unit0 < g.job[j].n_units) {
+            job = j;
+            return v;
+        }
+        v += stride;
+    }
+    return -1;
+}
+
+struct UnitAt {
+    int p0, n0, img0, ty0, tx0;
+};
+template <int TILES, int NB>
+__device__ __forceinline__ UnitAt unit_at(const WinoJob& a, int unit) {
+    const int tile = xcd_remap(unit, a.n_units);
+    const int pb = (int)magic_div((unsigned)tile, a.m_tiles_n);
+    UnitAt u;
+    u.p0 = pb * TILES;
+    u.n0 = (tile - pb * a.tiles_n) * (32 * NB);
+    u.img0 = (int)magic_div((unsigned)u.p0, a.m_tpi);
+    const int rem0 = u.p0 - u.img0 * (a.th * a.tw);
+    u.ty0 = (int)magic_div((unsigned)rem0, a.m_tw);
+    u.tx0 = rem0 - u.ty0 * a.tw;
+    return u;
+}
+
 template <int NB>
-__device__ __forceinline__ void wino_unit(const WinoJob& a, int unit, float* hs) {
-    VQ_PHASE(0)
+__device__ __forceinline__ void wino_walk(const WinoGroup& g, int v, const int stride, float* hs) {
     const int tid = threadIdx.x;
     const int lane = tid & 63, l31 = lane & 31, half = lane >> 5;
     const int wave = __builtin_amdgcn_readfirstlane(tid >> 6);
-    const int tile = xcd_remap(unit, a.n_units);
-    const int pb = (int)magic_div((unsigned)tile, a.m_tiles_n);
-    const int p0 = pb * BP;
-    const int n0 = (tile - pb * a.tiles_n) * (32 * NB);
-    const int tpi = a.th * a.tw;
-    const int img0 = (int)magic_div((unsigned)p0, a.m_tpi);
-    const int rem0 = p0 - img0 * tpi;
-    const int ty0 = (int)magic_div((unsigned)rem0, a.m_tw);
-    const int tx0 = rem0 - ty0 * a.tw;
-
-    const __amdgpu_buffer_rsrc_t in_rsrc = __builtin_amdgcn_make_buffer_rsrc(const_cast<float*>(a.in), 0, a.in_bytes, 0x00020000);
-    const __amdgpu_buffer_rsrc_t u_rsrc = __builtin_amdgcn_make_buffer_rsrc(const_cast<float*>(a.u), 0, a.u_bytes, 0x00020000);
-
-    unsigned poff[4];
-    {
-        const int t = lane >> 1, c4 = lane & 1;
-        const TileAt ta = tile_at(t, img0, ty0, tx0, a.th, a.tw, a.s_th, a.s_tw);
-        const int y = 2 * ta.ty - 1 + wave, x0 = 2 * ta.tx - 1;
-        const bool row_ok = p0 + t < a.P && (unsigned)y < (unsigned)a.H;
-        const int base = (imul24(imul24(ta.img * a.H + y, a.W) + x0, a.Cs_in) + a.coff_in + c4 * 4) * 4;
-        const int px = a.Cs_in * 4;
-#pragma unroll
-        for (int c = 0; c < 4; ++c)
-            poff[c] = (row_ok && (unsigned)(x0 + c) < (unsigned)a.W) ? (unsigned)(base + c * px) : 0xFFFFFFFFu;
-    }
+    int job;
+    v = walk_find(g, v, stride, job);
+    if (v < 0) return;
+#ifdef VQ_WINO_PHASES
+    long long* const ph_ = g.job[job].phases;
+#endif
+    VQ_PHASE(0)
+
     const int hs_store = (wave * 4 * BP * KC) + lane * 4;
-
     const int ra = wave == 0 ? 0 : (wave == 2 ? 2 : 1);
     const int rb = wave == 3 ? 3 : (wave == 2 ? 1 : 2);
     const float sgn = wave == 1 ? 1.0f : -1.0f;
     const floatx2 sgn2 = {sgn, sgn};
     const int fa_off = ra * 4 * BP * KC + l31 * KC + half * 4;
     const int fb_off = rb * 4 * BP * KC + l31 * KC + half * 4;
+
+    UnitAt at;
+    __amdgpu_buffer_rsrc_t in_rsrc, u_rsrc;
+    unsigned poff[4];
     unsigned uvoff[NB];
-#pragma unroll
-    for (int nb = 0; nb < NB; ++nb) uvoff[nb] = (n0 + 32 * nb < a.Cout) ? (unsigned)((l31 * 8 + half * 4) * 4) : 0xFFFFFFFFu;
-    const unsigned u_step = (unsigned)(16 * a.Cout * 8 * 4);
-    const unsigned u_wave = (unsigned)(((wave * 4) * a.Cout + n0) * 8 * 4);
-    const unsigned u_pos = (unsigned)(a.Cout * 8 * 4);
-
+    unsigned u_step, u_wave, u_pos;
+    int nk;
     floatx16 acc[4][NB];
-#pragma unroll
-    for (int j = 0; j < 4; ++j)
-#pragma unroll
-        for (int nb = 0; nb < NB; ++nb)
-#pragma unroll
-            for (int e = 0; e < 16; ++e) acc[j][nb][e] = 0.f;
-    if (wave == 1) {
-        const __amdgpu_buffer_rsrc_t b_rsrc = __builtin_amdgcn_make_buffer_rsrc(const_cast<float*>(a.bias), 0, (unsigned)a.Cout * 4u, 0x00020000);
-#pragma unroll
-        for (int nb = 0; nb < NB; ++nb)
-#pragma unroll
-            for (int g = 0; g < 4; ++g) {
-                const floatx4 bv = __builtin_bit_cast(floatx4, __builtin_amdgcn_raw_buffer_load_b128(
-                                                                   b_rsrc, (unsigned)((n0 + 32 * nb + 8 * g + 4 * half) * 4), 0, 0));
-#pragma unroll
-                for (int r = 0; r < 4; ++r) acc[1][nb][4 * g + r] = bv[r];
-            }
-    }
-
     constexpr int G = NB == 1 ? 2 : 1, NGRP = 4 / G;
     floatx4 d[4];
     floatx4 bq[4][NB];
@@ -180,86 +179,152 @@
         }                                                                                                       \
     }
 
-    const int nk = a.Cin / KC;
-    VQ_W_LOAD_PATCH(0)
-#pragma unroll
-    for (int j = 0; j < 4; ++j) VQ_W_LOAD_U(0, j)
-    VQ_W_STORE_H(0)
-    __syncthreads();
-    VQ_PHASE(1)
-    int kc = 0;
-    for (; kc + 1 < nk; ++kc) {
-        const int st = kc & 1;
-        VQ_W_LOAD_PATCH(kc + 1)
+#define VQ_W_OPEN(A, V)                                                                                            \
+    {                                                                                                           \
+        at = unit_at<BP, NB>(A, (V) - (A).unit0);                                                               \
+        in_rsrc = __builtin_amdgcn_make_buffer_rsrc(const_cast<float*>((A).in), 0, (A).in_bytes, 0x00020000);     \
+        u_rsrc = __builtin_amdgcn_make_buffer_rsrc(const_cast<float*>((A).u), 0, (A).u_bytes, 0x00020000);        \
+        const int tid_o = fresh(tid), lane = tid_o & 63, l31 = lane & 31, half = lane >> 5;                     \
+        const int t = lane >> 1, c4 = lane & 1;                                                                 \
+        const TileAt ta = tile_at(t, at.img0, at.ty0, at.tx0, (A).th, (A).tw, (A).s_th, (A).s_tw);                  \
+        const int y = 2 * ta.ty - 1 + wave, x0 = 2 * ta.tx - 1;                                                 \
+        const bool row_ok = at.p0 + t < (A).P && (unsigned)y < (unsigned)(A).H;                                   \
+        const int base = (imul24(imul24(ta.img * (A).H + y, (A).W) + x0, (A).Cs_in) + (A).coff_in + c4 * 4) * 4;    \
+        const int px = (A).Cs_in * 4;                                                                            \
+        _Pragma("unroll") for (int c = 0; c < 4; ++c)                                                           \
+            poff[c] = (row_ok && (unsigned)(x0 + c) < (unsigned)(A).W) ? (unsigned)(base + c * px) : 0xFFFFFFFFu; \
+        _Pragma("unroll") for (int nb = 0; nb < NB; ++nb)                                                       \
+            uvoff[nb] = (at.n0 + 32 * nb < (A).Cout) ? (unsigned)((l31 * 8 + half * 4) * 4) : 0xFFFFFFFFu;       \
+        u_step = (unsigned)(16 * (A).Cout * 8 * 4);               \
+        u_wave = (unsigned)(((wave * 4) * (A).Cout + at.n0) * 8 * 4);                                            \
+        u_pos = (unsigned)((A).Cout * 8 * 4);                                        \
+        nk = (A).Cin / KC;                                                                                       \
+        VQ_W_LOAD_PATCH(0)                                                                                      \
+        _Pragma("unroll") for (int j = 0; j < 4; ++j) VQ_W_LOAD_U(0, j)                                         \
+    }
+#define VQ_W_ACC0(A)                                                                                              \
+    {                                                                                                           \
+        _Pragma("unroll") for (int j = 0; j < 4; ++j)                                                           \
+            _Pragma("unroll") for (int nb = 0; nb < NB; ++nb)                                                   \
+                _Pragma("unroll") for (int e = 0; e < 16; ++e) acc[j][nb][e] = 0.f;                             \
+        if (wave == 1) {                                                                                        \
+            const int half = (fresh(tid) >> 5) & 1;                                                             \
+            const __amdgpu_buffer_rsrc_t b_rsrc =                                                               \
+                __builtin_amdgcn_make_buffer_rsrc(const_cast<float*>((A).bias), 0, (unsigned)(A).Cout * 4u, 0x00020000); \
+            _Pragma("unroll") for (int nb = 0; nb < NB; ++nb)                                                   \
+                _Pragma("unroll") for (int g4 = 0; g4 < 4; ++g4) {                                              \
+                    const floatx4 bv = __builtin_bit_cast(floatx4, __builtin_amdgcn_raw_buffer_load_b128(       \
+                                                                       b_rsrc, (unsigned)((at.n0 + 32 * nb + 8 * g4 + 4 * half) * 4), 0, 0)); \
+                    _Pragma("unroll") for (int r = 0; r < 4; ++r) acc[1][nb][4 * g4 + r] = bv[r];               \
+                }                                                                                               \
+        }                                                                                                       \
+    }
+
+    VQ_W_OPEN(g.job[job], v)
+    VQ_W_ACC0(g.job[job])
+    for (;;) {
+        const WinoJob& a = g.job[job];
+        VQ_W_STORE_H(0)
+        __syncthreads();
+        VQ_PHASE(1)
+        int kc = 0;
+        for (; kc + 1 < nk; ++kc) {
+            const int st = kc & 1;
+            VQ_W_LOAD_PATCH(kc + 1)
+            __builtin_amdgcn_sched_barrier(0);
+            VQ_W_STEP(st, kc, true)
+            VQ_W_STORE_H(st ^ 1)
+            __syncthreads();
+        }
+        VQ_W_STEP(kc & 1, kc, false)
+        VQ_PHASE(2)
+
+        const int tid_e = fresh(tid), l31 = tid_e & 31, half = (tid_e >> 5) & 1;
+        const int et = tid_e >> 3, ec = tid_e & 7;
+        float* ep_w = hs + ((wave * 2) * BP + l31) * EP_ROW + 4 * half;
+        const float* ep_r = hs + et * EP_ROW + ec * 4;
+        const TileAt te = tile_at(et, at.img0, at.ty0, at.tx0, a.th, a.tw, a.s_th, a.s_tw);
+        const __amdgpu_buffer_rsrc_t out_rsrc = __builtin_amdgcn_make_buffer_rsrc(a.out, 0, a.out_bytes, 0x00020000);
+        const int oy = 2 * te.ty, ox = 2 * te.tx;
+        const int obase = (imul24(imul24(te.img * a.H + oy, a.W) + ox, a.Cs_out) + a.coff_out + at.n0 + ec * 4) * 4;
+        const bool tile_ok = at.p0 + et < a.P;
+        unsigned ooff[4];
+#pragma unroll
+        for (int u = 0; u < 4; ++u)
+            ooff[u] = (tile_ok && oy + (u >> 1) < a.H && ox + (u & 1) < a.W) ? (unsigned)(obase + ((u >> 1) * a.W + (u & 1)) * a.Cs_out * 4)
+                                                                                 : 0xFFFFFFFFu;
+#pragma unroll
+        for (int u = 0; u < 4; ++u) ooff[u] = (unsigned)fresh((int)ooff[u]);
+        const int relu = a.relu;
+        const int blocks_ok = (a.Cout - at.n0 + 31) >> 5;
+
+        constexpr bool kEarly = NB > 1;
+        int jn = 0;
+        const int vn = walk_find(g, v + stride, stride, jn);
+        if (kEarly && vn >= 0) VQ_W_OPEN(g.job[jn], vn)
         __builtin_amdgcn_sched_barrier(0);
-        VQ_W_STEP(st, kc, true)
-        VQ_W_STORE_H(st ^ 1)
         __syncthreads();
-    }
-    VQ_W_STEP(kc & 1, kc, false)
-    VQ_PHASE(2)
+#pragma unroll
+        for (int nb = 0; nb < NB; ++nb) {
+#pragma unroll
+            for (int g4 = 0; g4 < 4; ++g4) {
+                floatx4 t0, t1;
+#pragma unroll
+                for (int h2 = 0; h2 < 2; ++h2) {
+                    const int e = 4 * g4 + 2 * h2;
+                    const floatx2 m0 = {acc[0][nb][e], acc[0][nb][e + 1]}, m1 = {acc[1][nb][e], acc[1][nb][e + 1]};
+                    const floatx2 m2 = {acc[2][nb][e], acc[2][nb][e + 1]}, m3 = {acc[3][nb][e], acc[3][nb][e + 1]};
+                    const floatx2 s0 = pk_add2(pk_add2(m0, m1), m2), s1 = pk_sub2(pk_sub2(m1, m2), m3);
+                    t0[2 * h2] = s0.x;
+                    t0[2 * h2 + 1] = s0.y;
+                    t1[2 * h2] = s1.x;
+                    t1[2 * h2 + 1] = s1.y;
+                }
+                *reinterpret_cast<floatx4*>(ep_w + 8 * g4) = t0;
+                *reinterpret_cast<floatx4*>(ep_w + BP * EP_ROW + 8 * g4) = t1;
+            }
+            if (nb + 1 == NB && vn >= 0) {
+                if (!kEarly) VQ_W_OPEN(g.job[jn], vn)
+                VQ_W_ACC0(g.job[jn])
+            }
+            __syncthreads();
+#pragma unroll
+            for (int b_ = 0; b_ < 2; ++b_) {
+                const floatx4 v0 = *reinterpret_cast<const floatx4*>(ep_r + (0 * 2 + b_) * BP * EP_ROW);
+                const floatx4 v1 = *reinterpret_cast<const floatx4*>(ep_r + (1 * 2 + b_) * BP * EP_ROW);
+                const floatx4 v2 = *reinterpret_cast<const floatx4*>(ep_r + (2 * 2 + b_) * BP * EP_ROW);
+                const floatx4 v3 = *reinterpret_cast<const floatx4*>(ep_r + (3 * 2 + b_) * BP * EP_ROW);
+                floatx4 y0 = pk_add(pk_add(v0, v1), v2);
+                floatx4 y1 = pk_sub(pk_sub(v1, v2), v3);
+                if (relu) {
+#pragma unroll
+                    for (int r = 0; r < 4; ++r) {
+                        y0[r] = relu1(y0[r]);
+                        y1[r] = relu1(y1[r]);
+                    }
+                }
+                const bool blk_ok = nb < blocks_ok;
+                __builtin_amdgcn_raw_buffer_store_b128(__builtin_bit_cast(uintx4, y0), out_rsrc, blk_ok ? ooff[b_] : 0xFFFFFFFFu, nb * (32 * 4), 0);
+                __builtin_amdgcn_raw_buffer_store_b128(__builtin_bit_cast(uintx4, y1), out_rsrc, blk_ok ? ooff[2 + b_] : 0xFFFFFFFFu, nb * (32 * 4), 0);
+            }
+            if (nb + 1 < NB) __syncthreads();
+        }
+        VQ_PHASE(3)
+        if (vn < 0) break;
+        v = vn;
+        job = jn;
+        job = jn;
+        VQ_PHASE(0)
+        __syncthreads();
+    }
+#undef VQ_W_OPEN
+#undef VQ_W_ACC0
 #undef VQ_W_LOAD_PATCH
 #undef VQ_W_LOAD_U
 #undef VQ_W_STORE_H
 #undef VQ_W_STEP
 #undef VQ_W_READ_A
 
-    const int et = tid >> 3, ec = tid & 7;
-    const TileAt te = tile_at(et, img0, ty0, tx0, a.th, a.tw, a.s_th, a.s_tw);
-    const __amdgpu_buffer_rsrc_t out_rsrc = __builtin_amdgcn_make_buffer_rsrc(a.out, 0, a.out_bytes, 0x00020000);
-    const int oy = 2 * te.ty, ox = 2 * te.tx;
-    const int obase = (imul24(imul24(te.img * a.H + oy, a.W) + ox, a.Cs_out) + a.coff_out + n0 + ec * 4) * 4;
-    const bool tile_ok = p0 + et < a.P;
-    unsigned ooff[4];
-#pragma unroll
-    for (int u = 0; u < 4; ++u)
-        ooff[u] = (tile_ok && oy + (u >> 1) < a.H && ox + (u & 1) < a.W) ? (unsigned)(obase + ((u >> 1) * a.W + (u & 1)) * a.Cs_out * 4)
-                                                                           : 0xFFFFFFFFu;
-    float* ep_w = hs + ((wave * 2) * BP + l31) * EP_ROW + 4 * half;
-    const float* ep_r = hs + et * EP_ROW + ec * 4;
-    __syncthreads();
-#pragma unroll
-    for (int nb = 0; nb < NB; ++nb) {
-#pragma unroll
-        for (int g = 0; g < 4; ++g) {
-            floatx4 t0, t1;
-#pragma unroll
-            for (int h2 = 0; h2 < 2; ++h2) {
-                const int e = 4 * g + 2 * h2;
-                const floatx2 m0 = {acc[0][nb][e], acc[0][nb][e + 1]}, m1 = {acc[1][nb][e], acc[1][nb][e + 1]};
-                const floatx2 m2 = {acc[2][nb][e], acc[2][nb][e + 1]}, m3 = {acc[3][nb][e], acc[3][nb][e + 1]};
-                const floatx2 s0 = pk_add2(pk_add2(m0, m1), m2), s1 = pk_sub2(pk_sub2(m1, m2), m3);
-                t0[2 * h2] = s0.x;
-                t0[2 * h2 + 1] = s0.y;
-                t1[2 * h2] = s1.x;
-                t1[2 * h2 + 1] = s1.y;
-            }
-            *reinterpret_cast<floatx4*>(ep_w + 8 * g) = t0;
-            *reinterpret_cast<floatx4*>(ep_w + BP * EP_ROW + 8 * g) = t1;
-        }
-        __syncthreads();
-#pragma unroll
-        for (int b_ = 0; b_ < 2; ++b_) {
-            const floatx4 v0 = *reinterpret_cast<const floatx4*>(ep_r + (0 * 2 + b_) * BP * EP_ROW);
-            const floatx4 v1 = *reinterpret_cast<const floatx4*>(ep_r + (1 * 2 + b_) * BP * EP_ROW);
-            const floatx4 v2 = *reinterpret_cast<const floatx4*>(ep_r + (2 * 2 + b_) * BP * EP_ROW);
-            const floatx4 v3 = *reinterpret_cast<const floatx4*>(ep_r + (3 * 2 + b_) * BP * EP_ROW);
-            floatx4 y0 = pk_add(pk_add(v0, v1), v2);
-            floatx4 y1 = pk_sub(pk_sub(v1, v2), v3);
-            if (a.relu) {
-#pragma unroll
-                for (int r = 0; r < 4; ++r) {
-                    y0[r] = relu1(y0[r]);
-                    y1[r] = relu1(y1[r]);
-                }
-            }
-            const bool blk_ok = n0 + 32 * nb < a.Cout;
-            __builtin_amdgcn_raw_buffer_store_b128(__builtin_bit_cast(uintx4, y0), out_rsrc, blk_ok ? ooff[b_] : 0xFFFFFFFFu, nb * (32 * 4), 0);
-            __builtin_amdgcn_raw_buffer_store_b128(__builtin_bit_cast(uintx4, y1), out_rsrc, blk_ok ? ooff[2 + b_] : 0xFFFFFFFFu, nb * (32 * 4), 0);
-        }
-        if (nb + 1 < NB) __syncthreads();
-    }
-    VQ_PHASE(3)
 }
 
 constexpr int BP16 = 16;
@@ -269,65 +334,32 @@
 constexpr int LDS16_FLOATS = EP16_FLOATS > 2 * HS16_STAGE ? EP16_FLOATS : 2 * HS16_STAGE;
 
 template <int NB>
-__device__ __forceinline__ void wino16_unit(const WinoJob& a, int unit, float* hs) {
+__device__ __forceinline__ void wino16_walk(const WinoGroup& g, int v, const int stride, float* hs) {
     constexpr int NBLK = 2 * NB;
     const int tid = threadIdx.x;
     const int lane = tid & 63, l15 = lane & 15, kq = lane >> 4;
     const int wave = __builtin_amdgcn_readfirstlane(tid >> 6);
-    const int tile = xcd_remap(unit, a.n_units);
-    const int pb = (int)magic_div((unsigned)tile, a.m_tiles_n);
-    const int p0 = pb * BP16;
-    const int n0 = (tile - pb * a.tiles_n) * (32 * NB);
-    const int tpi = a.th * a.tw;
-    const int img0 = (int)magic_div((unsigned)p0, a.m_tpi);
-    const int rem0 = p0 - img0 * tpi;
-    const int ty0 = (int)magic_div((unsigned)rem0, a.m_tw);
-    const int tx0 = rem0 - ty0 * a.tw;
-
-    const __amdgpu_buffer_rsrc_t in_rsrc = __builtin_amdgcn_make_buffer_rsrc(const_cast<float*>(a.in), 0, a.in_bytes, 0x00020000);
-    const __amdgpu_buffer_rsrc_t u_rsrc = __builtin_amdgcn_make_buffer_rsrc(const_cast<float*>(a.u), 0, a.u_bytes, 0x00020000);
-
-    unsigned poff[4];
+    int job;
+    v = walk_find(g, v, stride, job);
+    if (v < 0) return;
+
     const int lq = lane & 3;
-    {
-        const int t = lane >> 2;
-        const TileAt ta = tile_at(t, img0, ty0, tx0, a.th, a.tw, a.s_th, a.s_tw);
-        const int y = 2 * ta.ty - 1 + wave, x0 = 2 * ta.tx - 1;
-        const bool row_ok = p0 + t < a.P && (unsigned)y < (unsigned)a.H;
-        const int base = (imul24(imul24(ta.img * a.H + y, a.W) + x0, a.Cs_in) + a.coff_in + lq * 4) * 4;
-        const int px = a.Cs_in * 4;
-#pragma unroll
-        for (int c = 0; c < 4; ++c)
-            poff[c] = (row_ok && (unsigned)(x0 + c) < (unsigned)a.W) ? (unsigned)(base + c * px) : 0xFFFFFFFFu;
-    }
     const int slot_a = ((lq & 1) << 2) | (lq & 2);
     const int hs_store = (wave * 4 * BP16 + (lane >> 2)) * KC16 + slot_a;
-
     const int ra = wave == 0 ? 0 : (wave == 2 ? 2 : 1);
     const int rb = wave == 3 ? 3 : (wave == 2 ? 1 : 2);
     const float sgn = wave == 1 ? 1.0f : -1.0f;
     const floatx2 sgn2 = {sgn, sgn};
     const int fa_off = (ra * 4 * BP16 + l15) * KC16 + kq * 4;
     const int fb_off = (rb * 4 * BP16 + l15) * KC16 + kq * 4;
+
+    UnitAt at;
+    __amdgpu_buffer_rsrc_t in_rsrc, u_rsrc;
+    unsigned poff[4];
     unsigned uvoff[NBLK];
-#pragma unroll
-    for (int b = 0; b < NBLK; ++b) uvoff[b] = (n0 + 16 * b < a.Cout) ? (unsigned)(((16 * b + l15) * 16 + kq * 4) * 4) : 0xFFFFFFFFu;
-    const unsigned u_step = (unsigned)(16 * a.Cout * 16 * 4);
-    const unsigned u_wave = (unsigned)(((wave * 4) * a.Cout + n0) * 16 * 4);
-    const unsigned u_pos = (unsigned)(a.Cout * 16 * 4);
-
+    unsigned u_step, u_wave, u_pos;
+    int nk;
     floatx4 acc[4][NBLK];
-#pragma unroll
-    for (int j = 0; j < 4; ++j)
-#pragma unroll
-        for (int b = 0; b < NBLK; ++b) acc[j][b] = (floatx4){0.f, 0.f, 0.f, 0.f};
-    if (wave == 1) {
-        const __amdgpu_buffer_rsrc_t b_rsrc = __builtin_amdgcn_make_buffer_rsrc(const_cast<float*>(a.bias), 0, (unsigned)a.Cout * 4u, 0x00020000);
-#pragma unroll
-        for (int b = 0; b < NBLK; ++b)
-            acc[1][b] = __builtin_bit_cast(floatx4, __builtin_amdgcn_raw_buffer_load_b128(b_rsrc, (unsigned)((n0 + 16 * b + 4 * kq) * 4), 0, 0));
-    }
-
     floatx4 d[4];
     floatx4 bq[4][NBLK];
 
@@ -377,82 +409,136 @@
         }                                                                                                       \
     }
 
-    const int nk = a.Cin / KC16;
-    VQ_W16_LOAD_PATCH(0)
-#pragma unroll
-    for (int j = 0; j < 4; ++j) VQ_W16_LOAD_U(0, j)
-    VQ_W16_STORE_H(0)
-    __syncthreads();
-    int kc = 0;
-    for (; kc + 1 < nk; ++kc) {
-        const int st = kc & 1;
-        VQ_W16_LOAD_PATCH(kc + 1)
+#define VQ_W16_OPEN(A, V)                                                                                          \
+    {                                                                                                           \
+        at = unit_at<BP16, NB>(A, (V) - (A).unit0);                                                             \
+        in_rsrc = __builtin_amdgcn_make_buffer_rsrc(const_cast<float*>((A).in), 0, (A).in_bytes, 0x00020000);     \
+        u_rsrc = __builtin_amdgcn_make_buffer_rsrc(const_cast<float*>((A).u), 0, (A).u_bytes, 0x00020000);        \
+        const int tid_o = fresh(tid), lane = tid_o & 63, l15 = lane & 15, kq = lane >> 4, lq = lane & 3;        \
+        const int t = lane >> 2;                                                                                \
+        const TileAt ta = tile_at(t, at.img0, at.ty0, at.tx0, (A).th, (A).tw, (A).s_th, (A).s_tw);                  \
+        const int y = 2 * ta.ty - 1 + wave, x0 = 2 * ta.tx - 1;                                                 \
+        const bool row_ok = at.p0 + t < (A).P && (unsigned)y < (unsigned)(A).H;                                   \
+        const int base = (imul24(imul24(ta.img * (A).H + y, (A).W) + x0, (A).Cs_in) + (A).coff_in + lq * 4) * 4;    \
+        const int px = (A).Cs_in * 4;                                                                            \
+        _Pragma("unroll") for (int c = 0; c < 4; ++c)                                                           \
+            poff[c] = (row_ok && (unsigned)(x0 + c) < (unsigned)(A).W) ? (unsigned)(base + c * px) : 0xFFFFFFFFu; \
+        _Pragma("unroll") for (int b = 0; b < NBLK; ++b)                                                        \
+            uvoff[b] = (at.n0 + 16 * b < (A).Cout) ? (unsigned)(((16 * b + l15) * 16 + kq * 4) * 4) : 0xFFFFFFFFu; \
+        u_step = (unsigned)(16 * (A).Cout * 16 * 4);             \
+        u_wave = (unsigned)(((wave * 4) * (A).Cout + at.n0) * 16 * 4);                                           \
+        u_pos = (unsigned)((A).Cout * 16 * 4);                                       \
+        nk = (A).Cin / KC16;                                                                                     \
+        VQ_W16_LOAD_PATCH(0)                                                                                    \
+        _Pragma("unroll") for (int j = 0; j < 4; ++j) VQ_W16_LOAD_U(0, j)                                       \
+    }
+#define VQ_W16_ACC0(A)                                                                                            \
+    {                                                                                                           \
+        _Pragma("unroll") for (int j = 0; j < 4; ++j)                                                           \
+            _Pragma("unroll") for (int b = 0; b < NBLK; ++b) acc[j][b] = (floatx4){0.f, 0.f, 0.f, 0.f};         \
+        if (wave == 1) {                                                                                        \
+            const int kq = (fresh(tid) >> 4) & 3;                                                               \
+            const __amdgpu_buffer_rsrc_t b_rsrc =                                                               \
+                __builtin_amdgcn_make_buffer_rsrc(const_cast<float*>((A).bias), 0, (unsigned)(A).Cout * 4u, 0x00020000); \
+            _Pragma("unroll") for (int b = 0; b < NBLK; ++b)                                                    \
+                acc[1][b] = __builtin_bit_cast(floatx4, __builtin_amdgcn_raw_buffer_load_b128(                  \
+                                                            b_rsrc, (unsigned)((at.n0 + 16 * b + 4 * kq) * 4), 0, 0)); \
+        }                                                                                                       \
+    }
+
+    VQ_W16_OPEN(g.job[job], v)
+    VQ_W16_ACC0(g.job[job])
+    for (;;) {
+        const WinoJob& a = g.job[job];
+        VQ_W16_STORE_H(0)
+        __syncthreads();
+        int kc = 0;
+        for (; kc + 1 < nk; ++kc) {
+            const int st = kc & 1;
+            VQ_W16_LOAD_PATCH(kc + 1)
+            __builtin_amdgcn_sched_barrier(0);
+            VQ_W16_STEP(st, kc, true)
+            VQ_W16_STORE_H(st ^ 1)
+            __syncthreads();
+        }
+        VQ_W16_STEP(kc & 1, kc, false)
+
+        const int tid_e = fresh(tid), l15 = tid_e & 15, kq = (tid_e >> 4) & 3;
+        const int et = (tid_e >> 3) & 15, ec = tid_e & 7, bsel = tid_e >> 7;
+        float* ep_w = hs + ((wave * 2) * BP16 + l15) * EP_ROW + 4 * kq;
+        const float* ep_r = hs + et * EP_ROW + ec * 4;
+        const TileAt te = tile_at(et, at.img0, at.ty0, at.tx0, a.th, a.tw, a.s_th, a.s_tw);
+        const __amdgpu_buffer_rsrc_t out_rsrc = __builtin_amdgcn_make_buffer_rsrc(a.out, 0, a.out_bytes, 0x00020000);
+        const int oy = 2 * te.ty, ox = 2 * te.tx;
+        const int obase = (imul24(imul24(te.img * a.H + oy, a.W) + ox, a.Cs_out) + a.coff_out + at.n0 + ec * 4) * 4;
+        const bool tile_ok = at.p0 + et < a.P;
+        unsigned ooff[2];
+#pragma unroll
+        for (int u = 0; u < 2; ++u)
+            ooff[u] = (tile_ok && oy + u < a.H && ox + bsel < a.W) ? (unsigned)(obase + (u * a.W + bsel) * a.Cs_out * 4) : 0xFFFFFFFFu;
+        const int relu = a.relu;
+        const int blocks_ok = (a.Cout - at.n0 + 31) >> 5;
+
+        int jn = 0;
+        const int vn = walk_find(g, v + stride, stride, jn);
+        if (vn >= 0) VQ_W16_OPEN(g.job[jn], vn)
         __builtin_amdgcn_sched_barrier(0);
-        VQ_W16_STEP(st, kc, true)
-        VQ_W16_STORE_H(st ^ 1)
         __syncthreads();
-    }
-    VQ_W16_STEP(kc & 1, kc, false)
+#pragma unroll
+        for (int nb = 0; nb < NB; ++nb) {
+#pragma unroll
+            for (int bb = 0; bb < 2; ++bb) {
+                const int b = 2 * nb + bb;
+                floatx4 t0, t1;
+#pragma unroll
+                for (int h2 = 0; h2 < 2; ++h2) {
+                    const floatx2 m0 = {acc[0][b][2 * h2], acc[0][b][2 * h2 + 1]}, m1 = {acc[1][b][2 * h2], acc[1][b][2 * h2 + 1]};
+                    const floatx2 m2 = {acc[2][b][2 * h2], acc[2][b][2 * h2 + 1]}, m3 = {acc[3][b][2 * h2], acc[3][b][2 * h2 + 1]};
+                    const floatx2 s0 = pk_add2(pk_add2(m0, m1), m2), s1 = pk_sub2(pk_sub2(m1, m2), m3);
+                    t0[2 * h2] = s0.x;
+                    t0[2 * h2 + 1] = s0.y;
+                    t1[2 * h2] = s1.x;
+                    t1[2 * h2 + 1] = s1.y;
+                }
+                *reinterpret_cast<floatx4*>(ep_w + 16 * bb) = t0;
+                *reinterpret_cast<floatx4*>(ep_w + BP16 * EP_ROW + 16 * bb) = t1;
+            }
+            if (nb + 1 == NB && vn >= 0) VQ_W16_ACC0(g.job[jn])
+            __syncthreads();
+            {
+                const floatx4 v0 = *reinterpret_cast<const floatx4*>(ep_r + (0 * 2 + bsel) * BP16 * EP_ROW);
+                const floatx4 v1 = *reinterpret_cast<const floatx4*>(ep_r + (1 * 2 + bsel) * BP16 * EP_ROW);
+                const floatx4 v2 = *reinterpret_cast<const floatx4*>(ep_r + (2 * 2 + bsel) * BP16 * EP_ROW);
+                const floatx4 v3 = *reinterpret_cast<const floatx4*>(ep_r + (3 * 2 + bsel) * BP16 * EP_ROW);
+                floatx4 y0 = pk_add(pk_add(v0, v1), v2);
+                floatx4 y1 = pk_sub(pk_sub(v1, v2), v3);
+                if (relu) {
+#pragma unroll
+                    for (int r = 0; r < 4; ++r) {
+                        y0[r] = relu1(y0[r]);
+                        y1[r] = relu1(y1[r]);
+                    }
+                }
+                const bool blk_ok = nb < blocks_ok;
+                __builtin_amdgcn_raw_buffer_store_b128(__builtin_bit_cast(uintx4, y0), out_rsrc, blk_ok ? ooff[0] : 0xFFFFFFFFu, nb * (32 * 4), 0);
+                __builtin_amdgcn_raw_buffer_store_b128(__builtin_bit_cast(uintx4, y1), out_rsrc, blk_ok ? ooff[1] : 0xFFFFFFFFu, nb * (32 * 4), 0);
+            }
+            if (nb + 1 < NB) __syncthreads();
+        }
+        if (vn < 0) break;
+        v = vn;
+        job = jn;
+        job = jn;
+        __syncthreads();
+    }
+#undef VQ_W16_OPEN
+#undef VQ_W16_ACC0
 #undef VQ_W16_LOAD_PATCH
 #undef VQ_W16_LOAD_U
 #undef VQ_W16_PUT
 #undef VQ_W16_STORE_H
 #undef VQ_W16_STEP
 #undef VQ_W16_READ_A
-
-    const int et = (tid >> 3) & 15, ec = tid & 7, bsel = tid >> 7;
-    const TileAt te = tile_at(et, img0, ty0, tx0, a.th, a.tw, a.s_th, a.s_tw);
-    const __amdgpu_buffer_rsrc_t out_rsrc = __builtin_amdgcn_make_buffer_rsrc(a.out, 0, a.out_bytes, 0x00020000);
-    const int oy = 2 * te.ty, ox = 2 * te.tx;
-    const int obase = (imul24(imul24(te.img * a.H + oy, a.W) + ox, a.Cs_out) + a.coff_out + n0 + ec * 4) * 4;
-    const bool tile_ok = p0 + et < a.P;
-    unsigned ooff[2];
-#pragma unroll
-    for (int u = 0; u < 2; ++u)
-        ooff[u] = (tile_ok && oy + u < a.H && ox + bsel < a.W) ? (unsigned)(obase + (u * a.W + bsel) * a.Cs_out * 4) : 0xFFFFFFFFu;
-    float* ep_w = hs + ((wave * 2) * BP16 + l15) * EP_ROW + 4 * kq;
-    const float* ep_r = hs + et * EP_ROW + ec * 4;
-    __syncthreads();
-#pragma unroll
-    for (int nb = 0; nb < NB; ++nb) {
-#pragma unroll
-        for (int bb = 0; bb < 2; ++bb) {
-            const int b = 2 * nb + bb;
-            floatx4 t0, t1;
-#pragma unroll
-            for (int h2 = 0; h2 < 2; ++h2) {
-                const floatx2 m0 = {acc[0][b][2 * h2], acc[0][b][2 * h2 + 1]}, m1 = {acc[1][b][2 * h2], acc[1][b][2 * h2 + 1]};
-                const floatx2 m2 = {acc[2][b][2 * h2], acc[2][b][2 * h2 + 1]}, m3 = {acc[3][b][2 * h2], acc[3][b][2 * h2 + 1]};
-                const floatx2 s0 = pk_add2(pk_add2(m0, m1), m2), s1 = pk_sub2(pk_sub2(m1, m2), m3);
-                t0[2 * h2] = s0.x;
-                t0[2 * h2 + 1] = s0.y;
-                t1[2 * h2] = s1.x;
-                t1[2 * h2 + 1] = s1.y;
-            }
-            *reinterpret_cast<floatx4*>(ep_w + 16 * bb) = t0;
-            *reinterpret_cast<floatx4*>(ep_w + BP16 * EP_ROW + 16 * bb) = t1;
-        }
-        __syncthreads();
-        {
-            const floatx4 v0 = *reinterpret_cast<const floatx4*>(ep_r + (0 * 2 + bsel) * BP16 * EP_ROW);
-            const floatx4 v1 = *reinterpret_cast<const floatx4*>(ep_r + (1 * 2 + bsel) * BP16 * EP_ROW);
-            const floatx4 v2 = *reinterpret_cast<const floatx4*>(ep_r + (2 * 2 + bsel) * BP16 * EP_ROW);
-            const floatx4 v3 = *reinterpret_cast<const floatx4*>(ep_r + (3 * 2 + bsel) * BP16 * EP_ROW);
-            floatx4 y0 = pk_add(pk_add(v0, v1), v2);
-            floatx4 y1 = pk_sub(pk_sub(v1, v2), v3);
-            if (a.relu) {
-#pragma unroll
-                for (int r = 0; r < 4; ++r) {
-                    y0[r] = relu1(y0[r]);
-                    y1[r] = relu1(y1[r]);
-                }
-            }
-            const bool blk_ok = n0 + 32 * nb < a.Cout;
-            __builtin_amdgcn_raw_buffer_store_b128(__builtin_bit_cast(uintx4, y0), out_rsrc, blk_ok ? ooff[0] : 0xFFFFFFFFu, nb * (32 * 4), 0);
-            __builtin_amdgcn_raw_buffer_store_b128(__builtin_bit_cast(uintx4, y1), out_rsrc, blk_ok ? ooff[1] : 0xFFFFFFFFu, nb * (32 * 4), 0);
-        }
-        if (nb + 1 < NB) __syncthreads();
-    }
 }
 
 template <int NB, int TB>
@@ -460,8 +546,8 @@
 void wino_f2x2_3x3_kernel(WinoGroup g) {
     extern __shared__ __attribute__((aligned(16))) char smem_raw[];
     float* hs = reinterpret_cast<float*>(smem_raw);
-    const int b = blockIdx.x;
-    if (b >= g.pool_unit0) {
+    if ((int)blockIdx.x >= g.walk_wgs) {
+        const int b = (int)blockIdx.x - g.walk_wgs + g.pool_unit0;
         int q = 0;
         if (g.n_pools > 1 && b >= g.pool[1].unit0) q = 1;
         const PoolArgs& pa = g.pool[q];
@@ -479,17 +565,10 @@
         }
         return;
     }
-    int j = 0;
-#pragma unroll
-    for (int q = 1; q < kWinoMaxJobs; ++q)
-        if (q < g.n_jobs && b >= g.job[q].unit0) j = q;
-    const WinoJob& a = g.job[j];
-    const int unit = b - a.unit0;
-    if (unit >= a.n_units) return;
     if constexpr (TB == 16)
-        wino16_unit<NB>(a, unit, hs);
+        wino16_walk<NB>(g, (int)blockIdx.x, g.walk_wgs, hs);
     else
-        wino_unit<NB>(a, unit, hs);
+        wino_walk<NB>(g, (int)blockIdx.x, g.walk_wgs, hs);
 }
 
 unsigned magic_u32(unsigned d) { return d == 1 ? 0u : (unsigned)(0x100000000ull / d) + 1u; }
@@ -527,11 +606,24 @@
         units += (int)n;
     }
     g.total_units = units;
+    const int slots = g.walk_slots & ~7;
+    g.walk_wgs = slots >= 8 && slots < g.pool_unit0 ? slots : g.pool_unit0;
     auto kern = wino_f2x2_3x3_kernel<NB, TB>;
     const size_t lds = (TB == 16 ? LDS16_FLOATS : LDS_FLOATS) * sizeof(float);
-    VQ_LAUNCH(kern, units, 256, lds, stream, ev_start, ev_stop, g);
+    VQ_LAUNCH(kern, g.walk_wgs + (units - g.pool_unit0), 256, lds, stream, ev_start, ev_stop, g);
     VQ_CHECK_LAUNCH();
     return VQ_OK;
+}
+
+template <int NB, int TB>
+int slots_t(int cus) {
+    int per_cu = 0;
+    const size_t lds = (TB == 16 ? LDS16_FLOATS : LDS_FLOATS) * sizeof(float);
+    if (hipOccupancyMaxActiveBlocksPerMultiprocessor(&per_cu, wino_f2x2_3x3_kernel<NB, TB>, 256, lds) != hipSuccess) {
+        (void)hipGetLastError();
+        return 0;
+    }
+    return per_cu * cus;
 }
 
 }
@@ -556,4 +648,12 @@
     return fail(VQ_E_INVALID, "no Winograd kernel variant %d", variant);
 }
 
-}
+int wino_resident_workgroups(int variant, int cus) {
+    if (variant == 0) return slots_t<1, 32>(cus);
+    if (variant == 1) return slots_t<2, 32>(cus);
+    if (variant == 2) return slots_t<1, 16>(cus);
+    if (variant == 3) return slots_t<2, 16>(cus);
+    return 0;
+}
+
+}
```

Result: slower. 12510 clips/s (-2.4%).
